# yxgeee/OpenIBL

Hardware: NVIDIA H100
Metric: images_per_sec_extraction (higher is better)
Workload: dtype f32 (bf16x3 split on wgmma, fp32 accumulate)

## Files before the change

### include/iblb200.h

```cpp
#ifndef IBLB200_H_
#define IBLB200_H_

#include <stddef.h>
#include <stdint.h>

#ifdef __cplusplus
extern "C" {
#endif

#define IBLB200_ABI_VERSION 1

typedef enum ibl_status {
  IBL_OK = 0,
  IBL_ERR_BAD_ARG = 1,
  IBL_ERR_NOT_READY = 2,
  IBL_ERR_CUDA = 3,
  IBL_ERR_NO_DEVICE = 4,
  IBL_ERR_OOM = 5,
  IBL_ERR_UNSUPPORTED = 6
} ibl_status;

typedef struct ibl_engine ibl_engine;

#define IBL_OUT_VLAD 0x1u
#define IBL_OUT_PCA  0x2u
#define IBL_OUT_POOL 0x4u

#define IBL_CONV_SIMT_FP32 0
#define IBL_CONV_TC_BF16X3 1

int ibl_abi_version(void);
const char* ibl_status_string(int status);
const char* ibl_last_error(void);

int ibl_engine_create(int device, ibl_engine** out);
int ibl_engine_destroy(ibl_engine* e);
int ibl_engine_set_conv_mode(ibl_engine* e, int mode);
int ibl_engine_get_conv_mode(ibl_engine* e, int* mode);
int ibl_engine_set_gemm_mode(ibl_engine* e, int mode);
int ibl_engine_launch_count(ibl_engine* e, uint64_t* count);

int ibl_engine_set_vgg16(ibl_engine* e, const float* const* weights13,
                         const float* const* biases13, void* stream);
int ibl_engine_set_netvlad(ibl_engine* e, const float* conv_w, const float* centroids,
                           int K, int C, void* stream);
int ibl_engine_set_pca(ibl_engine* e, const float* W, const float* b, int P, int D, void* stream);

int ibl_vgg16_forward(ibl_engine* e, const float* x_nchw, int N, int H, int W,
                      float* feat_nhwc, float* feat_nchw, float* pool, void* stream);

int ibl_vgg16_prefix_forward(ibl_engine* e, const float* x_nchw, int N, int H, int W, int n_layers,
                             float* out_nhwc, void* stream);
int ibl_vgg16_layer_forward(ibl_engine* e, int layer, const float* x, int N, int H, int W, float* y_nhwc,
                            void* stream);
int ibl_maxpool2x2_forward(ibl_engine* e, const float* x_nhwc, int N, int H, int W, int C, float* y_nhwc,
                           void* stream);
int ibl_maxpool2x2_backward(ibl_engine* e, const float* x_nhwc, const float* gy_nhwc, int N, int H, int W, int C,
                            float* gx_nhwc, void* stream);
int ibl_vgg16_layer_backward(ibl_engine* e, int layer, const float* x, const float* y, const float* gy, int N,
                             int H, int W, float* gx, float* gw, float* gb, void* stream);

int ibl_netvlad_forward(ibl_engine* e, const float* feat, int nhwc, int N, int C, int S,
                        const float* conv_w, const float* centroids, int K,
                        int normalize_input, float* vlad_raw, float* vlad_norm, void* stream);
int ibl_netvlad_backward(ibl_engine* e, const float* feat, int nhwc, int N, int C, int S,
                         const float* conv_w, const float* centroids, int K, int normalize_input,
                         const float* grad_vlad, float* grad_feat, float* grad_conv_w,
                         float* grad_centroids, void* stream);
int ibl_vlad_normalize(ibl_engine* e, const float* vlad_raw, int N, int K, int C,
                       float* out, void* stream);

int ibl_pca_l2(ibl_engine* e, const float* v, int N, int D, const float* W, const float* b,
               int P, float* out, void* stream);
int ibl_l2_normalize_rows(ibl_engine* e, const float* x, int N, int D, float* out, void* stream);

int ibl_extract(ibl_engine* e, const float* x_nchw, int N, int H, int W, unsigned flags,
                float* out, float* pool, void* stream);
int ibl_extract_host(ibl_engine* e, const float* x_nchw_host, int N, int H, int W,
                     unsigned flags, float* out_host, float* pool_host, void* stream);

int ibl_extract_host_submit(ibl_engine* e, int slot, const float* x_nchw_host, int N, int H, int W, unsigned flags,
                            float* out_host, float* pool_host, void* stream);
int ibl_extract_host_wait(ibl_engine* e, int slot);

int ibl_preprocess_u8(ibl_engine* e, const uint8_t* x_nhwc, int N, int H, int W, const float* mean3,
                      const float* std3, float* out_nchw, void* stream);
int ibl_resize_bilinear_u8(ibl_engine* e, const uint8_t* x_nhwc, int N, int Hin, int Win, int Hout, int Wout,
                           const int* bounds_h, const int* kk_h, int ksize_h, const int* bounds_v, const int* kk_v,
                           int ksize_v, uint8_t* out_nhwc, void* stream);
int ibl_extract_host_u8(ibl_engine* e, const uint8_t* x_nhwc_host, int N, int H, int W, const float* mean3,
                        const float* std3, unsigned flags, float* out_host, float* pool_host, void* stream);

typedef struct ibl_jpeg_info {
  int width, height;
  int components;
  int h_samp, v_samp;
  int restart_interval;
  int intervals;
  int mcus;
  uint64_t entropy_bytes;
  char reason[120];
} ibl_jpeg_info;
int ibl_jpeg_parse(const uint8_t* data, size_t len, ibl_jpeg_info* out);
int ibl_jpeg_decode_u8(ibl_engine* e, const uint8_t* const* files, const size_t* lens, int N, uint8_t* out_u8,
                       const uint64_t* out_offsets, int* status, int* err_dev, void* stream);
typedef struct ibl_jpeg_scan {
  int components;
  int comp[3];
  int ss, se, ah, al;
  int restart_interval;
  int intervals;
} ibl_jpeg_scan;
int ibl_jpeg_parse_progressive(const uint8_t* data, size_t len, ibl_jpeg_info* out, int* n_scans,
                               ibl_jpeg_scan* scans, int max_scans);
int ibl_jpeg_decode_progressive_u8(ibl_engine* e, const uint8_t* const* files, const size_t* lens, int N,
                                   uint8_t* out_u8, const uint64_t* out_offsets, int* status, int* err_dev,
                                   void* stream);

typedef struct ibl_png_info {
  int width, height;
  int color_type;
  int bit_depth;
  int palette_size;
  uint64_t zlib_bytes;
  char reason[120];
} ibl_png_info;
int ibl_png_parse(const uint8_t* data, size_t len, ibl_png_info* out);
int ibl_png_decode_u8(ibl_engine* e, const uint8_t* const* files, const size_t* lens, int N, uint8_t* out_u8,
                      const uint64_t* out_offsets, int* status, int* err_dev, void* stream);

typedef struct ibl_color_jitter_params {
  int order[4];
  float brightness, contrast, saturation, hue;
} ibl_color_jitter_params;
int ibl_color_jitter_u8(ibl_engine* e, uint8_t* buf, const uint64_t* out_offsets, const int* H, const int* W,
                        const ibl_color_jitter_params* params, int N, void* stream);

int ibl_l2dist_self(ibl_engine* e, const float* x, int n, int d, float* out, void* stream);
int ibl_l2dist_dense(ibl_engine* e, const float* q, int m, const float* db, int n, int d,
                     float* out, void* stream);
int ibl_l2dist_topk(ibl_engine* e, const float* q, int m, const float* db, int n, int n_valid,
                    int d, int k, int64_t idx_base, float* out_dist, int64_t* out_idx,
                    void* stream);
int ibl_topk_rows(ibl_engine* e, const float* dist, int m, int n, int k, float* out_dist,
                  int64_t* out_idx, void* stream);
int ibl_argsort_rows(ibl_engine* e, const float* dist, int m, int n, int64_t* out_idx, void* stream);
int ibl_topk_merge(ibl_engine* e, const float* cand_dist, const int64_t* cand_idx, int parts,
                   int m, int k_in, int k_out, float* out_dist, int64_t* out_idx, void* stream);
int ibl_l2dist_topk_host(ibl_engine* e, const float* q_host, int m, const float* db_host, int n,
                         int d, int k, float* out_dist_host, int64_t* out_idx_host, void* stream);

int ibl_knn_rowmax(ibl_engine* e, const float* X, int N, int d, int row0, int n_rows, int w, int64_t* out_idx,
                   float* out_dist, float* out_rowmax, void* stream);
int ibl_rerank_topk(ibl_engine* e, const float* X, int N, int m, int d, const int64_t* nbr_idx, const float* nbr_dist,
                    int w, const float* rowmax, int k1, int k2, float lambda_value, const int64_t* orig_idx, int k_orig,
                    int k, float* out_dist, int64_t* out_idx, void* stream);
int ibl_rerank_dense(ibl_engine* e, const float* qg, const float* qq, const float* gg, int m, int n, int k1, int k2,
                     double lambda_value, float* out_final, void* stream);

int ibl_gemm_nt(ibl_engine* e, const float* A, int m, const float* B, int n, int k, float alpha, float* C, int mode,
                void* stream);

int ibl_debug_dist_flagged(ibl_engine* e, int* count, void* stream);
int ibl_debug_dist_path(ibl_engine* e, int* path);
int ibl_debug_knn_flagged(ibl_engine* e, int* count, void* stream);
int ibl_debug_rerank_workspace_bytes(ibl_engine* e, uint64_t* bytes);
int ibl_selftest_tc(ibl_engine* e, float* max_rel_err);

int ibl_debug_conv3x3(ibl_engine* e, const float* x_nhwc, int N, int H, int W, int cin,
                      const float* w_oihw, const float* bias, int cout, int relu, int pool, int mode,
                      int bn_override, float* y_nhwc, void* stream);

int ibl_debug_gemm_tn(ibl_engine* e, const float* A, const float* B, float* C, void* stream);
int ibl_debug_umma_strided(ibl_engine* e, const void* A, int rows, const void* B, int s0, int group_rows,
                           int base_mode, float* D, void* stream);
int ibl_debug_umma_halo_view(ibl_engine* e, const void* A, int rows, const void* B, int s0, int group_rows,
                             int half_rows, float* D, void* stream);
int ibl_debug_conv1_fused(ibl_engine* e, const float* x, int N, int H, int W, void* y_hi, void* y_lo, void* stream);
int ibl_debug_time_layer(ibl_engine* e, int layer, const float* x, int N, int H, int W, int bn_override,
                         int reps, float* ms_out);

#ifdef __cplusplus
}
#endif
#endif
```

### openibl_b200/_cabi.py

```python
from __future__ import annotations

import ctypes
import os
from ctypes import POINTER, Structure, c_char, c_char_p, c_double, c_float, c_int, c_int64, c_size_t, c_uint, c_uint64, c_void_p

_HERE = os.path.dirname(os.path.abspath(__file__))
LIB_PATH = os.path.join(_HERE, "lib", "libiblb200.so")

IBL_OK = 0
STATUS_NAMES = {0: "IBL_OK", 1: "IBL_ERR_BAD_ARG", 2: "IBL_ERR_NOT_READY", 3: "IBL_ERR_CUDA",
                4: "IBL_ERR_NO_DEVICE", 5: "IBL_ERR_OOM", 6: "IBL_ERR_UNSUPPORTED"}
OUT_VLAD, OUT_PCA, OUT_POOL = 0x1, 0x2, 0x4
CONV_SIMT_FP32, CONV_TC_BF16X3 = 0, 1
PNG_SIGNATURE = b"\x89PNG\r\n\x1a\n"

_P = c_void_p


class JpegInfo(Structure):
    _fields_ = [("width", c_int), ("height", c_int), ("components", c_int), ("h_samp", c_int), ("v_samp", c_int),
                ("restart_interval", c_int), ("intervals", c_int), ("mcus", c_int), ("entropy_bytes", c_uint64),
                ("reason", c_char * 120)]


class JpegScan(Structure):
    _fields_ = [("components", c_int), ("comp", c_int * 3), ("ss", c_int), ("se", c_int), ("ah", c_int), ("al", c_int),
                ("restart_interval", c_int), ("intervals", c_int)]


class PngInfo(Structure):
    _fields_ = [("width", c_int), ("height", c_int), ("color_type", c_int), ("bit_depth", c_int),
                ("palette_size", c_int), ("zlib_bytes", c_uint64), ("reason", c_char * 120)]


class ColorJitterParams(Structure):
    _fields_ = [("order", c_int * 4), ("brightness", c_float), ("contrast", c_float), ("saturation", c_float),
                ("hue", c_float)]


SIGNATURES = {
    "ibl_abi_version": (c_int, []),
    "ibl_status_string": (c_char_p, [c_int]),
    "ibl_last_error": (c_char_p, []),
    "ibl_engine_create": (c_int, [c_int, POINTER(c_void_p)]),
    "ibl_engine_destroy": (c_int, [_P]),
    "ibl_engine_set_conv_mode": (c_int, [_P, c_int]),
    "ibl_engine_set_gemm_mode": (c_int, [_P, c_int]),
    "ibl_engine_get_conv_mode": (c_int, [_P, POINTER(c_int)]),
    "ibl_engine_launch_count": (c_int, [_P, POINTER(c_uint64)]),
    "ibl_engine_set_vgg16": (c_int, [_P, POINTER(c_void_p), POINTER(c_void_p), _P]),
    "ibl_engine_set_netvlad": (c_int, [_P, _P, _P, c_int, c_int, _P]),
    "ibl_engine_set_pca": (c_int, [_P, _P, _P, c_int, c_int, _P]),
    "ibl_vgg16_forward": (c_int, [_P, _P, c_int, c_int, c_int, _P, _P, _P, _P]),
    "ibl_vgg16_prefix_forward": (c_int, [_P, _P, c_int, c_int, c_int, c_int, _P, _P]),
    "ibl_vgg16_layer_forward": (c_int, [_P, c_int, _P, c_int, c_int, c_int, _P, _P]),
    "ibl_maxpool2x2_forward": (c_int, [_P, _P, c_int, c_int, c_int, c_int, _P, _P]),
    "ibl_maxpool2x2_backward": (c_int, [_P, _P, _P, c_int, c_int, c_int, c_int, _P, _P]),
    "ibl_vgg16_layer_backward": (c_int, [_P, c_int, _P, _P, _P, c_int, c_int, c_int, _P, _P, _P, _P]),
    "ibl_netvlad_forward": (c_int, [_P, _P, c_int, c_int, c_int, c_int, _P, _P, c_int, c_int, _P, _P, _P]),
    "ibl_netvlad_backward": (c_int, [_P, _P, c_int, c_int, c_int, c_int, _P, _P, c_int, c_int, _P, _P, _P, _P, _P]),
    "ibl_vlad_normalize": (c_int, [_P, _P, c_int, c_int, c_int, _P, _P]),
    "ibl_pca_l2": (c_int, [_P, _P, c_int, c_int, _P, _P, c_int, _P, _P]),
    "ibl_l2_normalize_rows": (c_int, [_P, _P, c_int, c_int, _P, _P]),
    "ibl_extract": (c_int, [_P, _P, c_int, c_int, c_int, c_uint, _P, _P, _P]),
    "ibl_extract_host": (c_int, [_P, _P, c_int, c_int, c_int, c_uint, _P, _P, _P]),
    "ibl_extract_host_submit": (c_int, [_P, c_int, _P, c_int, c_int, c_int, c_uint, _P, _P, _P]),
    "ibl_extract_host_wait": (c_int, [_P, c_int]),
    "ibl_preprocess_u8": (c_int, [_P, _P, c_int, c_int, c_int, _P, _P, _P, _P]),
    "ibl_resize_bilinear_u8": (c_int, [_P, _P, c_int, c_int, c_int, c_int, c_int, _P, _P, c_int, _P, _P, c_int, _P, _P]),
    "ibl_extract_host_u8": (c_int, [_P, _P, c_int, c_int, c_int, _P, _P, c_uint, _P, _P, _P]),
    "ibl_jpeg_parse": (c_int, [c_char_p, c_size_t, POINTER(JpegInfo)]),
    "ibl_jpeg_decode_u8": (c_int, [_P, _P, _P, c_int, _P, _P, _P, _P, _P]),
    "ibl_jpeg_parse_progressive": (c_int, [c_char_p, c_size_t, POINTER(JpegInfo), POINTER(c_int), POINTER(JpegScan),
                                           c_int]),
    "ibl_jpeg_decode_progressive_u8": (c_int, [_P, _P, _P, c_int, _P, _P, _P, _P, _P]),
    "ibl_png_parse": (c_int, [c_char_p, c_size_t, POINTER(PngInfo)]),
    "ibl_png_decode_u8": (c_int, [_P, _P, _P, c_int, _P, _P, _P, _P, _P]),
    "ibl_color_jitter_u8": (c_int, [_P, _P, _P, _P, _P, POINTER(ColorJitterParams), c_int, _P]),
    "ibl_l2dist_dense": (c_int, [_P, _P, c_int, _P, c_int, c_int, _P, _P]),
    "ibl_l2dist_self": (c_int, [_P, _P, c_int, c_int, _P, _P]),
    "ibl_l2dist_topk": (c_int, [_P, _P, c_int, _P, c_int, c_int, c_int, c_int, c_int64, _P, _P, _P]),
    "ibl_topk_rows": (c_int, [_P, _P, c_int, c_int, c_int, _P, _P, _P]),
    "ibl_argsort_rows": (c_int, [_P, _P, c_int, c_int, _P, _P]),
    "ibl_topk_merge": (c_int, [_P, _P, _P, c_int, c_int, c_int, c_int, _P, _P, _P]),
    "ibl_l2dist_topk_host": (c_int, [_P, _P, c_int, _P, c_int, c_int, c_int, _P, _P, _P]),
    "ibl_knn_rowmax": (c_int, [_P, _P, c_int, c_int, c_int, c_int, c_int, _P, _P, _P, _P]),
    "ibl_rerank_topk": (c_int, [_P, _P, c_int, c_int, c_int, _P, _P, c_int, _P, c_int, c_int, c_float, _P, c_int,
                                c_int, _P, _P, _P]),
    "ibl_rerank_dense": (c_int, [_P, _P, _P, _P, c_int, c_int, c_int, c_int, c_double, _P, _P]),
    "ibl_debug_rerank_workspace_bytes": (c_int, [_P, POINTER(c_uint64)]),
    "ibl_debug_knn_flagged": (c_int, [_P, POINTER(c_int), _P]),
    "ibl_gemm_nt": (c_int, [_P, _P, c_int, _P, c_int, c_int, c_float, _P, c_int, _P]),
    "ibl_debug_dist_flagged": (c_int, [_P, POINTER(c_int), _P]),
    "ibl_debug_dist_path": (c_int, [_P, POINTER(c_int)]),
    "ibl_selftest_tc": (c_int, [_P, POINTER(c_float)]),
    "ibl_debug_gemm_tn": (c_int, [_P, _P, _P, _P, _P]),
    "ibl_debug_umma_strided": (c_int, [_P, _P, c_int, _P, c_int, c_int, c_int, _P, _P]),
    "ibl_debug_umma_halo_view": (c_int, [_P, _P, c_int, _P, c_int, c_int, c_int, _P, _P]),
    "ibl_debug_conv1_fused": (c_int, [_P, _P, c_int, c_int, c_int, _P, _P, _P]),
    "ibl_debug_time_layer": (c_int, [_P, c_int, _P, c_int, c_int, c_int, c_int, c_int, POINTER(c_float)]),
    "ibl_debug_conv3x3": (c_int, [_P, _P, c_int, c_int, c_int, c_int, _P, _P, c_int, c_int, c_int, c_int,
                                  c_int, _P, _P]),
}

_lib = None


class IblError(RuntimeError):
    def __init__(self, status: int, where: str, detail: str):
        self.status = status
        super().__init__(f"{where}: {STATUS_NAMES.get(status, status)}: {detail}")


def load(build_if_missing: bool = True) -> ctypes.CDLL:
    global _lib
    if _lib is not None:
        return _lib
    if not os.path.exists(LIB_PATH):
        if not build_if_missing:
            raise ImportError(f"{LIB_PATH} is missing; run `python -m openibl_b200.build`")
        from . import build as _build
        _build.build()
    lib = ctypes.CDLL(LIB_PATH)
    for name, (res, args) in SIGNATURES.items():
        fn = getattr(lib, name)
        fn.restype = res
        fn.argtypes = args
    _lib = lib
    return lib


def jpeg_parse(data: bytes) -> dict:
    lib = load()
    info = JpegInfo()
    data = bytes(data)
    st = lib.ibl_jpeg_parse(data, len(data), ctypes.byref(info))
    return {"ok": st == IBL_OK, "status": st, "width": info.width, "height": info.height,
            "components": info.components, "h_samp": info.h_samp, "v_samp": info.v_samp,
            "restart_interval": info.restart_interval, "intervals": info.intervals, "mcus": info.mcus,
            "entropy_bytes": info.entropy_bytes, "reason": info.reason.decode()}


def jpeg_parse_progressive(data: bytes) -> dict:
    lib = load()
    info = JpegInfo()
    data = bytes(data)
    n = c_int(0)
    st = lib.ibl_jpeg_parse_progressive(data, len(data), ctypes.byref(info), ctypes.byref(n), None, 0)
    scans = (JpegScan * max(n.value, 1))()
    if n.value:
        lib.ibl_jpeg_parse_progressive(data, len(data), ctypes.byref(info), ctypes.byref(n), scans, n.value)
    return {"ok": st == IBL_OK, "status": st, "width": info.width, "height": info.height,
            "components": info.components, "h_samp": info.h_samp, "v_samp": info.v_samp,
            "restart_interval": info.restart_interval, "intervals": info.intervals, "mcus": info.mcus,
            "entropy_bytes": info.entropy_bytes, "reason": info.reason.decode(),
            "scans": [{"components": tuple(s.comp[:s.components]), "ss": s.ss, "se": s.se, "ah": s.ah, "al": s.al,
                       "restart_interval": s.restart_interval, "intervals": s.intervals}
                      for s in scans[:n.value]]}


def png_parse(data: bytes) -> dict:
    lib = load()
    info = PngInfo()
    data = bytes(data)
    st = lib.ibl_png_parse(data, len(data), ctypes.byref(info))
    return {"ok": st == IBL_OK, "status": st, "width": info.width, "height": info.height,
            "color_type": info.color_type, "bit_depth": info.bit_depth, "palette_size": info.palette_size,
            "zlib_bytes": info.zlib_bytes, "reason": info.reason.decode()}


def check(status: int, where: str) -> None:
    if status != IBL_OK:
        lib = load()
        detail = lib.ibl_last_error().decode() or lib.ibl_status_string(status).decode()
        raise IblError(status, where, detail)
```

### openibl_b200/csrc/common.cuh

```cuda
#pragma once
#include <cuda_runtime.h>
#include <cuda_bf16.h>
#include <stdint.h>
#include <stdio.h>
#include <atomic>
#include <string>

#include "../../include/iblb200.h"

namespace ibl {

void set_last_error(const std::string& s);

#define IBL_CUDA_OK(expr)                                                          \
  do {                                                                             \
    cudaError_t _e = (expr);                                                       \
    if (_e != cudaSuccess) {                                                       \
      ::ibl::set_last_error(std::string(#expr) + ": " + cudaGetErrorString(_e) +   \
                            " (" __FILE__ ":" + std::to_string(__LINE__) + ")");   \
      return IBL_ERR_CUDA;                                                         \
    }                                                                              \
  } while (0)

#define IBL_RET(expr)                 \
  do {                                \
    int _s = (expr);                  \
    if (_s != IBL_OK) return _s;      \
  } while (0)

#define IBL_REQUIRE(cond, msg)                                  \
  do {                                                          \
    if (!(cond)) {                                              \
      ::ibl::set_last_error(std::string("bad argument: ") + msg); \
      return IBL_ERR_BAD_ARG;                                   \
    }                                                           \
  } while (0)

static inline int cdiv(long long a, long long b) { return (int)((a + b - 1) / b); }

constexpr int NETVLAD_MAX_K = 64;
static inline int check_netvlad_clusters(int K) {
  if (K < 1) {
    set_last_error("bad argument: NetVLAD num_clusters must be in 1..64, got " + std::to_string(K));
    return IBL_ERR_BAD_ARG;
  }
  if (K > NETVLAD_MAX_K) {
    set_last_error("unsupported: NetVLAD num_clusters must be in 1..64, got " + std::to_string(K));
    return IBL_ERR_UNSUPPORTED;
  }
  return IBL_OK;
}

struct DeviceOnce {
  std::atomic<unsigned long long> mask[4];
  DeviceOnce() { for (auto& m : mask) m.store(0); }
  static int cur() { int d = 0; cudaGetDevice(&d); return d & 255; }
  bool done() const { const int d = cur(); return (mask[d >> 6].load(std::memory_order_acquire) >> (d & 63)) & 1ull; }
  void mark() { const int d = cur(); mask[d >> 6].fetch_or(1ull << (d & 63), std::memory_order_release); }
};

static inline int device_sm_count() {
  int dev = 0, sms = 0;
  cudaGetDevice(&dev);
  if (cudaDeviceGetAttribute(&sms, cudaDevAttrMultiProcessorCount, dev) != cudaSuccess || sms <= 0) sms = 132;
  return sms;
}

struct ConvLayer {
  int cin, cout;
  bool relu;
  bool pool;
};

struct ConvParams {
  float* w_tck = nullptr;
  float* bias = nullptr;
  __nv_bfloat16* w_hi = nullptr;
  __nv_bfloat16* w_lo = nullptr;
  int cin_pad = 0;
};

int launch_repack_weights(const float* w_oihw, int cout, int cin, ConvParams& p, cudaStream_t s);
int launch_conv3x3_simt(const float* x_nhwc, const ConvParams& p, int N, int H, int W, int cin,
                        int cout, bool relu, float* y_nhwc, cudaStream_t s);
int launch_conv1_1(const float* x_nchw, const ConvParams& p, int N, int H, int W, float* y_nhwc, cudaStream_t s);
int launch_maxpool2x2(const float* x, int N, int H, int W, int C, float* y, cudaStream_t s);
int launch_nhwc_to_nchw(const float* x, int N, int S, int C, float* y, cudaStream_t s);
int launch_u8_hwc_to_nchw_norm(const uint8_t* x, int N, int H, int W, const float* mean, const float* stdv, float* y,
                               cudaStream_t s);
int launch_global_maxpool_nhwc(const float* x, int N, int S, int C, float* y, cudaStream_t s);
int launch_planes_to_f32(const __nv_bfloat16* hi, const __nv_bfloat16* lo, size_t n, float* y,
                         cudaStream_t s);
int launch_f32_to_planes(const float* x, size_t n, __nv_bfloat16* hi, __nv_bfloat16* lo,
                         cudaStream_t s);

struct TcConvPlan;
int tc_driver_init();
int launch_conv3x3_tc(const __nv_bfloat16* x_hi, const __nv_bfloat16* x_lo, const ConvParams& p,
                      int N, int H, int W, int cin, int cout, bool relu, bool pool,
                      __nv_bfloat16* y_hi, __nv_bfloat16* y_lo, float* y_f32, cudaStream_t s,
                      float* ssq = nullptr, int* ssq_parts = nullptr);
int launch_conv1_fused_tc(const float* x_nchw, const float* w1_oihw, const float* bias1, const ConvParams& p2, int N, int H,
                          int W, __nv_bfloat16* y_hi, __nv_bfloat16* y_lo, cudaStream_t s);
int launch_maxpool2x2_planes(const __nv_bfloat16* hi, const __nv_bfloat16* lo, int N, int H, int W,
                             int C, __nv_bfloat16* yhi, __nv_bfloat16* ylo, cudaStream_t s);
int tc_selftest(float* max_rel_err, cudaStream_t s);
int launch_argsort_rows(const float* dist, long long ld, int m, int n, long long* idx, unsigned long long* scratch,
                        cudaStream_t s, uint64_t* launches);
int launch_resize_bilinear_u8(const uint8_t* x, int N, int Hin, int Win, int Hout, int Wout, const int* bounds_h,
                              const int* kk_h, int ksize_h, const int* bounds_v, const int* kk_v, int ksize_v,
                              uint8_t* tmp, uint8_t* out, cudaStream_t s, uint64_t* launches);
struct JpegWs {
  uint8_t* host = nullptr;
  size_t host_cap = 0;
  void* blob = nullptr;
  size_t blob_cap = 0;
  void* arena = nullptr;
  size_t arena_cap = 0;
  cudaEvent_t copied = nullptr;
  bool pending = false;
};
void jpeg_ws_destroy(JpegWs* ws);
int ws_open(JpegWs** pws);
int grow_device(void** p, size_t* cap, size_t need);
int stage_host(JpegWs* ws, size_t bytes);
int jpeg_decode_u8(JpegWs** ws, const uint8_t* const* files, const size_t* lens, int N, uint8_t* out_u8,
                   const uint64_t* out_offsets, int* status, int* err_dev, cudaStream_t s, uint64_t* launches);
int jpeg_decode_progressive_u8(JpegWs** ws, const uint8_t* const* files, const size_t* lens, int N, uint8_t* out_u8,
                               const uint64_t* out_offsets, int* status, int* err_dev, cudaStream_t s,
                               uint64_t* launches);
int png_decode_u8(JpegWs** ws, const uint8_t* const* files, const size_t* lens, int N, uint8_t* out_u8,
                  const uint64_t* out_offsets, int* status, int* err_dev, cudaStream_t s, uint64_t* launches);
struct JitterWs;
void jitter_ws_destroy(JitterWs* ws);
int color_jitter_u8(JitterWs** ws, uint8_t* buf, const uint64_t* out_offsets, const int* H, const int* W,
                    const ibl_color_jitter_params* params, int N, cudaStream_t s, uint64_t* launches);
int launch_repack_weights_dgrad(const float* w_tck, int cout, int cin, __nv_bfloat16* w_hi, __nv_bfloat16* w_lo,
                                cudaStream_t s);
int launch_relu_mask_planes(const float* g, const float* y, size_t n, bool relu, __nv_bfloat16* hi, __nv_bfloat16* lo,
                            cudaStream_t s);
int launch_maxpool2x2_bwd(const float* x, const float* gy, int N, int H, int W, int C, float* gx, cudaStream_t s);
int wgrad_tc_splits(int N, int H, int W, int cin, int cout);
int launch_conv_wgrad_tc(const __nv_bfloat16* g_hi, const __nv_bfloat16* g_lo, const __nv_bfloat16* x_hi,
                         const __nv_bfloat16* x_lo, int N, int H, int W, int cin, int cout, float* part, int splits,
                         float* bpart, float* dw_oihw, float* db, cudaStream_t s);
int launch_conv1_1_wgrad(const float* x_nchw, const __nv_bfloat16* g_hi, const __nv_bfloat16* g_lo, int N, int H, int W,
                         float* part, float* dw_oihw, float* db, cudaStream_t s);
int launch_conv1_1_tc(const float* x_nchw, const float* w_oihw, const float* bias, int N, int H, int W,
                      __nv_bfloat16* y_hi, __nv_bfloat16* y_lo, cudaStream_t s);
int debug_gmma_strided(const void* A, int rows, const void* B, int s0, int group_rows, int half_rows, int base_mode,
                       float* D, cudaStream_t s);
int debug_gemm_tn(const float* A, const float* B, float* C, cudaStream_t s);
int netvlad_tc_units(int B, int S);
int launch_netvlad_tc(const __nv_bfloat16* x_hi, const __nv_bfloat16* x_lo, int B, int S, int K,
                      const __nv_bfloat16* w_hi, const __nv_bfloat16* w_lo, const float* ssq, int ssq_parts,
                      const float* cent, bool normalize_input, float* part, float* asum_part, int* ticket,
                      float* vlad_raw, float* vlad_norm, cudaStream_t s);
int launch_global_maxpool_planes(const __nv_bfloat16* hi, const __nv_bfloat16* lo, int N, int S, int C, float* y,
                                 cudaStream_t s);

int dist_top16_max_runs(int n_valid);
int launch_dist_top16_tc(const __nv_bfloat16* q_hi, const __nv_bfloat16* q_lo, const float* qn, int m,
                         const __nv_bfloat16* d_hi, const __nv_bfloat16* d_lo, const float* dn, int n,
                         int n_valid, int K, float* cand_d, long long* cand_i, int max_runs, int* runs_out,
                         cudaStream_t s);
int launch_dist_dense_tc(const __nv_bfloat16* q_hi, const __nv_bfloat16* q_lo, const float* qn, int m,
                         const __nv_bfloat16* d_hi, const __nv_bfloat16* d_lo, const float* dn, int n, int K,
                         float* out, long long ld_out, cudaStream_t s);
size_t dist1_workspace_bytes(int m, int n, int d, size_t* off );
int launch_dist_topk_1pass(const float* q, int m, const float* db, int n, int n_valid, int d, int k, long long idx_base,
                           void* ws, float* out_dist, long long* out_idx, uint64_t* launches, cudaStream_t s);
const int* dist1_flag_counter(const void* ws, int m, int n, int d);
size_t dist_guard_workspace_bytes(int m);
int launch_dist_guard_bf16x3(const float* q, const float* q_sq, const float2* q_err, int m, const float* db,
                             const float* db_sq, const float2* db_err, int n_valid, int d, const float* screened, int kc,
                             int k, long long idx_base, void* ws, float* out_dist, long long* out_idx,
                             uint64_t* launches, cudaStream_t s);
int launch_bf16x3_colmax(const float2* err, const float* sq, int n, float* out3, cudaStream_t s);
int pca_tc_splits(int P, int D);
int launch_pca_partial_tc(const __nv_bfloat16* w_hi, const __nv_bfloat16* w_lo, int P,
                          const __nv_bfloat16* v_hi, const __nv_bfloat16* v_lo, int N, int D,
                          float* partial, int* splits_out, cudaStream_t s);
int launch_rescore_sort(const float* q, const float* qn, int m, const float* db, const float* dbn, int d,
                        const long long* cand_i, int kc, int k_out, long long idx_base, float* out_dist,
                        long long* out_idx, cudaStream_t s);
int launch_pca_finalize(const float* partial, int splits, int N, int P, const float* bias, float* out,
                        cudaStream_t s);

struct NetvladWorkspace {
  float* assign = nullptr;
  float* invnorm = nullptr;
  float* asum = nullptr;
  float* raw = nullptr;
  size_t cap_N = 0;
  int cap_S = 0, cap_K = 0, cap_C = 0;
};
int launch_netvlad(const float* feat, bool nhwc, int N, int C, int S, const float* conv_w,
                   const float* centroids, int K, bool normalize_input, float* assign,
                   float* invnorm, float* asum, float* vlad_raw, float* vlad_norm,
                   cudaStream_t s, uint64_t* launches);
int launch_vlad_normalize(const float* raw, int N, int K, int C, float* out, cudaStream_t s);
int launch_netvlad_assign(const float* feat, bool nhwc, int N, int C, int S, const float* conv_w, int K,
                          bool normalize_input, float* assign, float* invnorm, cudaStream_t s);
int launch_netvlad_backward(const float* x, bool nhwc, int N, int C, int S, const float* conv_w,
                            const float* centroids, int K, const float* g, bool normalize_input, float* assign,
                            float* invnorm, float* dz, float* part, int splits, float* dx, float* dW,
                            float* dcent, cudaStream_t s, uint64_t* launches);

int launch_pca_l2(const float* v, int N, int D, const float* W, const float* b, int P,
                  float* partial, int splits, float* out, cudaStream_t s, uint64_t* launches);
int launch_l2_normalize_rows(const float* x, int N, int D, float* out, cudaStream_t s);
int launch_row_sqnorm(const float* x, int N, int D, float* out, cudaStream_t s);
int launch_scale(const float* x, float s, int n, float* y, cudaStream_t st);
int launch_planes_sqnorm(const float* x, int N, int D, __nv_bfloat16* hi, __nv_bfloat16* lo, float* sq,
                         float2* err, cudaStream_t st);
int launch_l2dist_dense(const float* q, const float* qn, int m, const float* db, const float* dbn,
                        int n, int d, float* out, long long ld_out, cudaStream_t s);

size_t knn_rowmax_workspace_bytes(int N, int d, int n_rows, int w);
const int* knn_rowmax_flag_counter(const void* ws, int N, int d, int n_rows, int w);
int launch_knn_rowmax(const float* X, int N, int d, int row0, int n_rows, int w, void* ws, long long* out_idx,
                      float* out_dist, float* out_max, uint64_t* launches, cudaStream_t s);
struct RerankWs;
RerankWs* rerank_ws_create();
void rerank_ws_destroy(RerankWs* w);
size_t rerank_ws_bytes(const RerankWs* w);
int launch_rerank_topk(RerankWs* W, const float* X, int N, int m, int d, const long long* nbr, const float* nbr_dist,
                       int w, const float* rowmax, int k1, int k2, float lam, const long long* orig, int k_orig, int k,
                       float* out_dist, long long* out_idx, uint64_t* launches, cudaStream_t s);
int launch_rerank_dense(RerankWs* W, const float* qg, const float* qq, const float* gg, int m, int n, int k1, int k2,
                        double lam, float* out, uint64_t* launches, cudaStream_t s);

int launch_topk_rows(const float* dist, long long ld, int m, int n_valid, int k, int64_t idx_base,
                     float* out_dist, int64_t* out_idx, bool accumulate, cudaStream_t s);
int launch_topk_merge(const float* cand_dist, const int64_t* cand_idx, int parts, int m, int k_in,
                      int k_out, float* out_dist, int64_t* out_idx, cudaStream_t s);

}
```

### openibl_b200/csrc/engine.cu

```cuda
#include <stdlib.h>

#include <mutex>
#include <new>
#include <vector>

#include "common.cuh"

namespace ibl {

static thread_local std::string g_last_error;
void set_last_error(const std::string& s) { g_last_error = s; }
void tc_set_bn_override(int bn);

static const ConvLayer kVgg16[13] = {
    {3, 64, true, false},    {64, 64, true, true},
    {64, 128, true, false},  {128, 128, true, true},
    {128, 256, true, false}, {256, 256, true, false}, {256, 256, true, true},
    {256, 512, true, false}, {512, 512, true, false}, {512, 512, true, true},
    {512, 512, true, false}, {512, 512, true, false}, {512, 512, false, false}
};

struct DevBuf {
  void* p = nullptr;
  size_t cap = 0;
  int ensure(size_t bytes) {
    if (bytes <= cap) return IBL_OK;
    if (p) cudaFree(p);
    p = nullptr;
    cap = 0;
    cudaError_t e = cudaMalloc(&p, bytes);
    if (e != cudaSuccess) {
      cudaGetLastError();
      set_last_error("workspace cudaMalloc(" + std::to_string(bytes) + " B) failed: " + cudaGetErrorString(e));
      return IBL_ERR_OOM;
    }
    cap = bytes;
    return IBL_OK;
  }
  void release() {
    if (p) cudaFree(p);
    p = nullptr;
    cap = 0;
  }
  template <class T> T* as() const { return reinterpret_cast<T*>(p); }
};

}

using namespace ibl;

struct ibl_engine {
  int device = 0;
  int conv_mode = IBL_CONV_TC_BF16X3;
  int gemm_mode = IBL_CONV_TC_BF16X3;
  uint64_t launches = 0;
  bool vgg_ready = false;
  ConvParams conv[13];
  float* w0_oihw = nullptr;
  const float* nv_w = nullptr;
  const float* nv_c = nullptr;
  int nv_K = 0, nv_C = 0;
  const float* pca_W = nullptr;
  const float* pca_b = nullptr;
  int pca_P = 0, pca_D = 0;
  DevBuf act[2];
  DevBuf feat;
  DevBuf nv_assign, nv_inv, nv_raw, vlad;
  DevBuf pca_partial;
  DevBuf qn, dbn, dist_chunk, cand_d, cand_i;
  DevBuf stage_in, stage_out, stage_out2, stage_u8;
  DevBuf q_pl, db_pl, v_pl, pca_pl;
  const float* pca_pl_src = nullptr;
  DevBuf mrg_d, mrg_i;
  DevBuf bw_g, bw_x, bw_part, bw_w;
  DevBuf d1_ws;
  DevBuf q_err, db_err, guard_ws;
  DevBuf knn_ws;
  const int* knn_flag_counter = nullptr;
  JpegWs* jpeg_ws = nullptr;
  JpegWs* jpeg_prog_ws = nullptr;
  JpegWs* png_ws = nullptr;
  JitterWs* jitter_ws = nullptr;
  RerankWs* rr_ws = nullptr;
  const int* flag_counter = nullptr;
  int dist_path = -1;
  DevBuf ssq, nv_part, nv_asum, nvw_pl;
  DevBuf nv_ticket;
  const float* nvw_pl_src = nullptr;
  cudaStream_t copy_stream = nullptr;
  cudaEvent_t copy_ev[2] = {nullptr, nullptr};
  DevBuf pipe_in[2], pipe_out[2], pipe_pool[2];
  cudaEvent_t pipe_h2d[2] = {nullptr, nullptr}, pipe_done[2] = {nullptr, nullptr};
  bool pipe_busy[2] = {false, false};
};

struct FeatPlanes {
  __nv_bfloat16* hi = nullptr;
  __nv_bfloat16* lo = nullptr;
  int ssq_parts = 0;
};

namespace {

inline cudaStream_t S(void* s) { return reinterpret_cast<cudaStream_t>(s); }

struct DeviceGuard {
  int prev = -1;
  explicit DeviceGuard(int dev) {
    cudaGetDevice(&prev);
    if (prev != dev) cudaSetDevice(dev);
    else prev = -1;
  }
  ~DeviceGuard() {
    if (prev >= 0) cudaSetDevice(prev);
  }
};

int ensure_tickets(ibl_engine* e, int n_images, cudaStream_t s) {
  const size_t need = (size_t)(n_images > 1024 ? n_images : 1024) * sizeof(int);
  if (e->nv_ticket.cap >= need) return IBL_OK;
  IBL_RET(e->nv_ticket.ensure(need));
  IBL_CUDA_OK(cudaMemsetAsync(e->nv_ticket.p, 0, e->nv_ticket.cap, s));
  return IBL_OK;
}

int vgg_forward_impl(ibl_engine* e, const float* x, int N, int H, int W, float* feat_nhwc,
                     cudaStream_t s, FeatPlanes* planes_out = nullptr, int last_layer = 12) {
  const size_t act_bytes = (size_t)N * H * W * 64 * 4;
  IBL_RET(e->act[0].ensure(act_bytes));
  IBL_RET(e->act[1].ensure(act_bytes));
  int h = H, w = W;
  int cur = 0;
  if (e->conv_mode == IBL_CONV_SIMT_FP32) {
    IBL_RET(launch_conv1_1(x, e->conv[0], N, h, w, e->act[0].as<float>(), s));
    e->launches++;
    for (int l = 1; l <= last_layer; ++l) {
      const ConvLayer& L = kVgg16[l];
      const bool last = (l == last_layer);
      float* dst = (last && !L.pool) ? feat_nhwc : e->act[cur ^ 1].as<float>();
      IBL_RET(launch_conv3x3_simt(e->act[cur].as<float>(), e->conv[l], N, h, w, L.cin, L.cout, L.relu, dst, s));
      e->launches++;
      cur ^= 1;
      if (L.pool) {
        IBL_RET(launch_maxpool2x2(e->act[cur].as<float>(), N, h, w, L.cout, last ? feat_nhwc : e->act[cur ^ 1].as<float>(), s));
        e->launches++;
        cur ^= 1;
        h /= 2;
        w /= 2;
      }
    }
    return IBL_OK;
  }
  auto hi_of = [&](int b, size_t elems) { (void)elems; return e->act[b].as<__nv_bfloat16>(); };
  auto lo_of = [&](int b, size_t elems) { return e->act[b].as<__nv_bfloat16>() + elems; };
  size_t elems = (size_t)N * h * w * 64;
  int first_l = 1;
  const bool fused1 = last_layer >= 2 && h >= 2 && w >= 2;
  if (fused1) {
    const size_t out_elems = (size_t)N * (h / 2) * (w / 2) * 64;
    IBL_RET(launch_conv1_fused_tc(x, e->w0_oihw, e->conv[0].bias, e->conv[1], N, h, w, hi_of(1, out_elems),
                                  lo_of(1, out_elems), s));
    e->launches++;
    cur = 1;
    h /= 2;
    w /= 2;
    first_l = 2;
  } else {
    IBL_RET(launch_conv1_1_tc(x, e->w0_oihw, e->conv[0].bias, N, h, w, hi_of(0, elems), lo_of(0, elems), s));
    e->launches++;
  }
  for (int l = first_l; l <= last_layer; ++l) {
    const ConvLayer& L = kVgg16[l];
    const bool last = (l == last_layer);
    const size_t in_elems = (size_t)N * h * w * L.cin;
    const int oh = L.pool ? h / 2 : h, ow = L.pool ? w / 2 : w;
    const size_t out_elems = (size_t)N * oh * ow * L.cout;
    if (last && planes_out) {
      IBL_RET(e->ssq.ensure((size_t)8 * N * oh * ow * sizeof(float)));
      IBL_RET(launch_conv3x3_tc(hi_of(cur, in_elems), lo_of(cur, in_elems), e->conv[l], N, h, w, L.cin,
                                L.cout, L.relu, L.pool, hi_of(cur ^ 1, out_elems), lo_of(cur ^ 1, out_elems),
                                nullptr, s, e->ssq.as<float>(), &planes_out->ssq_parts));
      planes_out->hi = hi_of(cur ^ 1, out_elems);
      planes_out->lo = lo_of(cur ^ 1, out_elems);
      e->launches++;
      return IBL_OK;
    }
    IBL_RET(launch_conv3x3_tc(hi_of(cur, in_elems), lo_of(cur, in_elems), e->conv[l], N, h, w, L.cin,
                              L.cout, L.relu, L.pool, last ? nullptr : hi_of(cur ^ 1, out_elems),
                              last ? nullptr : lo_of(cur ^ 1, out_elems), last ? feat_nhwc : nullptr, s));
    e->launches++;
    cur ^= 1;
    h = oh;
    w = ow;
  }
  return IBL_OK;
}

}

extern "C" {

int ibl_abi_version(void) { return IBLB200_ABI_VERSION; }

const char* ibl_status_string(int status) {
  switch (status) {
    case IBL_OK: return "ok";
    case IBL_ERR_BAD_ARG: return "bad argument";
    case IBL_ERR_NOT_READY: return "parameters for this stage were not set";
    case IBL_ERR_CUDA: return "CUDA error";
    case IBL_ERR_NO_DEVICE: return "no usable sm_90 CUDA device (this library has no CPU fallback)";
    case IBL_ERR_OOM: return "out of device memory";
    case IBL_ERR_UNSUPPORTED: return "unsupported request";
    default: return "unknown status";
  }
}

const char* ibl_last_error(void) { return g_last_error.c_str(); }

int ibl_engine_create(int device, ibl_engine** out) {
  if (!out) return IBL_ERR_BAD_ARG;
  *out = nullptr;
  int count = 0;
  if (cudaGetDeviceCount(&count) != cudaSuccess || count <= 0) {
    cudaGetLastError();
    set_last_error("no CUDA device visible; libiblb200 has no CPU fallback");
    return IBL_ERR_NO_DEVICE;
  }
  IBL_REQUIRE(device >= 0 && device < count, "device index out of range");
  cudaDeviceProp prop;
  IBL_CUDA_OK(cudaGetDeviceProperties(&prop, device));
  if (prop.major != 9 || prop.minor != 0) {
    set_last_error(std::string("device '") + prop.name + "' is sm_" + std::to_string(prop.major) +
                   std::to_string(prop.minor) + "; this library is built for sm_90a only");
    return IBL_ERR_NO_DEVICE;
  }
  ibl_engine* e = new (std::nothrow) ibl_engine();
  if (!e) return IBL_ERR_OOM;
  e->device = device;
  *out = e;
  return IBL_OK;
}

int ibl_engine_destroy(ibl_engine* e) {
  if (!e) return IBL_OK;
  DeviceGuard g(e->device);
  for (auto& c : e->conv) {
    if (c.w_tck) cudaFree(c.w_tck);
    if (c.bias) cudaFree(c.bias);
    if (c.w_hi) cudaFree(c.w_hi);
    if (c.w_lo) cudaFree(c.w_lo);
  }
  if (e->w0_oihw) cudaFree(e->w0_oihw);
  if (e->copy_stream) { cudaStreamDestroy(e->copy_stream); cudaEventDestroy(e->copy_ev[0]); cudaEventDestroy(e->copy_ev[1]); }
  for (int i = 0; i < 2; ++i) {
    if (e->pipe_h2d[i]) cudaEventDestroy(e->pipe_h2d[i]);
    if (e->pipe_done[i]) cudaEventDestroy(e->pipe_done[i]);
    e->pipe_in[i].release(); e->pipe_out[i].release(); e->pipe_pool[i].release();
  }
  DevBuf* bufs[] = {&e->act[0], &e->act[1], &e->feat, &e->nv_assign, &e->nv_inv, &e->nv_raw, &e->vlad,
                    &e->pca_partial, &e->qn, &e->dbn, &e->dist_chunk, &e->cand_d, &e->cand_i,
                    &e->stage_in, &e->stage_out, &e->stage_out2, &e->stage_u8, &e->q_pl, &e->db_pl, &e->v_pl, &e->pca_pl,
                    &e->mrg_d, &e->mrg_i, &e->d1_ws, &e->bw_g, &e->bw_x, &e->bw_part, &e->bw_w, &e->ssq, &e->nv_part, &e->nv_asum, &e->nvw_pl, &e->nv_ticket};
  for (DevBuf* b : bufs) b->release();
  e->knn_ws.release();
  rerank_ws_destroy(e->rr_ws);
  jpeg_ws_destroy(e->jpeg_ws);
  jpeg_ws_destroy(e->jpeg_prog_ws);
  jpeg_ws_destroy(e->png_ws);
  jitter_ws_destroy(e->jitter_ws);
  delete e;
  return IBL_OK;
}

int ibl_engine_set_conv_mode(ibl_engine* e, int mode) {
  IBL_REQUIRE(e, "null engine");
  IBL_REQUIRE(mode == IBL_CONV_SIMT_FP32 || mode == IBL_CONV_TC_BF16X3, "unknown conv mode");
  e->conv_mode = mode;
  return IBL_OK;
}
int ibl_engine_get_conv_mode(ibl_engine* e, int* mode) {
  IBL_REQUIRE(e && mode, "null argument");
  *mode = e->conv_mode;
  return IBL_OK;
}
int ibl_engine_set_gemm_mode(ibl_engine* e, int mode) {
  IBL_REQUIRE(e, "null engine");
  IBL_REQUIRE(mode == IBL_CONV_SIMT_FP32 || mode == IBL_CONV_TC_BF16X3, "unknown gemm mode");
  e->gemm_mode = mode;
  return IBL_OK;
}
int ibl_engine_launch_count(ibl_engine* e, uint64_t* count) {
  IBL_REQUIRE(e && count, "null argument");
  *count = e->launches;
  return IBL_OK;
}

int ibl_engine_set_vgg16(ibl_engine* e, const float* const* w13, const float* const* b13, void* stream) {
  IBL_REQUIRE(e && w13 && b13, "null argument");
  DeviceGuard g(e->device);
  for (int l = 0; l < 13; ++l) {
    IBL_REQUIRE(w13[l] && b13[l], "null weight/bias pointer");
    const ConvLayer& L = kVgg16[l];
    ConvParams& p = e->conv[l];
    const size_t nw = (size_t)L.cout * L.cin * 9;
    if (!p.w_tck) IBL_CUDA_OK(cudaMalloc(&p.w_tck, nw * sizeof(float)));
    if (!p.bias) IBL_CUDA_OK(cudaMalloc(&p.bias, L.cout * sizeof(float)));
    if (L.cin % 64 == 0) {
      if (!p.w_hi) IBL_CUDA_OK(cudaMalloc(&p.w_hi, nw * sizeof(__nv_bfloat16)));
      if (!p.w_lo) IBL_CUDA_OK(cudaMalloc(&p.w_lo, nw * sizeof(__nv_bfloat16)));
      p.cin_pad = L.cin;
    }
    IBL_RET(launch_repack_weights(w13[l], L.cout, L.cin, p, S(stream)));
    IBL_CUDA_OK(cudaMemcpyAsync(p.bias, b13[l], L.cout * sizeof(float), cudaMemcpyDeviceToDevice, S(stream)));
    if (l == 0) {
      if (!e->w0_oihw) IBL_CUDA_OK(cudaMalloc(&e->w0_oihw, nw * sizeof(float)));
      IBL_CUDA_OK(cudaMemcpyAsync(e->w0_oihw, w13[0], nw * sizeof(float), cudaMemcpyDeviceToDevice, S(stream)));
    }
    e->launches++;
  }
  e->vgg_ready = true;
  return IBL_OK;
}

static int netvlad_weight_planes(const float* conv_w, int K, __nv_bfloat16* pl, cudaStream_t s) {
  const size_t n64 = (size_t)NETVLAD_MAX_K * 512;
  if (K < NETVLAD_MAX_K) IBL_CUDA_OK(cudaMemsetAsync(pl, 0, n64 * 4, s));
  return launch_f32_to_planes(conv_w, (size_t)K * 512, pl, pl + n64, s);
}

int ibl_engine_set_netvlad(ibl_engine* e, const float* conv_w, const float* centroids, int K, int C,
                           void* stream) {
  IBL_RET(check_netvlad_clusters(K));
  IBL_REQUIRE(e && conv_w && centroids, "null argument");
  IBL_REQUIRE(C >= 4 && C % 4 == 0, "NetVLAD dim must be a positive multiple of 4");
  e->nv_w = conv_w;
  e->nv_c = centroids;
  e->nv_K = K;
  e->nv_C = C;
  e->nvw_pl_src = nullptr;
  if (C == 512) {
    DeviceGuard g(e->device);
    IBL_RET(e->nvw_pl.ensure((size_t)NETVLAD_MAX_K * 512 * 4));
    IBL_RET(netvlad_weight_planes(conv_w, K, e->nvw_pl.as<__nv_bfloat16>(), S(stream)));
    e->launches++;
    e->nvw_pl_src = conv_w;
  }
  return IBL_OK;
}

int ibl_engine_set_pca(ibl_engine* e, const float* W, const float* b, int P, int D, void* stream) {
  (void)stream;
  IBL_REQUIRE(e && W && b, "null argument");
  IBL_REQUIRE(P >= 1 && D >= 4 && D % 4 == 0, "bad PCA shape");
  e->pca_W = W;
  e->pca_b = b;
  e->pca_P = P;
  e->pca_D = D;
  e->pca_pl_src = nullptr;
  if (D % 64 == 0) {
    DeviceGuard g(e->device);
    const size_t n = (size_t)P * D;
    IBL_RET(e->pca_pl.ensure(n * 4));
    IBL_RET(launch_f32_to_planes(W, n, e->pca_pl.as<__nv_bfloat16>(), e->pca_pl.as<__nv_bfloat16>() + n, S(stream)));
    e->launches++;
    e->pca_pl_src = W;
  }
  return IBL_OK;
}

int ibl_vgg16_forward(ibl_engine* e, const float* x, int N, int H, int W, float* feat_nhwc,
                      float* feat_nchw, float* pool, void* stream) {
  IBL_REQUIRE(e && x, "null argument");
  IBL_REQUIRE(N >= 1 && H >= 16 && W >= 16, "VGG16 trunk needs N>=1 and H,W>=16");
  if (!e->vgg_ready) { set_last_error("ibl_engine_set_vgg16 was not called"); return IBL_ERR_NOT_READY; }
  DeviceGuard g(e->device);
  const int fh = H / 16, fw = W / 16;
  const size_t fbytes = (size_t)N * fh * fw * 512 * sizeof(float);
  float* f = feat_nhwc;
  if (!f) {
    IBL_RET(e->feat.ensure(fbytes));
    f = e->feat.as<float>();
  }
  IBL_RET(vgg_forward_impl(e, x, N, H, W, f, S(stream)));
  if (feat_nchw) { IBL_RET(launch_nhwc_to_nchw(f, N, fh * fw, 512, feat_nchw, S(stream))); e->launches++; }
  if (pool) { IBL_RET(launch_global_maxpool_nhwc(f, N, fh * fw, 512, pool, S(stream))); e->launches++; }
  return IBL_OK;
}


int ibl_vgg16_prefix_forward(ibl_engine* e, const float* x, int N, int H, int W, int n_layers, float* out_nhwc,
                             void* stream) {
  IBL_REQUIRE(e && x && out_nhwc, "null argument");
  IBL_REQUIRE(n_layers >= 1 && n_layers <= 13, "prefix length must be 1..13");
  IBL_REQUIRE(N >= 1 && H >= 16 && W >= 16, "VGG16 trunk needs N>=1 and H,W>=16");
  if (!e->vgg_ready) { set_last_error("ibl_engine_set_vgg16 was not called"); return IBL_ERR_NOT_READY; }
  DeviceGuard g(e->device);
  if (n_layers == 1) {
    e->launches++;
    return launch_conv1_1(x, e->conv[0], N, H, W, out_nhwc, S(stream));
  }
  return vgg_forward_impl(e, x, N, H, W, out_nhwc, S(stream), nullptr, n_layers - 1);
}

int ibl_vgg16_layer_forward(ibl_engine* e, int layer, const float* x, int N, int H, int W, float* y_nhwc, void* stream) {
  IBL_REQUIRE(e && x && y_nhwc, "null argument");
  IBL_REQUIRE(layer >= 0 && layer < 13 && N >= 1 && H >= 1 && W >= 1, "bad layer / shape");
  if (!e->vgg_ready) { set_last_error("ibl_engine_set_vgg16 was not called"); return IBL_ERR_NOT_READY; }
  DeviceGuard g(e->device);
  cudaStream_t s = S(stream);
  const ConvLayer& L = kVgg16[layer];
  if (layer == 0) {
    e->launches++;
    return launch_conv1_1(x, e->conv[0], N, H, W, y_nhwc, s);
  }
  if (e->conv_mode == IBL_CONV_SIMT_FP32) {
    e->launches++;
    return launch_conv3x3_simt(x, e->conv[layer], N, H, W, L.cin, L.cout, L.relu, y_nhwc, s);
  }
  const size_t in_e = (size_t)N * H * W * L.cin;
  IBL_RET(e->act[0].ensure(in_e * 4));
  __nv_bfloat16* xh = e->act[0].as<__nv_bfloat16>();
  IBL_RET(launch_f32_to_planes(x, in_e, xh, xh + in_e, s));
  IBL_RET(launch_conv3x3_tc(xh, xh + in_e, e->conv[layer], N, H, W, L.cin, L.cout, L.relu, false, nullptr, nullptr,
                            y_nhwc, s));
  e->launches += 2;
  return IBL_OK;
}

int ibl_maxpool2x2_forward(ibl_engine* e, const float* x_nhwc, int N, int H, int W, int C, float* y_nhwc, void* stream) {
  IBL_REQUIRE(e && x_nhwc && y_nhwc && N >= 1 && H >= 2 && W >= 2 && C >= 4 && C % 4 == 0, "bad argument");
  DeviceGuard g(e->device);
  e->launches++;
  return launch_maxpool2x2(x_nhwc, N, H, W, C, y_nhwc, S(stream));
}

int ibl_maxpool2x2_backward(ibl_engine* e, const float* x_nhwc, const float* gy_nhwc, int N, int H, int W, int C,
                            float* gx_nhwc, void* stream) {
  IBL_REQUIRE(e && x_nhwc && gy_nhwc && gx_nhwc && N >= 1 && H >= 2 && W >= 2 && C >= 1, "bad argument");
  DeviceGuard g(e->device);
  e->launches++;
  return launch_maxpool2x2_bwd(x_nhwc, gy_nhwc, N, H, W, C, gx_nhwc, S(stream));
}

int ibl_vgg16_layer_backward(ibl_engine* e, int layer, const float* x, const float* y, const float* gy, int N, int H,
                             int W, float* gx, float* gw, float* gb, void* stream) {
  IBL_REQUIRE(e && x && gy && gw && gb, "null argument");
  IBL_REQUIRE(layer >= 0 && layer < 13 && N >= 1 && H >= 1 && W >= 1, "bad layer / shape");
  if (!e->vgg_ready) { set_last_error("ibl_engine_set_vgg16 was not called"); return IBL_ERR_NOT_READY; }
  const ConvLayer& L = kVgg16[layer];
  IBL_REQUIRE(!L.relu || y, "the layer has a ReLU: its output is needed for the mask");
  DeviceGuard g(e->device);
  cudaStream_t s = S(stream);
  const size_t out_e = (size_t)N * H * W * L.cout, in_e = (size_t)N * H * W * L.cin;
  IBL_RET(e->bw_g.ensure(out_e * 4));
  __nv_bfloat16* gh = e->bw_g.as<__nv_bfloat16>();
  IBL_RET(launch_relu_mask_planes(gy, y, out_e, L.relu, gh, gh + out_e, s));
  e->launches++;
  if (layer == 0) {
    IBL_REQUIRE(!gx, "conv1_1 has no input gradient (its input is the image)");
    IBL_RET(e->bw_part.ensure((size_t)1024 * 64 * 28 * sizeof(float)));
    IBL_RET(launch_conv1_1_wgrad(x, gh, gh + out_e, N, H, W, e->bw_part.as<float>(), gw, gb, s));
    e->launches += 2;
    return IBL_OK;
  }
  IBL_RET(e->bw_x.ensure(in_e * 4));
  __nv_bfloat16* xh = e->bw_x.as<__nv_bfloat16>();
  IBL_RET(launch_f32_to_planes(x, in_e, xh, xh + in_e, s));
  const int splits = wgrad_tc_splits(N, H, W, L.cin, L.cout);
  IBL_RET(e->bw_part.ensure(((size_t)splits * 9 * L.cout * L.cin + (size_t)256 * L.cout) * sizeof(float)));
  float* part = e->bw_part.as<float>();
  IBL_RET(launch_conv_wgrad_tc(gh, gh + out_e, xh, xh + in_e, N, H, W, L.cin, L.cout, part, splits,
                               part + (size_t)splits * 9 * L.cout * L.cin, gw, gb, s));
  e->launches += 5;
  if (gx) {
    const size_t nw = (size_t)L.cout * L.cin * 9;
    IBL_RET(e->bw_w.ensure(nw * 4 + (size_t)L.cin * sizeof(float)));
    ConvParams p;
    p.w_hi = e->bw_w.as<__nv_bfloat16>();
    p.w_lo = p.w_hi + nw;
    p.bias = reinterpret_cast<float*>(p.w_lo + nw);
    p.cin_pad = L.cout;
// ... 483 lines not shown
      const int max_runs = dist_top16_max_runs(n_valid);
      IBL_RET(e->cand_d.ensure((size_t)max_runs * m * kc * sizeof(float)));
      IBL_RET(e->cand_i.ensure((size_t)max_runs * m * kc * sizeof(int64_t)));
      IBL_RET(launch_dist_top16_tc(qh, qh + qe, e->qn.as<float>(), m, dh, dh + de, e->dbn.as<float>(), n,
                                   n_valid, d, e->cand_d.as<float>(), e->cand_i.as<long long>(), max_runs,
                                   &parts, s));
      e->launches++;
    } else {
      const int CHT = 32768;
      parts = cdiv(n_valid, CHT);
      kc = k + 8 > 128 ? 128 : k + 8;
      IBL_REQUIRE((long long)parts * kc <= 8192, "database shard too large for one call; shard it");
      const int chw = n_valid < CHT ? cdiv(n_valid, 4) * 4 : CHT;
      IBL_RET(e->dist_chunk.ensure((size_t)m * chw * sizeof(float)));
      IBL_RET(e->cand_d.ensure((size_t)parts * m * kc * sizeof(float)));
      IBL_RET(e->cand_i.ensure((size_t)parts * m * kc * sizeof(int64_t)));
      for (int c = 0; c < parts; ++c) {
        const int j0 = c * CHT;
        const int nc = (n_valid - j0 < CHT) ? (n_valid - j0) : CHT;
        IBL_RET(launch_dist_dense_tc(qh, qh + qe, e->qn.as<float>(), m, dh + (size_t)j0 * d, dh + de + (size_t)j0 * d,
                                     e->dbn.as<float>() + j0, nc, d, e->dist_chunk.as<float>(), chw, s));
        IBL_RET(launch_topk_rows(e->dist_chunk.as<float>(), chw, m, nc, kc, j0,
                                 e->cand_d.as<float>() + (size_t)c * m * kc, e->cand_i.as<int64_t>() + (size_t)c * m * kc,
                                 false, s));
        e->launches += 2;
      }
    }
    const long long* ci = e->cand_i.as<long long>();
    const float* cd = e->cand_d.as<float>();
    if (parts > 1) {
      IBL_RET(e->mrg_d.ensure((size_t)m * kc * sizeof(float)));
      IBL_RET(e->mrg_i.ensure((size_t)m * kc * sizeof(int64_t)));
      IBL_RET(launch_topk_merge(e->cand_d.as<float>(), e->cand_i.as<int64_t>(), parts, m, kc, kc,
                                e->mrg_d.as<float>(), e->mrg_i.as<int64_t>(), s));
      e->launches++;
      ci = e->mrg_i.as<long long>();
      cd = e->mrg_d.as<float>();
    }
    IBL_RET(launch_rescore_sort(q, e->qn.as<float>(), m, db, e->dbn.as<float>(), d, ci, kc, k, idx_base, out_dist,
                                reinterpret_cast<long long*>(out_idx), s));
    e->launches++;
    return launch_dist_guard_bf16x3(q, e->qn.as<float>(), qerr, m, db, e->dbn.as<float>(), dberr, n_valid, d, cd, kc, k,
                                    idx_base, e->guard_ws.p, out_dist, reinterpret_cast<long long*>(out_idx),
                                    &e->launches, s);
  }
  const int CH = 32768;
  e->dist_path = 0;
  e->flag_counter = nullptr;
  const int nch = n_valid > 0 ? cdiv(n_valid, CH) : 1;
  IBL_REQUIRE((long long)nch * k <= 8192, "database shard too large for one call; shard it");
  IBL_RET(e->qn.ensure((size_t)m * sizeof(float)));
  IBL_RET(e->dbn.ensure((size_t)n * sizeof(float)));
  const int chw = n_valid < CH ? (n_valid > 0 ? n_valid : 1) : CH;
  IBL_RET(e->dist_chunk.ensure((size_t)m * chw * sizeof(float)));
  IBL_RET(launch_row_sqnorm(q, m, d, e->qn.as<float>(), S(stream)));
  IBL_RET(launch_row_sqnorm(db, n, d, e->dbn.as<float>(), S(stream)));
  e->launches += 2;
  float* cd = out_dist;
  int64_t* ci = out_idx;
  if (nch > 1) {
    IBL_RET(e->cand_d.ensure((size_t)nch * m * k * sizeof(float)));
    IBL_RET(e->cand_i.ensure((size_t)nch * m * k * sizeof(int64_t)));
    cd = e->cand_d.as<float>();
    ci = e->cand_i.as<int64_t>();
  }
  for (int c = 0; c < nch; ++c) {
    const int j0 = c * CH;
    const int nc = (n_valid - j0 < CH) ? (n_valid - j0) : CH;
    if (nc > 0)
      IBL_RET(launch_l2dist_dense(q, e->qn.as<float>(), m, db + (size_t)j0 * d, e->dbn.as<float>() + j0, nc,
                                  d, e->dist_chunk.as<float>(), chw, S(stream)));
    IBL_RET(launch_topk_rows(e->dist_chunk.as<float>(), chw, m, nc > 0 ? nc : 0, k, idx_base + j0,
                             cd + (size_t)c * m * k, ci + (size_t)c * m * k, false, S(stream)));
    e->launches += 2;
  }
  if (nch > 1) {
    IBL_RET(launch_topk_merge(cd, ci, nch, m, k, k, out_dist, out_idx, S(stream)));
    e->launches++;
  }
  return IBL_OK;
}

int ibl_topk_rows(ibl_engine* e, const float* dist, int m, int n, int k, float* out_dist, int64_t* out_idx,
                  void* stream) {
  IBL_REQUIRE(e && dist && out_dist && out_idx, "null argument");
  IBL_REQUIRE(m >= 0 && n >= 1 && k >= 1 && k <= 1024, "bad shape (ibl_topk_rows: 1 <= k <= 1024)");
  DeviceGuard g(e->device);
  e->launches++;
  return launch_topk_rows(dist, n, m, n, k, 0, out_dist, out_idx, false, S(stream));
}

int ibl_argsort_rows(ibl_engine* e, const float* dist, int m, int n, int64_t* out_idx, void* stream) {
  IBL_REQUIRE(e && dist && out_idx, "null argument");
  IBL_REQUIRE(m >= 0 && n >= 1, "bad shape");
  DeviceGuard g(e->device);
  unsigned long long* scratch = nullptr;
  if (n > 16384) {
    IBL_RET(e->dist_chunk.ensure((size_t)2 * m * n * sizeof(unsigned long long)));
    scratch = e->dist_chunk.as<unsigned long long>();
  }
  return launch_argsort_rows(dist, n, m, n, reinterpret_cast<long long*>(out_idx), scratch, S(stream), &e->launches);
}

int ibl_topk_merge(ibl_engine* e, const float* cand_dist, const int64_t* cand_idx, int parts, int m,
                   int k_in, int k_out, float* out_dist, int64_t* out_idx, void* stream) {
  IBL_REQUIRE(e && cand_dist && cand_idx && out_dist && out_idx, "null argument");
  IBL_REQUIRE(parts >= 1 && m >= 0 && k_in >= 1, "bad shape");
  DeviceGuard g(e->device);
  e->launches++;
  return launch_topk_merge(cand_dist, cand_idx, parts, m, k_in, k_out, out_dist, out_idx, S(stream));
}

int ibl_knn_rowmax(ibl_engine* e, const float* X, int N, int d, int row0, int n_rows, int w, int64_t* out_idx,
                   float* out_dist, float* out_rowmax, void* stream) {
  IBL_REQUIRE(e && X, "null argument");
  IBL_REQUIRE(N >= 1 && d >= 1, "bad shape");
  IBL_REQUIRE(w >= 1 && w <= 128, "knn_rowmax: 1 <= w <= 128");
  IBL_REQUIRE(w <= N, "knn_rowmax: w <= N");
  IBL_REQUIRE(row0 >= 0 && n_rows >= 0 && (long long)row0 + n_rows <= N, "knn_rowmax: rows out of range");
  if (n_rows == 0) return IBL_OK;
  IBL_REQUIRE(out_idx && out_dist && out_rowmax, "null argument");
  DeviceGuard g(e->device);
  IBL_RET(e->knn_ws.ensure(knn_rowmax_workspace_bytes(N, d, n_rows, w)));
  e->knn_flag_counter = knn_rowmax_flag_counter(e->knn_ws.p, N, d, n_rows, w);
  return launch_knn_rowmax(X, N, d, row0, n_rows, w, e->knn_ws.p, reinterpret_cast<long long*>(out_idx), out_dist,
                           out_rowmax, &e->launches, S(stream));
}

int ibl_rerank_topk(ibl_engine* e, const float* X, int N, int m, int d, const int64_t* nbr_idx, const float* nbr_dist,
                    int w, const float* rowmax, int k1, int k2, float lambda_value, const int64_t* orig_idx, int k_orig,
                    int k, float* out_dist, int64_t* out_idx, void* stream) {
  IBL_REQUIRE(e && X && nbr_idx && nbr_dist && rowmax && out_dist && out_idx, "null argument");
  IBL_REQUIRE(N >= 1 && d >= 1 && m >= 1 && m < N, "bad shape (1 <= m < N)");
  IBL_REQUIRE(k1 >= 0 && k1 + 1 <= w && w <= 128, "re-ranking: k1 + 1 <= w <= 128");
  IBL_REQUIRE(N >= k1 + 1, "re-ranking needs at least k1 + 1 images");
  IBL_REQUIRE(k2 >= 1 && k2 <= w, "re-ranking: 1 <= k2 <= w");
  IBL_REQUIRE(k >= 1 && k <= 128, "re-ranking: 1 <= k <= 128");
  IBL_REQUIRE(lambda_value >= 0.f && lambda_value <= 1.f, "re-ranking: 0 <= lambda <= 1");
  IBL_REQUIRE(lambda_value == 0.f || (orig_idx && k_orig >= (k < N - m ? k : N - m) && k_orig <= 256),
              "re-ranking with lambda > 0 needs the original ranking, min(k, N - m) <= k_orig <= 256");
  DeviceGuard g(e->device);
  if (!e->rr_ws) e->rr_ws = rerank_ws_create();
  return launch_rerank_topk(e->rr_ws, X, N, m, d, reinterpret_cast<const long long*>(nbr_idx), nbr_dist, w, rowmax,
                            k1, k2, lambda_value, reinterpret_cast<const long long*>(orig_idx),
                            lambda_value == 0.f ? 0 : k_orig, k, out_dist, reinterpret_cast<long long*>(out_idx),
                            &e->launches, S(stream));
}

int ibl_rerank_dense(ibl_engine* e, const float* qg, const float* qq, const float* gg, int m, int n, int k1, int k2,
                     double lambda_value, float* out_final, void* stream) {
  IBL_REQUIRE(e && qg && qq && gg && out_final, "null argument");
  IBL_REQUIRE(m >= 1 && n >= 1, "bad shape (m >= 1, n >= 1)");
  IBL_REQUIRE(k1 >= 0 && k2 >= 1, "re-ranking: k1 >= 0, k2 >= 1");
  IBL_REQUIRE((long long)m + n >= k1 + 1, "re-ranking needs at least k1 + 1 images");
  IBL_REQUIRE((k1 + 1 > k2 ? k1 + 1 : k2) <= 128, "dense re-ranking: max(k1 + 1, k2) <= 128");
  IBL_REQUIRE(k2 <= m + n, "dense re-ranking: k2 <= m + n");
  IBL_REQUIRE(lambda_value >= 0.0 && lambda_value <= 1.0, "re-ranking: 0 <= lambda <= 1");
  DeviceGuard g(e->device);
  if (!e->rr_ws) e->rr_ws = rerank_ws_create();
  return launch_rerank_dense(e->rr_ws, qg, qq, gg, m, n, k1, k2, lambda_value, out_final, &e->launches, S(stream));
}

int ibl_debug_knn_flagged(ibl_engine* e, int* count, void* stream) {
  IBL_REQUIRE(e && count, "null argument");
  *count = -1;
  if (!e->knn_flag_counter) return IBL_OK;
  DeviceGuard g(e->device);
  IBL_CUDA_OK(cudaMemcpyAsync(count, e->knn_flag_counter, sizeof(int), cudaMemcpyDeviceToHost, S(stream)));
  IBL_CUDA_OK(cudaStreamSynchronize(S(stream)));
  return IBL_OK;
}

int ibl_debug_rerank_workspace_bytes(ibl_engine* e, uint64_t* bytes) {
  IBL_REQUIRE(e && bytes, "null argument");
  *bytes = e->knn_ws.cap + (e->rr_ws ? rerank_ws_bytes(e->rr_ws) : 0);
  return IBL_OK;
}

int ibl_l2dist_topk_host(ibl_engine* e, const float* q_host, int m, const float* db_host, int n, int d,
                         int k, float* out_dist_host, int64_t* out_idx_host, void* stream) {
  IBL_REQUIRE(e && q_host && db_host && out_dist_host && out_idx_host, "null argument");
  IBL_REQUIRE(m >= 1 && n >= 1 && d >= 4 && k >= 1 && k <= 128, "bad shape");
  DeviceGuard g(e->device);
  const size_t qb = (size_t)m * d * sizeof(float), dbb = (size_t)n * d * sizeof(float);
  IBL_RET(e->stage_in.ensure(qb + dbb));
  IBL_RET(e->stage_out.ensure((size_t)m * k * sizeof(float)));
  IBL_RET(e->stage_out2.ensure((size_t)m * k * sizeof(int64_t)));
  float* dq = e->stage_in.as<float>();
  float* ddb = dq + (size_t)m * d;
  IBL_CUDA_OK(cudaMemcpyAsync(dq, q_host, qb, cudaMemcpyHostToDevice, S(stream)));
  IBL_CUDA_OK(cudaMemcpyAsync(ddb, db_host, dbb, cudaMemcpyHostToDevice, S(stream)));
  IBL_RET(ibl_l2dist_topk(e, dq, m, ddb, n, n, d, k, 0, e->stage_out.as<float>(), e->stage_out2.as<int64_t>(), stream));
  IBL_CUDA_OK(cudaMemcpyAsync(out_dist_host, e->stage_out.p, (size_t)m * k * sizeof(float), cudaMemcpyDeviceToHost, S(stream)));
  IBL_CUDA_OK(cudaMemcpyAsync(out_idx_host, e->stage_out2.p, (size_t)m * k * sizeof(int64_t), cudaMemcpyDeviceToHost, S(stream)));
  IBL_CUDA_OK(cudaStreamSynchronize(S(stream)));
  return IBL_OK;
}

int ibl_debug_dist_flagged(ibl_engine* e, int* count, void* stream) {
  IBL_REQUIRE(e && count, "null argument");
  *count = -1;
  if (!e->flag_counter) return IBL_OK;
  DeviceGuard g(e->device);
  IBL_CUDA_OK(cudaMemcpyAsync(count, e->flag_counter, sizeof(int), cudaMemcpyDeviceToHost, S(stream)));
  IBL_CUDA_OK(cudaStreamSynchronize(S(stream)));
  return IBL_OK;
}

int ibl_debug_dist_path(ibl_engine* e, int* path) {
  IBL_REQUIRE(e && path, "null argument");
  *path = e->dist_path;
  return IBL_OK;
}

int ibl_selftest_tc(ibl_engine* e, float* max_rel_err) {
  IBL_REQUIRE(e, "null engine");
  DeviceGuard g(e->device);
  return tc_selftest(max_rel_err, nullptr);
}

int ibl_debug_conv3x3(ibl_engine* e, const float* x_nhwc, int N, int H, int W, int cin, const float* w_oihw,
                      const float* bias, int cout, int relu, int pool, int mode, int bn_override,
                      float* y_nhwc, void* stream) {
  IBL_REQUIRE(e && x_nhwc && w_oihw && bias && y_nhwc, "null argument");
  IBL_REQUIRE(cin % 64 == 0 && cout % 64 == 0, "debug conv needs Cin%64==0, Cout%64==0");
  DeviceGuard g(e->device);
  cudaStream_t s = S(stream);
  ConvParams p;
  const size_t nw = (size_t)cout * cin * 9;
  IBL_CUDA_OK(cudaMalloc(&p.w_tck, nw * 4));
  IBL_CUDA_OK(cudaMalloc(&p.bias, cout * 4));
  IBL_CUDA_OK(cudaMalloc(&p.w_hi, nw * 2));
  IBL_CUDA_OK(cudaMalloc(&p.w_lo, nw * 2));
  int rc = launch_repack_weights(w_oihw, cout, cin, p, s);
  cudaMemcpyAsync(p.bias, bias, cout * 4, cudaMemcpyDeviceToDevice, s);
  const size_t in_e = (size_t)N * H * W * cin;
  const int oh = pool ? H / 2 : H, ow = pool ? W / 2 : W;
  const size_t out_e = (size_t)N * oh * ow * cout;
  if (rc == IBL_OK && mode == IBL_CONV_SIMT_FP32) {
    if (!pool) {
      rc = launch_conv3x3_simt(x_nhwc, p, N, H, W, cin, cout, relu != 0, y_nhwc, s);
    } else {
      float* tmp = nullptr;
      if (cudaMalloc(&tmp, (size_t)N * H * W * cout * 4) != cudaSuccess) rc = IBL_ERR_OOM;
      if (rc == IBL_OK) rc = launch_conv3x3_simt(x_nhwc, p, N, H, W, cin, cout, relu != 0, tmp, s);
      if (rc == IBL_OK) rc = launch_maxpool2x2(tmp, N, H, W, cout, y_nhwc, s);
      cudaStreamSynchronize(s);
      if (tmp) cudaFree(tmp);
    }
  } else if (rc == IBL_OK) {
    __nv_bfloat16 *xh = nullptr, *xl = nullptr;
    if (cudaMalloc(&xh, in_e * 2) != cudaSuccess || cudaMalloc(&xl, in_e * 2) != cudaSuccess) rc = IBL_ERR_OOM;
    if (rc == IBL_OK) rc = launch_f32_to_planes(x_nhwc, in_e, xh, xl, s);
    tc_set_bn_override(bn_override);
    if (mode == 2) {
      __nv_bfloat16 *yh = nullptr, *yl = nullptr;
      if (cudaMalloc(&yh, out_e * 2) != cudaSuccess || cudaMalloc(&yl, out_e * 2) != cudaSuccess) rc = IBL_ERR_OOM;
      if (rc == IBL_OK) rc = launch_conv3x3_tc(xh, xl, p, N, H, W, cin, cout, relu != 0, pool != 0, yh, yl, nullptr, s);
      if (rc == IBL_OK) rc = launch_planes_to_f32(yh, yl, out_e, y_nhwc, s);
      cudaStreamSynchronize(s);
      if (yh) cudaFree(yh);
      if (yl) cudaFree(yl);
    } else if (rc == IBL_OK) {
      rc = launch_conv3x3_tc(xh, xl, p, N, H, W, cin, cout, relu != 0, pool != 0, nullptr, nullptr, y_nhwc, s);
    }
    tc_set_bn_override(0);
    cudaStreamSynchronize(s);
    if (xh) cudaFree(xh);
    if (xl) cudaFree(xl);
  }
  cudaError_t ce = cudaStreamSynchronize(s);
  cudaFree(p.w_tck); cudaFree(p.bias); cudaFree(p.w_hi); cudaFree(p.w_lo);
  if (rc == IBL_OK && ce != cudaSuccess) {
    set_last_error(std::string("debug conv: ") + cudaGetErrorString(ce));
    return IBL_ERR_CUDA;
  }
  e->launches += 3;
  return rc;
}

int ibl_debug_gemm_tn(ibl_engine* e, const float* A, const float* B, float* C, void* stream) {
  IBL_REQUIRE(e && A && B && C, "null argument");
  DeviceGuard g(e->device);
  e->launches += 3;
  return debug_gemm_tn(A, B, C, S(stream));
}

int ibl_debug_umma_strided(ibl_engine* e, const void* A, int rows, const void* B, int s0, int group_rows,
                            int base_mode, float* D, void* stream) {
  IBL_REQUIRE(e && A && B && D, "null argument");
  DeviceGuard g(e->device);
  e->launches += 1;
  return debug_gmma_strided(A, rows, B, s0, group_rows, 8 * group_rows, base_mode, D, S(stream));
}

int ibl_debug_umma_halo_view(ibl_engine* e, const void* A, int rows, const void* B, int s0, int group_rows,
                             int half_rows, float* D, void* stream) {
  IBL_REQUIRE(e && A && B && D, "null argument");
  DeviceGuard g(e->device);
  e->launches += 1;
  return debug_gmma_strided(A, rows, B, s0, group_rows, half_rows, 0, D, S(stream));
}

int ibl_debug_conv1_fused(ibl_engine* e, const float* x, int N, int H, int W, void* y_hi, void* y_lo, void* stream) {
  IBL_REQUIRE(e && x && y_hi && y_lo && N >= 1 && H >= 2 && W >= 2, "bad argument");
  if (!e->vgg_ready) { set_last_error("ibl_engine_set_vgg16 was not called"); return IBL_ERR_NOT_READY; }
  DeviceGuard g(e->device);
  e->launches += 1;
  return launch_conv1_fused_tc(x, e->w0_oihw, e->conv[0].bias, e->conv[1], N, H, W, static_cast<__nv_bfloat16*>(y_hi),
                               static_cast<__nv_bfloat16*>(y_lo), S(stream));
}

int ibl_debug_time_layer(ibl_engine* e, int layer, const float* x, int N, int H, int W, int bn_override,
                         int reps, float* ms_out) {
  IBL_REQUIRE(e && x && ms_out && layer >= -1 && layer <= 12 && reps >= 1, "bad argument");
  if (!e->vgg_ready) { set_last_error("ibl_engine_set_vgg16 was not called"); return IBL_ERR_NOT_READY; }
  DeviceGuard g(e->device);
  const bool fused1 = layer < 0;
  const ConvLayer& L = kVgg16[fused1 ? 1 : layer];
  const size_t in_e = (size_t)N * H * W * L.cin;
  const int oh = L.pool ? H / 2 : H, ow = L.pool ? W / 2 : W;
  const size_t out_e = (size_t)N * oh * ow * L.cout;
  IBL_RET(e->act[0].ensure((in_e > out_e ? in_e : out_e) * 4));
  IBL_RET(e->act[1].ensure((in_e > out_e ? in_e : out_e) * 4));
  cudaEvent_t e0, e1;
  IBL_CUDA_OK(cudaEventCreate(&e0));
  IBL_CUDA_OK(cudaEventCreate(&e1));
  __nv_bfloat16* ih = e->act[0].as<__nv_bfloat16>();
  __nv_bfloat16* oh_ = e->act[1].as<__nv_bfloat16>();
  int rc = IBL_OK;
  if (layer > 0) rc = launch_f32_to_planes(x, in_e, ih, ih + in_e, nullptr);
  tc_set_bn_override(bn_override);
  for (int r = -1; r < reps && rc == IBL_OK; ++r) {
    if (r == 0) cudaEventRecord(e0, nullptr);
    if (fused1)
      rc = launch_conv1_fused_tc(x, e->w0_oihw, e->conv[0].bias, e->conv[1], N, H, W, oh_, oh_ + out_e, nullptr);
    else if (layer == 0)
      rc = launch_conv1_1_tc(x, e->w0_oihw, e->conv[0].bias, N, H, W, oh_, oh_ + out_e, nullptr);
    else
      rc = launch_conv3x3_tc(ih, ih + in_e, e->conv[layer], N, H, W, L.cin, L.cout, L.relu, L.pool,
                             layer == 12 ? nullptr : oh_, layer == 12 ? nullptr : oh_ + out_e,
                             layer == 12 ? e->act[1].as<float>() : nullptr, nullptr);
  }
  tc_set_bn_override(0);
  cudaEventRecord(e1, nullptr);
  cudaError_t ce = cudaEventSynchronize(e1);
  float ms = 0.f;
  cudaEventElapsedTime(&ms, e0, e1);
  cudaEventDestroy(e0);
  cudaEventDestroy(e1);
  if (rc == IBL_OK && ce != cudaSuccess) { set_last_error(cudaGetErrorString(ce)); return IBL_ERR_CUDA; }
  *ms_out = ms / reps;
  e->launches += reps + 1;
  return rc;
}

}
```

### openibl_b200/csrc/tc_common.cuh

```cuda
#pragma once
#include <cuda.h>
#include <cuda_runtime.h>
#include <stdint.h>

#include "wgmma.cuh"

namespace ibl {
namespace tc {

__device__ __forceinline__ uint32_t smem_u32(const void* p) {
  return static_cast<uint32_t>(__cvta_generic_to_shared(p));
}

__device__ __forceinline__ uint32_t warp_uniform(uint32_t v) { return __reduce_or_sync(0xffffffffu, v); }

__device__ __forceinline__ bool elect_one() {
  uint32_t pred;
  asm volatile(
      "{\n\t"
      ".reg .pred p;\n\t"
      "elect.sync _|p, 0xffffffff;\n\t"
      "selp.u32 %0, 1, 0, p;\n\t"
      "}"
      : "=r"(pred));
  return pred != 0;
}

__device__ __forceinline__ void mbar_init(uint64_t* bar, uint32_t count) {
  asm volatile("mbarrier.init.shared::cta.b64 [%0], %1;" ::"r"(smem_u32(bar)), "r"(count) : "memory");
}
__device__ __forceinline__ void mbar_arrive(uint64_t* bar) {
  asm volatile("mbarrier.arrive.shared::cta.b64 _, [%0];" ::"r"(smem_u32(bar)) : "memory");
}
__device__ __forceinline__ void mbar_arrive_expect_tx(uint64_t* bar, uint32_t bytes) {
  asm volatile("mbarrier.arrive.expect_tx.shared::cta.b64 _, [%0], %1;" ::"r"(smem_u32(bar)),
               "r"(bytes)
               : "memory");
}
__device__ __forceinline__ bool mbar_try_wait(uint64_t* bar, uint32_t parity) {
  uint32_t ok;
  asm volatile(
      "{\n\t"
      ".reg .pred p;\n\t"
      "mbarrier.try_wait.parity.shared::cta.b64 p, [%1], %2;\n\t"
      "selp.u32 %0, 1, 0, p;\n\t"
      "}"
      : "=r"(ok)
      : "r"(smem_u32(bar)), "r"(parity)
      : "memory");
  return ok != 0;
}
__device__ __forceinline__ void mbar_wait(uint64_t* bar, uint32_t parity) {
  while (!mbar_try_wait(bar, parity)) {
  }
}
__device__ __forceinline__ void mbar_wait_warp(uint64_t* bar, uint32_t parity) {
  if ((threadIdx.x & 31) == 0) mbar_wait(bar, parity);
  __syncwarp();
}
__device__ __forceinline__ void mbar_wait_warp_a(uint32_t bar_addr, uint32_t parity) {
  if ((threadIdx.x & 31) == 0) {
    uint32_t ok;
    do {
      asm volatile(
          "{\n\t"
          ".reg .pred p;\n\t"
          "mbarrier.try_wait.parity.shared::cta.b64 p, [%1], %2;\n\t"
          "selp.u32 %0, 1, 0, p;\n\t"
          "}"
          : "=r"(ok)
          : "r"(bar_addr), "r"(parity)
          : "memory");
    } while (!ok);
  }
  __syncwarp();
}
__device__ __forceinline__ void fence_barrier_init() {
  asm volatile("fence.mbarrier_init.release.cluster;" ::: "memory");
}
__device__ __forceinline__ void fence_proxy_async() {
  asm volatile("fence.proxy.async.shared::cta;" ::: "memory");
}

__device__ __forceinline__ void tma_prefetch_desc(const CUtensorMap* m) {
  asm volatile("prefetch.tensormap [%0];" ::"l"(reinterpret_cast<uint64_t>(m)) : "memory");
}
__device__ __forceinline__ void tma_load_2d(void* dst, const CUtensorMap* m, uint64_t* bar, int c0,
                                            int c1) {
  asm volatile(
      "cp.async.bulk.tensor.2d.shared::cluster.global.mbarrier::complete_tx::bytes"
      " [%0], [%1, {%3, %4}], [%2];" ::"r"(smem_u32(dst)),
      "l"(reinterpret_cast<uint64_t>(m)), "r"(smem_u32(bar)), "r"(c0), "r"(c1)
      : "memory");
}
__device__ __forceinline__ void tma_load_3d(void* dst, const CUtensorMap* m, uint64_t* bar, int c0,
                                            int c1, int c2) {
  asm volatile(
      "cp.async.bulk.tensor.3d.shared::cluster.global.mbarrier::complete_tx::bytes"
      " [%0], [%1, {%3, %4, %5}], [%2];" ::"r"(smem_u32(dst)),
      "l"(reinterpret_cast<uint64_t>(m)), "r"(smem_u32(bar)), "r"(c0), "r"(c1), "r"(c2)
      : "memory");
}
__device__ __forceinline__ void tma_load_4d(void* dst, const CUtensorMap* m, uint64_t* bar, int c0,
                                            int c1, int c2, int c3) {
  asm volatile(
      "cp.async.bulk.tensor.4d.shared::cluster.global.mbarrier::complete_tx::bytes"
      " [%0], [%1, {%3, %4, %5, %6}], [%2];" ::"r"(smem_u32(dst)),
      "l"(reinterpret_cast<uint64_t>(m)), "r"(smem_u32(bar)), "r"(c0), "r"(c1), "r"(c2), "r"(c3)
      : "memory");
}

__device__ __forceinline__ void mbar_arrive_expect_tx_a(uint32_t bar_addr, uint32_t bytes) {
  asm volatile("mbarrier.arrive.expect_tx.shared::cta.b64 _, [%0], %1;" ::"r"(bar_addr), "r"(bytes) : "memory");
}
__device__ __forceinline__ void tma_load_2d_a(uint32_t dst, const CUtensorMap* m, uint32_t bar_addr, int c0, int c1) {
  asm volatile(
      "cp.async.bulk.tensor.2d.shared::cluster.global.mbarrier::complete_tx::bytes"
      " [%0], [%1, {%3, %4}], [%2];" ::"r"(dst),
      "l"(reinterpret_cast<uint64_t>(m)), "r"(bar_addr), "r"(c0), "r"(c1)
      : "memory");
}
__device__ __forceinline__ void tma_load_3d_a(uint32_t dst, const CUtensorMap* m, uint32_t bar_addr, int c0, int c1,
                                              int c2) {
  asm volatile(
      "cp.async.bulk.tensor.3d.shared::cluster.global.mbarrier::complete_tx::bytes"
      " [%0], [%1, {%3, %4, %5}], [%2];" ::"r"(dst),
      "l"(reinterpret_cast<uint64_t>(m)), "r"(bar_addr), "r"(c0), "r"(c1), "r"(c2)
      : "memory");
}
__device__ __forceinline__ void tma_load_4d_a(uint32_t dst, const CUtensorMap* m, uint32_t bar_addr, int c0, int c1,
                                              int c2, int c3) {
  asm volatile(
      "cp.async.bulk.tensor.4d.shared::cluster.global.mbarrier::complete_tx::bytes"
      " [%0], [%1, {%3, %4, %5, %6}], [%2];" ::"r"(dst),
      "l"(reinterpret_cast<uint64_t>(m)), "r"(bar_addr), "r"(c0), "r"(c1), "r"(c2), "r"(c3)
      : "memory");
}
__device__ __forceinline__ void tma_load_2d_mc_a(uint32_t dst, const CUtensorMap* m, uint32_t bar_addr, int c0, int c1,
                                                 uint16_t mask) {
  asm volatile(
      "cp.async.bulk.tensor.2d.shared::cluster.global.mbarrier::complete_tx::bytes.multicast::cluster"
      " [%0], [%1, {%4, %5}], [%2], %3;" ::"r"(dst),
      "l"(reinterpret_cast<uint64_t>(m)), "r"(bar_addr), "h"(mask), "r"(c0), "r"(c1)
      : "memory");
}
__device__ __forceinline__ void tma_load_3d_mc_a(uint32_t dst, const CUtensorMap* m, uint32_t bar_addr, int c0, int c1,
                                                 int c2, uint16_t mask) {
  asm volatile(
      "cp.async.bulk.tensor.3d.shared::cluster.global.mbarrier::complete_tx::bytes.multicast::cluster"
      " [%0], [%1, {%4, %5, %6}], [%2], %3;" ::"r"(dst),
      "l"(reinterpret_cast<uint64_t>(m)), "r"(bar_addr), "h"(mask), "r"(c0), "r"(c1), "r"(c2)
      : "memory");
}
__device__ __forceinline__ void cluster_sync_all() {
  asm volatile("barrier.cluster.arrive.release.aligned;" ::: "memory");
  asm volatile("barrier.cluster.wait.acquire.aligned;" ::: "memory");
}
__device__ __forceinline__ uint32_t cluster_ctarank() {
  uint32_t r;
  asm volatile("mov.u32 %0, %%cluster_ctarank;" : "=r"(r));
  return r;
}
__device__ __forceinline__ uint32_t mapa_u32(uint32_t addr, uint32_t rank) {
  uint32_t r;
  asm volatile("mapa.shared::cluster.u32 %0, %1, %2;" : "=r"(r) : "r"(addr), "r"(rank));
  return r;
}
__device__ __forceinline__ void mbar_arrive_remote(uint32_t cluster_addr) {
  asm volatile("mbarrier.arrive.release.cluster.shared::cluster.b64 _, [%0];" ::"r"(cluster_addr) : "memory");
}

__device__ __forceinline__ void tma_prefetch_3d(const CUtensorMap* m, int c0, int c1, int c2) {
  asm volatile("cp.async.bulk.prefetch.tensor.3d.L2.global [%0, {%1, %2, %3}];" ::"l"(
                   reinterpret_cast<uint64_t>(m)),
               "r"(c0), "r"(c1), "r"(c2)
               : "memory");
}

__device__ __forceinline__ uint64_t gmma_desc_kmajor_sw128(uint32_t smem_addr) {
  uint64_t d = 0;
  d |= (uint64_t)((smem_addr >> 4) & 0x3fffu);
  d |= (uint64_t)1 << 16;
  d |= (uint64_t)(1024u >> 4) << 32;
  d |= (uint64_t)1 << 62;
  return d;
}
__device__ __forceinline__ uint64_t gmma_desc_kmajor_sw64(uint32_t smem_addr) {
  uint64_t d = 0;
  d |= (uint64_t)((smem_addr >> 4) & 0x3fffu);
  d |= (uint64_t)1 << 16;
  d |= (uint64_t)(512u >> 4) << 32;
  d |= (uint64_t)2 << 62;
  return d;
}
__device__ __forceinline__ uint64_t gmma_desc_mnmajor_sw128(uint32_t smem_addr, uint32_t lbo_bytes) {
  uint64_t d = 0;
  d |= (uint64_t)((smem_addr >> 4) & 0x3fffu);
  d |= (uint64_t)((lbo_bytes >> 4) & 0x3fffu) << 16;
  d |= (uint64_t)(1024u >> 4) << 32;
  d |= (uint64_t)1 << 62;
  return d;
}

__device__ __forceinline__ void wgmma_fence() { asm volatile("wgmma.fence.sync.aligned;" ::: "memory"); }
__device__ __forceinline__ void wgmma_commit() { asm volatile("wgmma.commit_group.sync.aligned;" ::: "memory"); }
template <int N>
__device__ __forceinline__ void wgmma_wait() { asm volatile("wgmma.wait_group.sync.aligned %0;" ::"n"(N) : "memory"); }

__device__ __forceinline__ void wg_sync(int id = 1) { asm volatile("bar.sync %0, 128;" ::"r"(id) : "memory"); }

template <int N>
__device__ __forceinline__ void setmaxnreg_dec() { asm volatile("setmaxnreg.dec.sync.aligned.u32 %0;" ::"n"(N)); }
template <int N>
__device__ __forceinline__ void setmaxnreg_inc() { asm volatile("setmaxnreg.inc.sync.aligned.u32 %0;" ::"n"(N)); }

template <int N>
struct Acc128 {
  float h[2][N / 2];
  template <bool F16 = false, int TA = 0, int TB = 0>
  __device__ __forceinline__ void mma(uint64_t a0, uint64_t a1, uint64_t b, uint32_t accumulate) {
    Wgmma<N, F16, TA, TB>::mma(h[0], a0, b, accumulate);
    Wgmma<N, F16, TA, TB>::mma(h[1], a1, b, accumulate);
  }
  __device__ __forceinline__ void fence_operands() {
#pragma unroll
    for (int j = 0; j < 2; ++j)
#pragma unroll
      for (int i = 0; i < N / 2; ++i) asm volatile("" : "+f"(h[j][i])::"memory");
  }
  __device__ __forceinline__ void rows32(int ch, float* stg, uint32_t (&raw)[32], int bar = 1) const;
};
constexpr int ACC_STG_PITCH = 36;
constexpr int ACC_STG_BYTES = 128 * ACC_STG_PITCH * 4;

template <int N>
__device__ __forceinline__ void Acc128<N>::rows32(int ch, float* stg, uint32_t (&raw)[32], int bar) const {
  const int t = threadIdx.x & 127, w = t >> 5, l = t & 31;
  wg_sync(bar);
#pragma unroll
  for (int j = 0; j < 2; ++j)
#pragma unroll
    for (int i = 0; i < 4; ++i) {
      const int r = 64 * j + 16 * w + (l >> 2), c = 8 * i + 2 * (l & 3);
      const float* f = &h[j][4 * (4 * ch + i)];
      *reinterpret_cast<float2*>(stg + r * ACC_STG_PITCH + c) = make_float2(f[0], f[1]);
      *reinterpret_cast<float2*>(stg + (r + 8) * ACC_STG_PITCH + c) = make_float2(f[2], f[3]);
    }
  wg_sync(bar);
#pragma unroll
  for (int i = 0; i < 8; ++i) {
    const float4 v = *reinterpret_cast<const float4*>(stg + t * ACC_STG_PITCH + 4 * i);
    raw[4 * i] = __float_as_uint(v.x); raw[4 * i + 1] = __float_as_uint(v.y);
    raw[4 * i + 2] = __float_as_uint(v.z); raw[4 * i + 3] = __float_as_uint(v.w);
  }
}

typedef CUresult (*EncodeTiledFn)(CUtensorMap*, CUtensorMapDataType, cuuint32_t, void*,
                                  const cuuint64_t*, const cuuint64_t*, const cuuint32_t*,
                                  const cuuint32_t*, CUtensorMapInterleave, CUtensorMapSwizzle,
                                  CUtensorMapL2promotion, CUtensorMapFloatOOBfill);
EncodeTiledFn get_encode_tiled();

int make_tmap(CUtensorMap* out, CUtensorMapDataType dt, int rank, const void* base,
              const uint64_t* dims, const uint64_t* strides_bytes, const uint32_t* box, int swizzle_bytes = 128);

}
}
```

### openibl_b200/csrc/tc_conv.cu

```cuda
#include "common.cuh"
#include "tc_common.cuh"

namespace ibl {

using namespace tc;

namespace tc {
EncodeTiledFn get_encode_tiled() {
  static const EncodeTiledFn fn = []() -> EncodeTiledFn {
    void* p = nullptr;
    cudaDriverEntryPointQueryResult qres;
    if (cudaGetDriverEntryPoint("cuTensorMapEncodeTiled", &p, cudaEnableDefault, &qres) ==
            cudaSuccess &&
        qres == cudaDriverEntryPointSuccess)
      return reinterpret_cast<EncodeTiledFn>(p);
    return nullptr;
  }();
  return fn;
}

int make_tmap(CUtensorMap* out, CUtensorMapDataType dt, int rank, const void* base,
              const uint64_t* dims, const uint64_t* strides_bytes, const uint32_t* box, int swizzle_bytes) {
  EncodeTiledFn enc = get_encode_tiled();
  if (!enc) {
    set_last_error("cuTensorMapEncodeTiled is not available (no CUDA driver?)");
    return IBL_ERR_NO_DEVICE;
  }
  cuuint64_t gdim[5];
  cuuint64_t gstr[5];
  cuuint32_t bx[5], es[5];
  for (int i = 0; i < rank; ++i) {
    gdim[i] = dims[i];
    bx[i] = box[i];
    es[i] = 1;
  }
  for (int i = 0; i + 1 < rank; ++i) gstr[i] = strides_bytes[i];
  CUresult r = enc(out, dt, (cuuint32_t)rank, const_cast<void*>(base), gdim, gstr, bx, es,
                   CU_TENSOR_MAP_INTERLEAVE_NONE,
                   swizzle_bytes == 64 ? CU_TENSOR_MAP_SWIZZLE_64B : CU_TENSOR_MAP_SWIZZLE_128B,
                   CU_TENSOR_MAP_L2_PROMOTION_L2_256B, CU_TENSOR_MAP_FLOAT_OOB_FILL_NONE);
  if (r != CUDA_SUCCESS) {
    set_last_error("cuTensorMapEncodeTiled failed with CUresult " + std::to_string((int)r));
    return IBL_ERR_CUDA;
  }
  return IBL_OK;
}
}

int tc_driver_init() { return get_encode_tiled() ? IBL_OK : IBL_ERR_NO_DEVICE; }

struct ConvTcArgs {
  int N, H, W, cin, cout;
  int tw_log2;
  int tiles_w, tiles_h;
  int n_tiles;
  int total_tiles;
  int relu, pool;
  const float* bias;
  __nv_bfloat16* y_hi;
  __nv_bfloat16* y_lo;
  float* y_f32;
  float* ssq;
  long long ssq_stride;
};

__device__ __forceinline__ uint32_t pack_bf16x2(float a, float b) {
  __nv_bfloat162 t = __floats2bfloat162_rn(a, b);
  return *reinterpret_cast<uint32_t*>(&t);
}

template <int BN>
__device__ __forceinline__ void conv_epilogue_tile(const ConvTcArgs& a, const Acc128<BN>& acc, float* stg, int img, int h0,
                                                   int w0, int n0, int nt, int r, int c, int dr_lanes, int bar = 1) {
  const int h = h0 + r, w = w0 + c;
  bool valid;
  long long pix;
  if (a.pool) {
    const int OH = a.H >> 1, OW = a.W >> 1;
    const int oh = h >> 1, ow = w >> 1;
    valid = oh < OH && ow < OW && img < a.N;
    pix = ((long long)img * OH + oh) * OW + ow;
  } else {
    valid = h < a.H && w < a.W && img < a.N;
    pix = ((long long)img * a.H + h) * a.W + w;
  }
  float ssq_acc = 0.f;
#pragma unroll
  for (int ch = 0; ch < BN / 32; ++ch) {
    uint32_t raw[32];
    acc.rows32(ch, stg, raw, bar);
    if (a.pool) {
      const bool s1 = (c & 1) != 0, s2 = (r & 1) != 0;
      float u[16];
#pragma unroll
      for (int j = 0; j < 16; ++j) {
        const float lo_h = __uint_as_float(raw[j]), hi_h = __uint_as_float(raw[j + 16]);
        const float got = __shfl_xor_sync(0xffffffffu, s1 ? lo_h : hi_h, 1);
        u[j] = fmaxf(s1 ? hi_h : lo_h, got);
      }
      float w8[8];
#pragma unroll
      for (int j = 0; j < 8; ++j) {
        const float got = __shfl_xor_sync(0xffffffffu, s2 ? u[j] : u[j + 8], dr_lanes);
        w8[j] = fmaxf(s2 ? u[j + 8] : u[j], got);
      }
      if (valid) {
        const int cbase = n0 + ch * 32 + (s1 ? 16 : 0) + (s2 ? 8 : 0);
        const float4 b0 = __ldg(reinterpret_cast<const float4*>(a.bias + cbase));
        const float4 b1 = __ldg(reinterpret_cast<const float4*>(a.bias + cbase) + 1);
        const float bb[8] = {b0.x, b0.y, b0.z, b0.w, b1.x, b1.y, b1.z, b1.w};
#pragma unroll
        for (int j = 0; j < 8; ++j) {
          w8[j] = w8[j] + bb[j];
          if (a.relu) w8[j] = fmaxf(w8[j], 0.f);
        }
        const long long off = pix * a.cout + cbase;
        if (a.y_f32) {
          float4* o = reinterpret_cast<float4*>(a.y_f32 + off);
          o[0] = make_float4(w8[0], w8[1], w8[2], w8[3]);
          o[1] = make_float4(w8[4], w8[5], w8[6], w8[7]);
        } else {
          uint32_t hi[4], lo[4];
#pragma unroll
          for (int j = 0; j < 4; ++j) {
            const float x0 = w8[2 * j], x1 = w8[2 * j + 1];
            const __nv_bfloat16 h0b = __float2bfloat16_rn(x0), h1b = __float2bfloat16_rn(x1);
            __nv_bfloat162 hh(h0b, h1b);
            hi[j] = *reinterpret_cast<uint32_t*>(&hh);
            lo[j] = pack_bf16x2(x0 - __bfloat162float(h0b), x1 - __bfloat162float(h1b));
          }
          *reinterpret_cast<uint4*>(a.y_hi + off) = make_uint4(hi[0], hi[1], hi[2], hi[3]);
          *reinterpret_cast<uint4*>(a.y_lo + off) = make_uint4(lo[0], lo[1], lo[2], lo[3]);
        }
      }
      continue;
    }
    float v[32];
    const float4* bp = reinterpret_cast<const float4*>(a.bias + n0 + ch * 32);
#pragma unroll
    for (int j = 0; j < 8; ++j) {
      const float4 b = __ldg(bp + j);
      v[4 * j + 0] = __uint_as_float(raw[4 * j + 0]) + b.x;
      v[4 * j + 1] = __uint_as_float(raw[4 * j + 1]) + b.y;
      v[4 * j + 2] = __uint_as_float(raw[4 * j + 2]) + b.z;
      v[4 * j + 3] = __uint_as_float(raw[4 * j + 3]) + b.w;
    }
    if (a.relu) {
#pragma unroll
      for (int j = 0; j < 32; ++j) v[j] = fmaxf(v[j], 0.f);
    }
    if (a.ssq) {
#pragma unroll
      for (int j = 0; j < 32; ++j) ssq_acc = fmaf(v[j], v[j], ssq_acc);
    }
    if (valid) {
      const long long off = pix * a.cout + n0 + ch * 32;
      if (a.y_f32) {
        float4* o = reinterpret_cast<float4*>(a.y_f32 + off);
#pragma unroll
        for (int j = 0; j < 8; ++j) o[j] = make_float4(v[4 * j], v[4 * j + 1], v[4 * j + 2], v[4 * j + 3]);
      } else {
        uint32_t hi[16], lo[16];
#pragma unroll
        for (int j = 0; j < 16; ++j) {
          const float x0 = v[2 * j], x1 = v[2 * j + 1];
          const __nv_bfloat16 h0b = __float2bfloat16_rn(x0), h1b = __float2bfloat16_rn(x1);
          __nv_bfloat162 hh(h0b, h1b);
          hi[j] = *reinterpret_cast<uint32_t*>(&hh);
          lo[j] = pack_bf16x2(x0 - __bfloat162float(h0b), x1 - __bfloat162float(h1b));
        }
        uint4* oh4 = reinterpret_cast<uint4*>(a.y_hi + off);
        uint4* ol4 = reinterpret_cast<uint4*>(a.y_lo + off);
#pragma unroll
        for (int j = 0; j < 4; ++j) {
          oh4[j] = make_uint4(hi[4 * j], hi[4 * j + 1], hi[4 * j + 2], hi[4 * j + 3]);
          ol4[j] = make_uint4(lo[4 * j], lo[4 * j + 1], lo[4 * j + 2], lo[4 * j + 3]);
        }
      }
    }
  }
  if (a.ssq && valid && !a.pool) a.ssq[(long long)nt * a.ssq_stride + pix] = ssq_acc;
}

constexpr int TC_BM = 128;
constexpr int TC_BK = 64;
constexpr int TC_A_BYTES = TC_BM * TC_BK * 2;

constexpr int TC_HALO_W = 10, TC_HALO_H = 18;
constexpr int TC_HALO_ROWS = TC_HALO_W * TC_HALO_H;
constexpr int TC_HALO_PLANE = 23 * 1024;
constexpr int TC_HALO_STAGE = 2 * TC_HALO_PLANE;

template <int BN, int STAGES, bool HALO = false, int NA = 0>
struct ConvTcSmem {
  static constexpr int THREADS = HALO ? 384 : 160;
  static constexpr int CONSUMERS = HALO ? 2 : 1;
  static constexpr int B_BYTES = BN * TC_BK * 2;
  static constexpr int STAGE_BYTES = HALO ? 2 * B_BYTES : 2 * TC_A_BYTES + 2 * B_BYTES;
  static constexpr int A_RING = HALO ? NA * TC_HALO_STAGE : 0;
  static constexpr int STG = CONSUMERS * ACC_STG_BYTES;
  static constexpr int BYTES = A_RING + STAGES * STAGE_BYTES + STG + 1024  + 256 ;
};

template <int BN, int STAGES, bool HALO, int NA>
__global__ void __launch_bounds__(ConvTcSmem<BN, STAGES, HALO, NA>::THREADS, 1)
conv3x3_tc_kernel(const __grid_constant__ CUtensorMap tm_xhi, const __grid_constant__ CUtensorMap tm_xlo,
                  const __grid_constant__ CUtensorMap tm_whi, const __grid_constant__ CUtensorMap tm_wlo,
                  const ConvTcArgs a) {
  extern __shared__ __align__(1024) uint8_t smem_raw[];
  uint8_t* smem = reinterpret_cast<uint8_t*>((reinterpret_cast<uintptr_t>(smem_raw) + 1023) & ~uintptr_t(1023));
  using L = ConvTcSmem<BN, STAGES, HALO, NA>;
  constexpr int B_BYTES = L::B_BYTES;
  constexpr int STAGE_BYTES = L::STAGE_BYTES;
  constexpr int A_RING = L::A_RING;
  uint8_t* ring = smem + A_RING;
  float* stg = reinterpret_cast<float*>(ring + STAGES * STAGE_BYTES);
  uint64_t* bars = reinterpret_cast<uint64_t*>(ring + STAGES * STAGE_BYTES + L::STG);
  uint64_t* full_bar = bars;
  uint64_t* empty_bar = bars + STAGES;
  uint64_t* afull_bar = bars + 2 * STAGES;
  uint64_t* aempty_bar = afull_bar + NA;
  uint64_t* order_bar = aempty_bar + NA;

  const int warp = threadIdx.x >> 5, lane = threadIdx.x & 31;
  const int worker = (int)blockIdx.x;
  const int n_workers = (int)gridDim.x;
  const int producer_warp = HALO ? 0 : 4;
  if (warp == producer_warp && lane == 0) {
    tma_prefetch_desc(&tm_xhi);
    tma_prefetch_desc(&tm_xlo);
    tma_prefetch_desc(&tm_whi);
    tma_prefetch_desc(&tm_wlo);
    for (int i = 0; i < STAGES; ++i) {
      mbar_init(&full_bar[i], 1);
      mbar_init(&empty_bar[i], 4);
    }
    for (int i = 0; i < NA; ++i) {
      mbar_init(&afull_bar[i], 1);
      mbar_init(&aempty_bar[i], 4);
    }
    if (HALO) {
      mbar_init(&order_bar[0], 4);
      mbar_init(&order_bar[1], 4);
    }
    fence_barrier_init();
    fence_proxy_async();
  }
  __syncthreads();

  const int TW = 1 << a.tw_log2;
  const int kchunks = a.cin / TC_BK;
  const int kiters = 9 * kchunks;
  const int tiles_per_img = a.tiles_h * a.tiles_w;
  auto coords = [&](int tile, int& img, int& h0, int& w0, int& nt) {
    nt = tile % a.n_tiles;
    const int pt = tile / a.n_tiles;
    img = pt / tiles_per_img;
    const int rem = pt - img * tiles_per_img;
    h0 = (rem / a.tiles_w) * (TC_BM >> a.tw_log2);
    w0 = (rem % a.tiles_w) * TW;
  };

  if (HALO && warp < 4) setmaxnreg_dec<40>();
  if (warp == producer_warp) {
    const uint32_t smem_a = warp_uniform(smem_u32(smem));
    const uint32_t ring_a = smem_a + A_RING;
    const uint32_t bars_a = ring_a + STAGES * STAGE_BYTES + L::STG;
    const uint32_t full_a = bars_a, empty_a = bars_a + 8 * STAGES;
    const uint32_t afull_a = bars_a + 16 * STAGES, aempty_a = afull_a + 8 * NA;
    auto load_w = [&](uint32_t st, uint32_t fb, int c0, int n0, int tap) {
      tma_load_3d_a(st, &tm_whi, fb, c0, n0, tap);
      tma_load_3d_a(st + B_BYTES, &tm_wlo, fb, c0, n0, tap);
    };
    int stage = 0;
    uint32_t phase = 0;
    if constexpr (HALO) {
      auto try_wait_warp = [&](uint32_t bar, uint32_t parity) -> bool {
        uint32_t ok = 0;
        if (lane == 0) {
          asm volatile(
              "{\n\t"
              ".reg .pred p;\n\t"
              "mbarrier.try_wait.parity.shared::cta.b64 p, [%1], %2;\n\t"
              "selp.u32 %0, 1, 0, p;\n\t"
              "}"
              : "=r"(ok)
              : "r"(bar), "r"(parity)
              : "memory");
        }
        return warp_uniform(ok) != 0;
      };
      int astage = 0;
      uint32_t aphase = 0;
      int tA = worker, kcA = 0, tB = worker, kcB = 0, tapB = 0;
      while (tB < a.total_tiles) {
        const uint32_t as_u = warp_uniform((uint32_t)astage);
        if (tA < a.total_tiles && try_wait_warp(aempty_a + 8 * as_u, aphase ^ 1)) {
          int img, h0, w0, nt;
          coords(tA, img, h0, w0, nt);
          img = (int)warp_uniform((uint32_t)img); h0 = (int)warp_uniform((uint32_t)h0);
          w0 = (int)warp_uniform((uint32_t)w0);
          const int c0 = (int)warp_uniform((uint32_t)(kcA * TC_BK));
          const uint32_t sa = smem_a + as_u * TC_HALO_STAGE;
          constexpr uint32_t kHaloBytes = 2u * TC_HALO_ROWS * 128u;
          if (elect_one()) {
            mbar_arrive_expect_tx_a(afull_a + 8 * as_u, kHaloBytes);
            tma_load_4d_a(sa, &tm_xhi, afull_a + 8 * as_u, c0, w0 - 1, h0 - 1, img);
            tma_load_4d_a(sa + TC_HALO_PLANE, &tm_xlo, afull_a + 8 * as_u, c0, w0 - 1, h0 - 1, img);
          }
          __syncwarp();
          if (++astage == NA) { astage = 0; aphase ^= 1; }
          if (++kcA == kchunks) { kcA = 0; tA += n_workers; }
          continue;
        }
        const uint32_t st_u = warp_uniform((uint32_t)stage);
        if (try_wait_warp(empty_a + 8 * st_u, phase ^ 1)) {
          int img, h0, w0, nt;
          coords(tB, img, h0, w0, nt);
          const int n0 = (int)warp_uniform((uint32_t)(nt * BN));
          const int c0 = (int)warp_uniform((uint32_t)(kcB * TC_BK));
          const int tap = (int)warp_uniform((uint32_t)tapB);
          const uint32_t st = ring_a + st_u * STAGE_BYTES;
          if (elect_one()) {
            mbar_arrive_expect_tx_a(full_a + 8 * st_u, STAGE_BYTES);
            load_w(st, full_a + 8 * st_u, c0, n0, tap);
          }
          __syncwarp();
          if (++stage == STAGES) { stage = 0; phase ^= 1; }
          if (++tapB == 9) { tapB = 0; if (++kcB == kchunks) { kcB = 0; tB += n_workers; } }
        }
      }
    } else
    for (int tile = worker; tile < a.total_tiles; tile += n_workers) {
      int img, h0, w0, nt;
      coords(tile, img, h0, w0, nt);
      img = (int)warp_uniform((uint32_t)img); h0 = (int)warp_uniform((uint32_t)h0);
      w0 = (int)warp_uniform((uint32_t)w0);
      const int n0 = (int)warp_uniform((uint32_t)(nt * BN));
      for (int kit = 0; kit < kiters; ++kit) {
        const int tap = (int)warp_uniform((uint32_t)(kit / kchunks));
        const int c0 = (int)warp_uniform((uint32_t)((kit - tap * kchunks) * TC_BK));
        const int kh = tap / 3 - 1, kw = tap % 3 - 1;
        const uint32_t st_u = warp_uniform((uint32_t)stage);
        mbar_wait_warp_a(empty_a + 8 * st_u, phase ^ 1);
        const uint32_t st = smem_a + st_u * STAGE_BYTES;
        if (elect_one()) {
          const uint32_t fb = full_a + 8 * st_u;
          mbar_arrive_expect_tx_a(fb, STAGE_BYTES);
          tma_load_4d_a(st, &tm_xhi, fb, c0, w0 + kw, h0 + kh, img);
          tma_load_4d_a(st + TC_A_BYTES, &tm_xlo, fb, c0, w0 + kw, h0 + kh, img);
          load_w(st + 2 * TC_A_BYTES, fb, c0, n0, tap);
        }
        __syncwarp();
        if (++stage == STAGES) { stage = 0; phase ^= 1; }
      }
    }
  } else if (!HALO || warp >= 4) {
    const uint32_t smem_a = smem_u32(smem);
    const uint32_t ring_a = smem_a + A_RING;
    auto release_w = [&](int st) {
      if (lane == 0) mbar_arrive(&empty_bar[st]);
    };
    if constexpr (HALO) {
    setmaxnreg_inc<232>();
    const int cw = warp / 4 - 1;
    const int bar = 1 + cw;
    float* my_stg = stg + cw * (ACC_STG_BYTES / 4);
    const int m = threadIdx.x & 127;
    const int r = TW == 16 ? (m >> 3) & 7 : m >> 3;
    const int c = TW == 16 ? ((m >> 6) << 3) | (m & 7) : m & 7;
    const uint32_t halo_w = (uint32_t)TW + 2;
    const uint64_t halo_desc = ((uint64_t)1 << 16) | ((uint64_t)((halo_w * 128) >> 4) << 32) | ((uint64_t)1 << 62);
    const uint64_t a_half = (TW == 16 ? 8u : 8u * halo_w) * 128u / 16u;
    for (int i = cw; worker + i * n_workers < a.total_tiles; i += 2) {
      int img, h0, w0, nt;
      coords(worker + i * n_workers, img, h0, w0, nt);
      int astage = (i * kchunks) % NA, stage = (i * kiters) % STAGES;
      uint32_t aphase = (uint32_t)((i * kchunks) / NA) & 1u, phase = (uint32_t)((i * kiters) / STAGES) & 1u;
      if (i > 0) mbar_wait(&order_bar[cw], (uint32_t)((i - 1) >> 1) & 1u);
      Acc128<BN> acc;
      int prev = -1, prev_a = -1;
      for (int kc = 0; kc < kchunks; ++kc) {
        mbar_wait(&afull_bar[astage], aphase);
        const uint32_t ha = smem_a + astage * TC_HALO_STAGE;
        for (int tap = 0; tap < 9; ++tap) {
          mbar_wait(&full_bar[stage], phase);
          const uint32_t toff = ((uint32_t)(tap / 3) * halo_w + (uint32_t)(tap % 3)) * 128u;
          const uint64_t a_hi = halo_desc | (uint64_t)(((ha + toff) >> 4) & 0x3fffu);
          const uint64_t a_lo = halo_desc | (uint64_t)(((ha + TC_HALO_PLANE + toff) >> 4) & 0x3fffu);
          const uint32_t sb = ring_a + stage * STAGE_BYTES;
          const uint64_t b_hi = gmma_desc_kmajor_sw128(sb), b_lo = gmma_desc_kmajor_sw128(sb + B_BYTES);
          wgmma_fence();
#pragma unroll
          for (int k = 0; k < TC_BK / 16; ++k) {
            const uint64_t ko = (uint64_t)(k * 2);
            acc.mma(a_lo + ko, a_lo + a_half + ko, b_hi + ko, (kc > 0 || tap > 0 || k > 0) ? 1u : 0u);
            acc.mma(a_hi + ko, a_hi + a_half + ko, b_lo + ko, 1u);
            acc.mma(a_hi + ko, a_hi + a_half + ko, b_hi + ko, 1u);
          }
          wgmma_commit();
          if (kc == kchunks - 1 && tap == 8 && lane == 0) mbar_arrive(&order_bar[cw ^ 1]);
          wgmma_wait<1>();
          if (prev >= 0) release_w(prev);
          if (prev_a >= 0) {
            if (lane == 0) mbar_arrive(&aempty_bar[prev_a]);
            prev_a = -1;
          }
          prev = stage;
          if (++stage == STAGES) { stage = 0; phase ^= 1; }
        }
        prev_a = astage;
        if (++astage == NA) { astage = 0; aphase ^= 1; }
      }
      wgmma_wait<0>();
      acc.fence_operands();
      release_w(prev);
      if (lane == 0) mbar_arrive(&aempty_bar[prev_a]);
      conv_epilogue_tile<BN>(a, acc, my_stg, img, h0, w0, nt * BN, nt, r, c, 8, bar);
    }
    } else {
    const int m = threadIdx.x;
    const int r = m >> a.tw_log2, c = m & (TW - 1);
    int stage = 0;
    uint32_t phase = 0;
    for (int tile = worker; tile < a.total_tiles; tile += n_workers) {
      int img, h0, w0, nt;
      coords(tile, img, h0, w0, nt);
      Acc128<BN> acc;
      int prev = -1;
      for (int kit = 0; kit < kiters; ++kit) {
        mbar_wait(&full_bar[stage], phase);
        const uint32_t sa = ring_a + stage * STAGE_BYTES;
        const uint64_t a_hi = gmma_desc_kmajor_sw128(sa), a_lo = gmma_desc_kmajor_sw128(sa + TC_A_BYTES);
        const uint64_t b_hi = gmma_desc_kmajor_sw128(sa + 2 * TC_A_BYTES);
        const uint64_t b_lo = gmma_desc_kmajor_sw128(sa + 2 * TC_A_BYTES + B_BYTES);
        constexpr uint64_t kHalf = (TC_BM / 2) * 128 / 16;
        wgmma_fence();
#pragma unroll
        for (int k = 0; k < TC_BK / 16; ++k) {
          const uint64_t ko = (uint64_t)(k * 2);
          acc.mma(a_lo + ko, a_lo + kHalf + ko, b_hi + ko, (kit > 0 || k > 0) ? 1u : 0u);
          acc.mma(a_hi + ko, a_hi + kHalf + ko, b_lo + ko, 1u);
          acc.mma(a_hi + ko, a_hi + kHalf + ko, b_hi + ko, 1u);
        }
        wgmma_commit();
        wgmma_wait<1>();
        if (prev >= 0) release_w(prev);
        prev = stage;
        if (++stage == STAGES) { stage = 0; phase ^= 1; }
      }
      wgmma_wait<0>();
      acc.fence_operands();
      if (prev >= 0) release_w(prev);
      conv_epilogue_tile<BN>(a, acc, stg, img, h0, w0, nt * BN, nt, r, c, TW);
    }
    }
  }
  __syncthreads();
}

template <int BN, int STAGES, bool HALO = false, int NA = 0>
static int launch_tc_variant(const CUtensorMap& xhi, const CUtensorMap& xlo, const CUtensorMap& whi,
                             const CUtensorMap& wlo, const ConvTcArgs& a, cudaStream_t s) {
  constexpr int smem = ConvTcSmem<BN, STAGES, HALO, NA>::BYTES;
  static_assert(smem <= 232448, "shared-memory budget");
  static DeviceOnce attr_done;
  if (!attr_done.done()) {
    IBL_CUDA_OK(cudaFuncSetAttribute(conv3x3_tc_kernel<BN, STAGES, HALO, NA>, cudaFuncAttributeMaxDynamicSharedMemorySize, smem));
    attr_done.mark();
  }
  const int sms = device_sm_count();
  const int grid = a.total_tiles < sms ? a.total_tiles : sms;
  conv3x3_tc_kernel<BN, STAGES, HALO, NA><<<grid, ConvTcSmem<BN, STAGES, HALO, NA>::THREADS, smem, s>>>(xhi, xlo, whi, wlo, a);
  IBL_CUDA_OK(cudaGetLastError());
  return IBL_OK;
}

static int g_tc_bn_override = 0;
void tc_set_bn_override(int bn) { g_tc_bn_override = bn; }

int launch_conv3x3_tc(const __nv_bfloat16* x_hi, const __nv_bfloat16* x_lo, const ConvParams& p,
                      int N, int H, int W, int cin, int cout, bool relu, bool pool,
                      __nv_bfloat16* y_hi, __nv_bfloat16* y_lo, float* y_f32, cudaStream_t s, float* ssq,
                      int* ssq_parts) {
  IBL_REQUIRE(cin % 64 == 0 && cout % 64 == 0, "tensor-core conv needs Cin%64==0 and Cout%64==0");
  IBL_REQUIRE(p.w_hi && p.w_lo, "tensor-core conv: weights were not re-laid-out");
  IBL_REQUIRE(H >= 1 && W >= 1 && N >= 1, "empty conv input");
  ConvTcArgs a{};
  a.N = N; a.H = H; a.W = W; a.cin = cin; a.cout = cout;
  auto waste = [&](int tw) {
    int th = 128 / tw;
    return (long long)cdiv(W, tw) * tw * cdiv(H, th) * th;
  };
  a.tw_log2 = (waste(16) <= waste(8)) ? 4 : 3;
  const int TW = 1 << a.tw_log2, TH = 128 / TW;
  a.tiles_w = cdiv(W, TW);
  a.tiles_h = cdiv(H, TH);
  int bn = cout % 128 == 0 ? 128 : 64;
  if (g_tc_bn_override && cout % g_tc_bn_override == 0 && (g_tc_bn_override == 64 || g_tc_bn_override == 128))
    bn = g_tc_bn_override;
  const bool halo = bn == 128;
  a.n_tiles = cout / bn;
  a.total_tiles = (int)((long long)N * a.tiles_h * a.tiles_w * a.n_tiles);
  a.relu = relu; a.pool = pool;
  a.bias = p.bias; a.y_hi = y_hi; a.y_lo = y_lo; a.y_f32 = y_f32;
  a.ssq = pool ? nullptr : ssq;
  a.ssq_stride = (long long)N * H * W;
  if (ssq_parts) *ssq_parts = a.n_tiles;

  CUtensorMap m_xhi, m_xlo, m_whi, m_wlo;
  {
    uint64_t dims[4] = {(uint64_t)cin, (uint64_t)W, (uint64_t)H, (uint64_t)N};
    uint64_t str[3] = {(uint64_t)cin * 2, (uint64_t)W * cin * 2, (uint64_t)H * W * cin * 2};
    uint32_t box[4] = {64, (uint32_t)(halo ? TW + 2 : TW), (uint32_t)(halo ? TH + 2 : TH), 1};
    IBL_RET(make_tmap(&m_xhi, CU_TENSOR_MAP_DATA_TYPE_BFLOAT16, 4, x_hi, dims, str, box));
    IBL_RET(make_tmap(&m_xlo, CU_TENSOR_MAP_DATA_TYPE_BFLOAT16, 4, x_lo, dims, str, box));
  }
  {
    uint64_t dims[3] = {(uint64_t)cin, (uint64_t)cout, 9};
    uint64_t str[2] = {(uint64_t)cin * 2, (uint64_t)cout * cin * 2};
    uint32_t box[3] = {64, (uint32_t)bn, 1};
    IBL_RET(make_tmap(&m_whi, CU_TENSOR_MAP_DATA_TYPE_BFLOAT16, 3, p.w_hi, dims, str, box));
    IBL_RET(make_tmap(&m_wlo, CU_TENSOR_MAP_DATA_TYPE_BFLOAT16, 3, p.w_lo, dims, str, box));
  }
  if (halo) return launch_tc_variant<128, 3, true, 2>(m_xhi, m_xlo, m_whi, m_wlo, a, s);
  return launch_tc_variant<64, 4>(m_xhi, m_xlo, m_whi, m_wlo, a, s);
}

struct Conv1FusedArgs {
  const float* x;
  const float* w1;
  const float* bias1;
  ConvTcArgs c2;
};

constexpr int F1_A1_ROWS = 192;
constexpr int F1_A1_PLANE = F1_A1_ROWS * 64;
constexpr int F1_W1_PLANE = 64 * 64;
constexpr int F1_W2_STAGE = 2 * 64 * TC_BK * 2;
constexpr int F1_W2_STAGES = 4;
constexpr int F1_OFF_W1 = 2 * TC_HALO_STAGE;
constexpr int F1_OFF_W2 = F1_OFF_W1 + 2 * F1_W1_PLANE;
constexpr int F1_OFF_STG = F1_OFF_W2 + F1_W2_STAGES * F1_W2_STAGE;
constexpr int F1_OFF_BAR = F1_OFF_STG + 2 * ACC_STG_BYTES;
constexpr int F1_SMEM = F1_OFF_BAR + 512 + 1024;
static_assert(2 * F1_A1_PLANE <= TC_HALO_STAGE, "A1 (hi | lo) is built inside the consumer's halo buffer");
static_assert(TC_HALO_STAGE % 1024 == 0 && F1_OFF_W1 % 512 == 0 && F1_OFF_W2 % 1024 == 0, "swizzle atom alignment");
static_assert(F1_SMEM <= 232448, "shared-memory budget of the fused conv1 kernel");

__device__ __forceinline__ void wgmma_n64_into_n128(float (&d)[64], uint64_t a, uint64_t b) {
  asm volatile(
      "{\n\t.reg .pred p;\n\tsetp.ne.b32 p, 1, 0;\n\t"
      "wgmma.mma_async.sync.aligned.m64n64k16.f32.bf16.bf16 {%0, %1, %2, %3, %4, %5, %6, %7, %8, %9, %10, %11, %12, %13, %14, %15, %16, %17, %18, %19, %20, %21, %22, %23, %24, %25, %26, %27, %28, %29, %30, %31}, %32, %33, p, 1, 1, 0, 0;\n\t}"
      : "+f"(d[0]), "+f"(d[1]), "+f"(d[2]), "+f"(d[3]), "+f"(d[4]), "+f"(d[5]), "+f"(d[6]), "+f"(d[7]), "+f"(d[8]), "+f"(d[9]), "+f"(d[10]), "+f"(d[11]), "+f"(d[12]), "+f"(d[13]), "+f"(d[14]), "+f"(d[15]), "+f"(d[16]), "+f"(d[17]), "+f"(d[18]), "+f"(d[19]), "+f"(d[20]), "+f"(d[21]), "+f"(d[22]), "+f"(d[23]), "+f"(d[24]), "+f"(d[25]), "+f"(d[26]), "+f"(d[27]), "+f"(d[28]), "+f"(d[29]), "+f"(d[30]), "+f"(d[31])
      : "l"(a), "l"(b));
}

__global__ void __launch_bounds__(384, 1)
conv1_fused_tc_kernel(const __grid_constant__ CUtensorMap tm_whi, const __grid_constant__ CUtensorMap tm_wlo,
                      const Conv1FusedArgs fa) {
  extern __shared__ __align__(1024) uint8_t smem_raw[];
  uint8_t* smem = reinterpret_cast<uint8_t*>((reinterpret_cast<uintptr_t>(smem_raw) + 1023) & ~uintptr_t(1023));
  const ConvTcArgs& a = fa.c2;
  uint8_t* w1 = smem + F1_OFF_W1;
  uint8_t* w2 = smem + F1_OFF_W2;
  float* stg = reinterpret_cast<float*>(smem + F1_OFF_STG);
  uint64_t* bars = reinterpret_cast<uint64_t*>(smem + F1_OFF_BAR);
  uint64_t* w_full = bars;
  uint64_t* w_empty = bars + F1_W2_STAGES;
  uint64_t* order_bar = bars + 2 * F1_W2_STAGES;
  float* bias1_s = reinterpret_cast<float*>(bars + 16);

  const int warp = threadIdx.x >> 5, lane = threadIdx.x & 31;
  for (int i = threadIdx.x; i < 64 * 4; i += blockDim.x) {
    const int n = i >> 2, j = i & 3;
    uint32_t hi[4], lo[4];
#pragma unroll
    for (int e = 0; e < 4; ++e) {
      float v[2];
#pragma unroll
      for (int u = 0; u < 2; ++u) {
        const int k = j * 8 + e * 2 + u;
        v[u] = 0.f;
        if (k < 27) v[u] = fa.w1[(n * 3 + (k % 3)) * 9 + (k / 3)];
      }
      const __nv_bfloat16 h0 = __float2bfloat16_rn(v[0]), h1 = __float2bfloat16_rn(v[1]);
      __nv_bfloat162 hh(h0, h1);
      hi[e] = *reinterpret_cast<uint32_t*>(&hh);
      lo[e] = pack_bf16x2(v[0] - __bfloat162float(h0), v[1] - __bfloat162float(h1));
    }
    const int pos = n * 64 + ((j ^ ((n >> 1) & 3)) * 16);
    *reinterpret_cast<uint4*>(w1 + pos) = make_uint4(hi[0], hi[1], hi[2], hi[3]);
    *reinterpret_cast<uint4*>(w1 + F1_W1_PLANE + pos) = make_uint4(lo[0], lo[1], lo[2], lo[3]);
  }
  if (threadIdx.x < 64) bias1_s[threadIdx.x] = fa.bias1[threadIdx.x];
  if (threadIdx.x == 0) {
    tma_prefetch_desc(&tm_whi);
    tma_prefetch_desc(&tm_wlo);
    for (int i = 0; i < F1_W2_STAGES; ++i) { mbar_init(&w_full[i], 1); mbar_init(&w_empty[i], 4); }
    mbar_init(&order_bar[0], 4);
    mbar_init(&order_bar[1], 4);
    fence_barrier_init();
  }
  fence_proxy_async();
  __syncthreads();
  const int tiles_per_img = a.tiles_h * a.tiles_w;
  auto coords = [&](int tile, int& img, int& h0, int& w0) {
    img = tile / tiles_per_img;
    const int rem = tile - img * tiles_per_img;
    h0 = (rem / a.tiles_w) * 16;
    w0 = (rem % a.tiles_w) * 8;
  };

  if (warp < 4) setmaxnreg_dec<40>();
  if (warp == 0) {
    int stage = 0; uint32_t phase = 0;
    for (int tile = blockIdx.x; tile < a.total_tiles; tile += gridDim.x) {
      for (int tap = 0; tap < 9; ++tap) {
        mbar_wait_warp(&w_empty[stage], phase ^ 1);
        uint8_t* st = w2 + stage * F1_W2_STAGE;
        if (elect_one()) {
          mbar_arrive_expect_tx(&w_full[stage], F1_W2_STAGE);
          tma_load_3d(st, &tm_whi, &w_full[stage], 0, 0, tap);
          tma_load_3d(st + F1_W2_STAGE / 2, &tm_wlo, &w_full[stage], 0, 0, tap);
        }
        __syncwarp();
        if (++stage == F1_W2_STAGES) { stage = 0; phase ^= 1; }
      }
    }
  } else if (warp >= 4) {
    setmaxnreg_inc<232>();
    const int cw = warp / 4 - 1;
    const int bar = 1 + cw;
    float* my_stg = stg + cw * (ACC_STG_BYTES / 4);
    uint8_t* halo = smem + cw * TC_HALO_STAGE;
    const int t = threadIdx.x & 127;
    const int r = t >> 3, c = t & 7;
    const uint32_t ha = smem_u32(halo);
    const uint64_t b1h = gmma_desc_kmajor_sw64(smem_u32(w1)), b1l = gmma_desc_kmajor_sw64(smem_u32(w1) + F1_W1_PLANE);
    const uint64_t a1h = gmma_desc_kmajor_sw64(ha), a1l = gmma_desc_kmajor_sw64(ha + F1_A1_PLANE);
    constexpr uint64_t kA1Tile = 64 * 64 / 16;
    constexpr uint64_t kHaloDesc = ((uint64_t)1 << 16) | ((uint64_t)((TC_HALO_W * 128) >> 4) << 32) | ((uint64_t)1 << 62);
    constexpr uint64_t kHaloHalf = 8 * TC_HALO_W * 128 / 16;
    const long long HW = (long long)a.H * a.W;
    for (int i = cw; blockIdx.x + i * gridDim.x < a.total_tiles; i += 2) {
      int img, h0, w0;
      coords(blockIdx.x + i * gridDim.x, img, h0, w0);
      int tl = t;
      asm volatile("" : "+r"(tl));
#pragma unroll
      for (int q = 0; q < 2; ++q) {
        const int p = q * 128 + tl;
        if (p < F1_A1_ROWS) {
          float v[32];
#pragma unroll
          for (int k = 0; k < 32; ++k) v[k] = 0.f;
          const int hl = p / TC_HALO_W, wl = p - hl * TC_HALO_W;
          const int ph = h0 - 1 + hl, pw = w0 - 1 + wl;
          if (p < TC_HALO_ROWS && ph >= 0 && ph < a.H && pw >= 0 && pw < a.W && img < a.N) {
            const float* xb = fa.x + (long long)img * 3 * HW;
#pragma unroll
            for (int tap = 0; tap < 9; ++tap) {
              const int ih = ph + tap / 3 - 1, iw = pw + tap % 3 - 1;
              if (ih >= 0 && ih < a.H && iw >= 0 && iw < a.W) {
                const long long o = (long long)ih * a.W + iw;
#pragma unroll
                for (int ci = 0; ci < 3; ++ci) v[tap * 3 + ci] = __ldg(xb + ci * HW + o);
              }
            }
          }
          uint8_t* rh = halo + p * 64;
#pragma unroll
          for (int j = 0; j < 4; ++j) {
            uint32_t hi[4], lo[4];
#pragma unroll
            for (int e = 0; e < 4; ++e) {
              const float x0 = v[8 * j + 2 * e], x1 = v[8 * j + 2 * e + 1];
              const __nv_bfloat16 h0b = __float2bfloat16_rn(x0), h1b = __float2bfloat16_rn(x1);
              __nv_bfloat162 hv(h0b, h1b);
              hi[e] = *reinterpret_cast<uint32_t*>(&hv);
              lo[e] = pack_bf16x2(x0 - __bfloat162float(h0b), x1 - __bfloat162float(h1b));
            }
            const int pos = (j ^ ((p >> 1) & 3)) * 16;
            *reinterpret_cast<uint4*>(rh + pos) = make_uint4(hi[0], hi[1], hi[2], hi[3]);
            *reinterpret_cast<uint4*>(rh + F1_A1_PLANE + pos) = make_uint4(lo[0], lo[1], lo[2], lo[3]);
          }
        }
      }
      fence_proxy_async();
      wg_sync(bar);
      float c1[3][32];
      wgmma_fence();
#pragma unroll
      for (int k = 0; k < 2; ++k) {
        const uint64_t ko = (uint64_t)(k * 2);
#pragma unroll
        for (int f = 0; f < 3; ++f) {
          const uint64_t fo = f * kA1Tile + ko;
          Wgmma<64, false, 0, 0>::mma(c1[f], a1l + fo, b1h + ko, k > 0 ? 1u : 0u);
          Wgmma<64, false, 0, 0>::mma(c1[f], a1h + fo, b1l + ko, 1u);
          Wgmma<64, false, 0, 0>::mma(c1[f], a1h + fo, b1h + ko, 1u);
        }
      }
      wgmma_commit();
      wgmma_wait<0>();
#pragma unroll
      for (int f = 0; f < 3; ++f)
#pragma unroll
        for (int j = 0; j < 32; ++j) asm volatile("" : "+f"(c1[f][j])::"memory");
      wg_sync(bar);
#pragma unroll
      for (int f = 0; f < 3; ++f) {
#pragma unroll
        for (int hf = 0; hf < 2; ++hf) {
          const int p = 64 * f + (tl & ~31) / 2 + ((tl & 31) >> 2) + 8 * hf;
          if (p < TC_HALO_ROWS) {
            const int hl = p / TC_HALO_W, wl = p - hl * TC_HALO_W;
            const int ph = h0 - 1 + hl, pw = w0 - 1 + wl;
            const bool inside = ph >= 0 && ph < a.H && pw >= 0 && pw < a.W && img < a.N;
            uint8_t* rh = halo + p * 128 + (tl & 3) * 4;
#pragma unroll
            for (int j = 0; j < 8; ++j) {
              const int ch = 8 * j + 2 * (tl & 3);
              float x0 = fmaxf(c1[f][4 * j + 2 * hf] + bias1_s[ch], 0.f);
              float x1 = fmaxf(c1[f][4 * j + 2 * hf + 1] + bias1_s[ch + 1], 0.f);
              if (!inside) { x0 = 0.f; x1 = 0.f; }
              const __nv_bfloat16 h0b = __float2bfloat16_rn(x0), h1b = __float2bfloat16_rn(x1);
              __nv_bfloat162 hv(h0b, h1b);
              const int pos = (j ^ (p & 7)) * 16;
              *reinterpret_cast<uint32_t*>(rh + pos) = *reinterpret_cast<uint32_t*>(&hv);
              *reinterpret_cast<uint32_t*>(rh + TC_HALO_PLANE + pos) =
                  pack_bf16x2(x0 - __bfloat162float(h0b), x1 - __bfloat162float(h1b));
            }
          }
        }
      }
      fence_proxy_async();
      wg_sync(bar);
      int stage = (i * 9) % F1_W2_STAGES;
      uint32_t phase = (uint32_t)((i * 9) / F1_W2_STAGES) & 1u;
      if (i > 0) mbar_wait(&order_bar[cw], (uint32_t)((i - 1) >> 1) & 1u);
      float d[2][64];
#pragma unroll
      for (int hm = 0; hm < 2; ++hm)
#pragma unroll
        for (int j = 0; j < 64; ++j) d[hm][j] = 0.f;
      int prev = -1;
      for (int tap = 0; tap < 9; ++tap) {
        mbar_wait(&w_full[stage], phase);
        const uint32_t toff = (uint32_t)((tap / 3) * TC_HALO_W + tap % 3) * 128u;
        const uint64_t a_hi = kHaloDesc | (uint64_t)(((ha + toff) >> 4) & 0x3fffu);
        const uint64_t a_lo = kHaloDesc | (uint64_t)(((ha + TC_HALO_PLANE + toff) >> 4) & 0x3fffu);
        const uint64_t b_w = gmma_desc_kmajor_sw128(smem_u32(w2 + stage * F1_W2_STAGE));
        wgmma_fence();
#pragma unroll
        for (int k = 0; k < TC_BK / 16; ++k) {
          const uint64_t ko = (uint64_t)(k * 2);
#pragma unroll
          for (int hm = 0; hm < 2; ++hm) {
            const uint64_t ho = hm ? kHaloHalf : 0;
            Wgmma<128, false, 0, 0>::mma(d[hm], a_hi + ho + ko, b_w + ko, (tap > 0 || k > 0) ? 1u : 0u);
            wgmma_n64_into_n128(d[hm], a_lo + ho + ko, b_w + ko);
          }
        }
        wgmma_commit();
        if (tap == 8 && lane == 0) mbar_arrive(&order_bar[cw ^ 1]);
        wgmma_wait<1>();
        if (prev >= 0 && lane == 0) mbar_arrive(&w_empty[prev]);
        prev = stage;
        if (++stage == F1_W2_STAGES) { stage = 0; phase ^= 1; }
      }
      wgmma_wait<0>();
#pragma unroll
      for (int hm = 0; hm < 2; ++hm)
#pragma unroll
        for (int j = 0; j < 64; ++j) asm volatile("" : "+f"(d[hm][j])::"memory");
      if (lane == 0) mbar_arrive(&w_empty[prev]);
      Acc128<64> acc;
#pragma unroll
      for (int hm = 0; hm < 2; ++hm)
#pragma unroll
        for (int j = 0; j < 32; ++j) acc.h[hm][j] = d[hm][j] + d[hm][32 + j];
      conv_epilogue_tile<64>(a, acc, my_stg, img, h0, w0, 0, 0, r, c, 8, bar);
    }
  }
  __syncthreads();
}

int launch_conv1_fused_tc(const float* x_nchw, const float* w1_oihw, const float* bias1, const ConvParams& p2, int N, int H,
                          int W, __nv_bfloat16* y_hi, __nv_bfloat16* y_lo, cudaStream_t s) {
  IBL_REQUIRE(p2.w_hi && p2.w_lo && p2.bias, "fused conv1: conv1_2 weights were not re-laid-out");
  Conv1FusedArgs fa{};
  fa.x = x_nchw; fa.w1 = w1_oihw; fa.bias1 = bias1;
  ConvTcArgs& a = fa.c2;
  a.N = N; a.H = H; a.W = W; a.cin = 64; a.cout = 64;
  a.tw_log2 = 3;
  a.tiles_w = cdiv(W, 8);
  a.tiles_h = cdiv(H, 16);
  a.n_tiles = 1;
  a.total_tiles = (int)((long long)N * a.tiles_h * a.tiles_w);
  a.relu = 1; a.pool = 1;
  a.bias = p2.bias; a.y_hi = y_hi; a.y_lo = y_lo; a.y_f32 = nullptr; a.ssq = nullptr; a.ssq_stride = 0;
  CUtensorMap m_whi, m_wlo;
  {
    uint64_t dims[3] = {64, 64, 9};
    uint64_t str[2] = {64 * 2, 64 * 64 * 2};
    uint32_t box[3] = {64, 64, 1};
    IBL_RET(make_tmap(&m_whi, CU_TENSOR_MAP_DATA_TYPE_BFLOAT16, 3, p2.w_hi, dims, str, box));
    IBL_RET(make_tmap(&m_wlo, CU_TENSOR_MAP_DATA_TYPE_BFLOAT16, 3, p2.w_lo, dims, str, box));
  }
  static DeviceOnce attr_done;
  if (!attr_done.done()) {
    IBL_CUDA_OK(cudaFuncSetAttribute(conv1_fused_tc_kernel, cudaFuncAttributeMaxDynamicSharedMemorySize, F1_SMEM));
    attr_done.mark();
  }
  const int sms = device_sm_count();
  const int grid = a.total_tiles < sms ? a.total_tiles : sms;
  conv1_fused_tc_kernel<<<grid, 384, F1_SMEM, s>>>(m_whi, m_wlo, fa);
  IBL_CUDA_OK(cudaGetLastError());
  return IBL_OK;
}

__global__ void maxpool2x2_planes_kernel(const __nv_bfloat16* __restrict__ hi,
                                         const __nv_bfloat16* __restrict__ lo, int N, int H, int W,
                                         int C, __nv_bfloat16* __restrict__ yhi,
                                         __nv_bfloat16* __restrict__ ylo) {
  const int OH = H / 2, OW = W / 2;
// ... 44 lines not shown
```

### openibl_b200/csrc/tc_probe.cu

```cuda
#include "common.cuh"
#include "tc_common.cuh"

namespace ibl {

using namespace tc;

__device__ __forceinline__ uint64_t probe_desc(uint32_t a_addr, uint32_t sbo, int base_mode) {
  uint64_t d = 0;
  d |= (uint64_t)((a_addr >> 4) & 0x3fffu);
  d |= (uint64_t)1 << 16;
  d |= (uint64_t)((sbo >> 4) & 0x3fffu) << 32;
  if (base_mode == 1) d |= (uint64_t)((a_addr >> 7) & 7u) << 49;
  d |= (uint64_t)1 << 62;
  return d;
}

__global__ void __launch_bounds__(128, 1)
gmma_strided_probe_kernel(const __grid_constant__ CUtensorMap tm_a, const __grid_constant__ CUtensorMap tm_b,
                          int rows, int s0, int group_rows, int half_rows, int base_mode, float* __restrict__ D) {
  extern __shared__ __align__(1024) uint8_t smem_raw[];
  uint8_t* smem = reinterpret_cast<uint8_t*>((reinterpret_cast<uintptr_t>(smem_raw) + 1023) & ~uintptr_t(1023));
  uint8_t* a_sm = smem;
  uint8_t* b_sm = smem + 32768;
  float* stg = reinterpret_cast<float*>(smem + 32768 + 8192);
  uint64_t* bars = reinterpret_cast<uint64_t*>(smem + 32768 + 8192 + ACC_STG_BYTES);
  if (threadIdx.x == 0) {
    mbar_init(&bars[0], 1);
    fence_barrier_init();
    fence_proxy_async();
  }
  __syncthreads();
  if (threadIdx.x == 0) {
    mbar_arrive_expect_tx(&bars[0], rows * 128 + 8192);
    tma_load_2d(a_sm, &tm_a, &bars[0], 0, 0);
    tma_load_2d(b_sm, &tm_b, &bars[0], 0, 0);
  }
  mbar_wait(&bars[0], 0);
  const uint32_t sbo = (uint32_t)group_rows * 128u;
  const uint32_t a0 = smem_u32(a_sm) + (uint32_t)s0 * 128u;
  const uint32_t a1 = a0 + (uint32_t)half_rows * 128u;
  const uint64_t da0 = probe_desc(a0, sbo, base_mode), da1 = probe_desc(a1, sbo, base_mode);
  const uint64_t db = gmma_desc_kmajor_sw128(smem_u32(b_sm));
  Acc128<64> acc;
  wgmma_fence();
#pragma unroll
  for (int k = 0; k < 4; ++k)
    acc.mma(da0 + (uint64_t)(k * 2), da1 + (uint64_t)(k * 2), db + (uint64_t)(k * 2), k > 0 ? 1u : 0u);
  wgmma_commit();
  wgmma_wait<0>();
  acc.fence_operands();
  float* o = D + (size_t)threadIdx.x * 64;
#pragma unroll
  for (int ch = 0; ch < 2; ++ch) {
    uint32_t r[32];
    acc.rows32(ch, stg, r);
#pragma unroll
    for (int j = 0; j < 32; ++j) o[ch * 32 + j] = __uint_as_float(r[j]);
  }
}

int debug_gmma_strided(const void* A, int rows, const void* B, int s0, int group_rows, int half_rows, int base_mode,
                       float* D, cudaStream_t s) {
  IBL_REQUIRE(rows >= 8 && rows <= 256 && s0 >= 0 && group_rows >= 8 && half_rows >= 0 &&
                  s0 + half_rows + 7 * group_rows + 8 <= rows,
              "probe view does not fit the halo tile");
  CUtensorMap ma, mb;
  {
    uint64_t dims[2] = {64, (uint64_t)rows};
    uint64_t str[1] = {128};
    uint32_t box[2] = {64, (uint32_t)rows};
    IBL_RET(make_tmap(&ma, CU_TENSOR_MAP_DATA_TYPE_BFLOAT16, 2, A, dims, str, box));
  }
  {
    uint64_t dims[2] = {64, 64};
    uint64_t str[1] = {128};
    uint32_t box[2] = {64, 64};
    IBL_RET(make_tmap(&mb, CU_TENSOR_MAP_DATA_TYPE_BFLOAT16, 2, B, dims, str, box));
  }
  const int smem = 32768 + 8192 + ACC_STG_BYTES + 1024 + 64;
  static DeviceOnce attr_done;
  if (!attr_done.done()) {
    IBL_CUDA_OK(cudaFuncSetAttribute(gmma_strided_probe_kernel, cudaFuncAttributeMaxDynamicSharedMemorySize, smem));
    attr_done.mark();
  }
  gmma_strided_probe_kernel<<<1, 128, smem, s>>>(ma, mb, rows, s0, group_rows, half_rows, base_mode, D);
  IBL_CUDA_OK(cudaGetLastError());
  return IBL_OK;
}

}
```

### openibl_b200/csrc/wgmma.cuh

```cuda
#pragma once
#include <stdint.h>

namespace ibl {
namespace tc {

template <int N, bool F16, int TA, int TB> struct Wgmma;

template <> struct Wgmma<32, false, 0, 0> {
  static __device__ __forceinline__ void mma(float (&d)[16], uint64_t a, uint64_t b, uint32_t accumulate) {
    asm volatile(
        "{\n\t.reg .pred p;\n\tsetp.ne.b32 p, %18, 0;\n\t"
        "wgmma.mma_async.sync.aligned.m64n32k16.f32.bf16.bf16 {%0, %1, %2, %3, %4, %5, %6, %7, %8, %9, %10, %11, %12, %13, %14, %15}, %16, %17, p, 1, 1, 0, 0;\n\t}"
        : "+f"(d[0]), "+f"(d[1]), "+f"(d[2]), "+f"(d[3]), "+f"(d[4]), "+f"(d[5]), "+f"(d[6]), "+f"(d[7]), "+f"(d[8]), "+f"(d[9]), "+f"(d[10]), "+f"(d[11]), "+f"(d[12]), "+f"(d[13]), "+f"(d[14]), "+f"(d[15])
        : "l"(a), "l"(b), "r"(accumulate));
  }
};

template <> struct Wgmma<64, false, 0, 0> {
  static __device__ __forceinline__ void mma(float (&d)[32], uint64_t a, uint64_t b, uint32_t accumulate) {
    asm volatile(
        "{\n\t.reg .pred p;\n\tsetp.ne.b32 p, %34, 0;\n\t"
        "wgmma.mma_async.sync.aligned.m64n64k16.f32.bf16.bf16 {%0, %1, %2, %3, %4, %5, %6, %7, %8, %9, %10, %11, %12, %13, %14, %15, %16, %17, %18, %19, %20, %21, %22, %23, %24, %25, %26, %27, %28, %29, %30, %31}, %32, %33, p, 1, 1, 0, 0;\n\t}"
        : "+f"(d[0]), "+f"(d[1]), "+f"(d[2]), "+f"(d[3]), "+f"(d[4]), "+f"(d[5]), "+f"(d[6]), "+f"(d[7]), "+f"(d[8]), "+f"(d[9]), "+f"(d[10]), "+f"(d[11]), "+f"(d[12]), "+f"(d[13]), "+f"(d[14]), "+f"(d[15]), "+f"(d[16]), "+f"(d[17]), "+f"(d[18]), "+f"(d[19]), "+f"(d[20]), "+f"(d[21]), "+f"(d[22]), "+f"(d[23]), "+f"(d[24]), "+f"(d[25]), "+f"(d[26]), "+f"(d[27]), "+f"(d[28]), "+f"(d[29]), "+f"(d[30]), "+f"(d[31])
        : "l"(a), "l"(b), "r"(accumulate));
  }
};

template <> struct Wgmma<128, false, 0, 0> {
  static __device__ __forceinline__ void mma(float (&d)[64], uint64_t a, uint64_t b, uint32_t accumulate) {
    asm volatile(
        "{\n\t.reg .pred p;\n\tsetp.ne.b32 p, %66, 0;\n\t"
        "wgmma.mma_async.sync.aligned.m64n128k16.f32.bf16.bf16 {%0, %1, %2, %3, %4, %5, %6, %7, %8, %9, %10, %11, %12, %13, %14, %15, %16, %17, %18, %19, %20, %21, %22, %23, %24, %25, %26, %27, %28, %29, %30, %31, %32, %33, %34, %35, %36, %37, %38, %39, %40, %41, %42, %43, %44, %45, %46, %47, %48, %49, %50, %51, %52, %53, %54, %55, %56, %57, %58, %59, %60, %61, %62, %63}, %64, %65, p, 1, 1, 0, 0;\n\t}"
        : "+f"(d[0]), "+f"(d[1]), "+f"(d[2]), "+f"(d[3]), "+f"(d[4]), "+f"(d[5]), "+f"(d[6]), "+f"(d[7]), "+f"(d[8]), "+f"(d[9]), "+f"(d[10]), "+f"(d[11]), "+f"(d[12]), "+f"(d[13]), "+f"(d[14]), "+f"(d[15]), "+f"(d[16]), "+f"(d[17]), "+f"(d[18]), "+f"(d[19]), "+f"(d[20]), "+f"(d[21]), "+f"(d[22]), "+f"(d[23]), "+f"(d[24]), "+f"(d[25]), "+f"(d[26]), "+f"(d[27]), "+f"(d[28]), "+f"(d[29]), "+f"(d[30]), "+f"(d[31]), "+f"(d[32]), "+f"(d[33]), "+f"(d[34]), "+f"(d[35]), "+f"(d[36]), "+f"(d[37]), "+f"(d[38]), "+f"(d[39]), "+f"(d[40]), "+f"(d[41]), "+f"(d[42]), "+f"(d[43]), "+f"(d[44]), "+f"(d[45]), "+f"(d[46]), "+f"(d[47]), "+f"(d[48]), "+f"(d[49]), "+f"(d[50]), "+f"(d[51]), "+f"(d[52]), "+f"(d[53]), "+f"(d[54]), "+f"(d[55]), "+f"(d[56]), "+f"(d[57]), "+f"(d[58]), "+f"(d[59]), "+f"(d[60]), "+f"(d[61]), "+f"(d[62]), "+f"(d[63])
        : "l"(a), "l"(b), "r"(accumulate));
  }
};

template <> struct Wgmma<64, false, 1, 1> {
  static __device__ __forceinline__ void mma(float (&d)[32], uint64_t a, uint64_t b, uint32_t accumulate) {
    asm volatile(
        "{\n\t.reg .pred p;\n\tsetp.ne.b32 p, %34, 0;\n\t"
        "wgmma.mma_async.sync.aligned.m64n64k16.f32.bf16.bf16 {%0, %1, %2, %3, %4, %5, %6, %7, %8, %9, %10, %11, %12, %13, %14, %15, %16, %17, %18, %19, %20, %21, %22, %23, %24, %25, %26, %27, %28, %29, %30, %31}, %32, %33, p, 1, 1, 1, 1;\n\t}"
        : "+f"(d[0]), "+f"(d[1]), "+f"(d[2]), "+f"(d[3]), "+f"(d[4]), "+f"(d[5]), "+f"(d[6]), "+f"(d[7]), "+f"(d[8]), "+f"(d[9]), "+f"(d[10]), "+f"(d[11]), "+f"(d[12]), "+f"(d[13]), "+f"(d[14]), "+f"(d[15]), "+f"(d[16]), "+f"(d[17]), "+f"(d[18]), "+f"(d[19]), "+f"(d[20]), "+f"(d[21]), "+f"(d[22]), "+f"(d[23]), "+f"(d[24]), "+f"(d[25]), "+f"(d[26]), "+f"(d[27]), "+f"(d[28]), "+f"(d[29]), "+f"(d[30]), "+f"(d[31])
        : "l"(a), "l"(b), "r"(accumulate));
  }
};

template <> struct Wgmma<128, false, 1, 1> {
  static __device__ __forceinline__ void mma(float (&d)[64], uint64_t a, uint64_t b, uint32_t accumulate) {
    asm volatile(
        "{\n\t.reg .pred p;\n\tsetp.ne.b32 p, %66, 0;\n\t"
        "wgmma.mma_async.sync.aligned.m64n128k16.f32.bf16.bf16 {%0, %1, %2, %3, %4, %5, %6, %7, %8, %9, %10, %11, %12, %13, %14, %15, %16, %17, %18, %19, %20, %21, %22, %23, %24, %25, %26, %27, %28, %29, %30, %31, %32, %33, %34, %35, %36, %37, %38, %39, %40, %41, %42, %43, %44, %45, %46, %47, %48, %49, %50, %51, %52, %53, %54, %55, %56, %57, %58, %59, %60, %61, %62, %63}, %64, %65, p, 1, 1, 1, 1;\n\t}"
        : "+f"(d[0]), "+f"(d[1]), "+f"(d[2]), "+f"(d[3]), "+f"(d[4]), "+f"(d[5]), "+f"(d[6]), "+f"(d[7]), "+f"(d[8]), "+f"(d[9]), "+f"(d[10]), "+f"(d[11]), "+f"(d[12]), "+f"(d[13]), "+f"(d[14]), "+f"(d[15]), "+f"(d[16]), "+f"(d[17]), "+f"(d[18]), "+f"(d[19]), "+f"(d[20]), "+f"(d[21]), "+f"(d[22]), "+f"(d[23]), "+f"(d[24]), "+f"(d[25]), "+f"(d[26]), "+f"(d[27]), "+f"(d[28]), "+f"(d[29]), "+f"(d[30]), "+f"(d[31]), "+f"(d[32]), "+f"(d[33]), "+f"(d[34]), "+f"(d[35]), "+f"(d[36]), "+f"(d[37]), "+f"(d[38]), "+f"(d[39]), "+f"(d[40]), "+f"(d[41]), "+f"(d[42]), "+f"(d[43]), "+f"(d[44]), "+f"(d[45]), "+f"(d[46]), "+f"(d[47]), "+f"(d[48]), "+f"(d[49]), "+f"(d[50]), "+f"(d[51]), "+f"(d[52]), "+f"(d[53]), "+f"(d[54]), "+f"(d[55]), "+f"(d[56]), "+f"(d[57]), "+f"(d[58]), "+f"(d[59]), "+f"(d[60]), "+f"(d[61]), "+f"(d[62]), "+f"(d[63])
        : "l"(a), "l"(b), "r"(accumulate));
  }
};

template <> struct Wgmma<128, true, 0, 0> {
  static __device__ __forceinline__ void mma(float (&d)[64], uint64_t a, uint64_t b, uint32_t accumulate) {
    asm volatile(
        "{\n\t.reg .pred p;\n\tsetp.ne.b32 p, %66, 0;\n\t"
        "wgmma.mma_async.sync.aligned.m64n128k16.f32.f16.f16 {%0, %1, %2, %3, %4, %5, %6, %7, %8, %9, %10, %11, %12, %13, %14, %15, %16, %17, %18, %19, %20, %21, %22, %23, %24, %25, %26, %27, %28, %29, %30, %31, %32, %33, %34, %35, %36, %37, %38, %39, %40, %41, %42, %43, %44, %45, %46, %47, %48, %49, %50, %51, %52, %53, %54, %55, %56, %57, %58, %59, %60, %61, %62, %63}, %64, %65, p, 1, 1, 0, 0;\n\t}"
        : "+f"(d[0]), "+f"(d[1]), "+f"(d[2]), "+f"(d[3]), "+f"(d[4]), "+f"(d[5]), "+f"(d[6]), "+f"(d[7]), "+f"(d[8]), "+f"(d[9]), "+f"(d[10]), "+f"(d[11]), "+f"(d[12]), "+f"(d[13]), "+f"(d[14]), "+f"(d[15]), "+f"(d[16]), "+f"(d[17]), "+f"(d[18]), "+f"(d[19]), "+f"(d[20]), "+f"(d[21]), "+f"(d[22]), "+f"(d[23]), "+f"(d[24]), "+f"(d[25]), "+f"(d[26]), "+f"(d[27]), "+f"(d[28]), "+f"(d[29]), "+f"(d[30]), "+f"(d[31]), "+f"(d[32]), "+f"(d[33]), "+f"(d[34]), "+f"(d[35]), "+f"(d[36]), "+f"(d[37]), "+f"(d[38]), "+f"(d[39]), "+f"(d[40]), "+f"(d[41]), "+f"(d[42]), "+f"(d[43]), "+f"(d[44]), "+f"(d[45]), "+f"(d[46]), "+f"(d[47]), "+f"(d[48]), "+f"(d[49]), "+f"(d[50]), "+f"(d[51]), "+f"(d[52]), "+f"(d[53]), "+f"(d[54]), "+f"(d[55]), "+f"(d[56]), "+f"(d[57]), "+f"(d[58]), "+f"(d[59]), "+f"(d[60]), "+f"(d[61]), "+f"(d[62]), "+f"(d[63])
        : "l"(a), "l"(b), "r"(accumulate));
  }
};

}
}
```

### openibl_b200/engine.py

```python
from __future__ import annotations

import ctypes
import threading
from ctypes import byref, c_double, c_float, c_int, c_uint64, c_void_p
from typing import Optional, Sequence

import torch

from . import _cabi
from ._cabi import CONV_SIMT_FP32, CONV_TC_BF16X3, OUT_PCA, OUT_POOL, OUT_VLAD, check

_engines = {}
_engines_lock = threading.Lock()


def invalidate_caches() -> None:
    with _engines_lock:
        engines = list(_engines.values())
    for eng in engines:
        eng.invalidate()


def _require_cuda(t: torch.Tensor, name: str, dtype=torch.float32) -> torch.Tensor:
    if not isinstance(t, torch.Tensor):
# ... 326 lines not shown
        ptrs = (ctypes.c_char_p * n)(*[bytes(f) for f in files])
        lens = (ctypes.c_size_t * n)(*[len(f) for f in files])
        status = (c_int * n)()
        check(self.lib.ibl_jpeg_decode_u8(self.h, ptrs, lens, n, _ptr(out), offsets, status, _ptr(err),
                                          _stream(self.device)), "ibl_jpeg_decode_u8")
        for name, sub in (("ibl_jpeg_decode_progressive_u8", prog), ("ibl_png_decode_u8", png)):
            if not sub:
                continue
            idx = sorted(sub)
            m = len(idx)
            s_status = (c_int * m)()
            s_err = torch.empty(m, dtype=torch.int32, device=dev)
            check(getattr(self.lib, name)(
                self.h, (ctypes.c_char_p * m)(*[bytes(files[i]) for i in idx]),
                (ctypes.c_size_t * m)(*[len(files[i]) for i in idx]),
                m, _ptr(out), (c_uint64 * m)(*[offsets[i] for i in idx]), s_status, _ptr(s_err), _stream(self.device)),
                name)
            err[idx] = s_err
            for j, i in enumerate(idx):
                status[i] = s_status[j]
        imgs = []
        for i, inf in enumerate(infos):
            inf = device.get(i, inf)
            if i in host:
                im = out[offsets[i]: offsets[i] + host[i].size].view(host[i].shape)
                im.copy_(torch.from_numpy(host[i]))
                imgs.append(im)
            elif status[i] != _cabi.IBL_OK:
                imgs.append(None)
            else:
                h, w = inf["height"], inf["width"]
                imgs.append(out[offsets[i]: offsets[i] + h * w * 3].view(h, w, 3))
        return imgs, err

    def decode_jpeg(self, files: Sequence[bytes]):
        imgs, err = self.decode_jpeg_async(files)
        bad = torch.nonzero(err).flatten().tolist()
        if bad:
            png = [i for i in bad if bytes(files[i][:8]) == _cabi.PNG_SIGNATURE]
            jpeg = [i for i in bad if i not in png]
            what = ([f"corrupt JPEG entropy data in file(s) {jpeg}"] if jpeg else []) + \
                   ([f"corrupt PNG image data in file(s) {png}"] if png else [])
            raise RuntimeError(" and ".join(what) + " of the batch")
        return imgs

    def color_jitter_u8(self, images: Sequence[torch.Tensor], params: Sequence) -> None:
        n = len(images)
        if n != len(params):
            raise ValueError(f"{n} images but {len(params)} parameter sets")
        if n == 0:
            return
        ims = []
        for i, im in enumerate(images):
            _require_cuda(im, f"images[{i}]", dtype=torch.uint8)
            if im.dim() != 3 or im.shape[2] != 3 or not im.is_contiguous() or im.numel() == 0:
                raise ValueError(f"images[{i}] must be a non-empty contiguous uint8 [H,W,3] tensor, got {tuple(im.shape)}")
            ims.append(im)
        nan = float("nan")
        p = (_cabi.ColorJitterParams * n)()
        for i, (order, b, c, s, h) in enumerate(params):
            p[i].order[:] = [int(k) for k in order]
            p[i].brightness, p[i].contrast, p[i].saturation, p[i].hue = [nan if v is None else float(v)
                                                                          for v in (b, c, s, h)]
        if any(im.device.index != self.device for im in ims):
            raise ValueError(f"images must be on cuda:{self.device}, the engine's device")
        base = ims[0].untyped_storage().data_ptr()
        if any(im.untyped_storage().data_ptr() != base for im in ims):
            raise ValueError("images must be views into one device buffer (decode_jpeg_async(..., fallback=...))")
        sizes = [im.numel() for im in ims]
        offs = [im.data_ptr() - base for im in ims]
        spans = sorted(zip(offs, sizes))
        if any(o0 + s0 > o1 for (o0, s0), (o1, _) in zip(spans, spans[1:])):
            raise ValueError("images overlap in memory")
        buf = c_void_p(base)
        off_a = (c_uint64 * n)(*offs)
        h_a = (c_int * n)(*[im.shape[0] for im in ims])
        w_a = (c_int * n)(*[im.shape[1] for im in ims])
        check(self.lib.ibl_color_jitter_u8(self.h, buf, off_a, h_a, w_a, p, n, _stream(self.device)),
              "ibl_color_jitter_u8")

    def argsort_rows(self, dist: torch.Tensor) -> torch.Tensor:
        dist = _require_cuda(dist, "distance matrix")
        m, n = dist.shape
        out = torch.empty(m, n, dtype=torch.int64, device=dist.device)
        check(self.lib.ibl_argsort_rows(self.h, _ptr(dist), m, n, _ptr(out), _stream(self.device)), "ibl_argsort_rows")
        return out

    def extract_host_u8(self, x_u8_host: torch.Tensor, out_host: torch.Tensor, mean, std, pca=False,
                        pool_host: Optional[torch.Tensor] = None) -> torch.Tensor:
        assert not x_u8_host.is_cuda and not out_host.is_cuda and x_u8_host.is_contiguous() and out_host.is_contiguous()
        assert x_u8_host.dtype == torch.uint8 and out_host.dtype == torch.float32
        N, H, W, C = x_u8_host.shape
        assert C == 3
        flags = OUT_VLAD | (OUT_PCA if pca else 0) | (OUT_POOL if pool_host is not None else 0)
        m, s = self._norm_consts(mean, std)
        check(self.lib.ibl_extract_host_u8(self.h, _ptr(x_u8_host), N, H, W, m, s, flags, _ptr(out_host),
                                           _ptr(pool_host), _stream(self.device)), "ibl_extract_host_u8")
        return out_host

    def l2dist_dense(self, q: torch.Tensor, db: torch.Tensor) -> torch.Tensor:
        q = _require_cuda(q, "queries")
        db = _require_cuda(db, "database")
        m, d = q.shape
        n = db.shape[0]
        out = torch.empty(m, n, device=q.device)
        check(self.lib.ibl_l2dist_dense(self.h, _ptr(q), m, _ptr(db), n, d, _ptr(out), _stream(self.device)),
              "ibl_l2dist_dense")
        return out

    def l2dist_self(self, x: torch.Tensor) -> torch.Tensor:
        x = _require_cuda(x, "features")
        n, d = x.shape
        out = torch.empty(n, n, device=x.device)
        check(self.lib.ibl_l2dist_self(self.h, _ptr(x), n, d, _ptr(out), _stream(self.device)), "ibl_l2dist_self")
        return out

    def l2dist_topk(self, q: torch.Tensor, db: torch.Tensor, k: int, idx_base: int = 0,
                    n_valid: Optional[int] = None):
        q = _require_cuda(q, "queries")
        db = _require_cuda(db, "database")
        m, d = q.shape
        n = db.shape[0]
        if n_valid is None:
            n_valid = n
        od = torch.empty(m, k, device=q.device)
        oi = torch.empty(m, k, device=q.device, dtype=torch.int64)
        check(self.lib.ibl_l2dist_topk(self.h, _ptr(q), m, _ptr(db), n, int(n_valid), d, int(k), int(idx_base),
                                       _ptr(od), _ptr(oi), _stream(self.device)), "ibl_l2dist_topk")
        return od, oi

    def topk_rows(self, dist: torch.Tensor, k: int):
        dist = _require_cuda(dist, "distance matrix")
        m, n = dist.shape
        od = torch.empty(m, k, device=dist.device)
        oi = torch.empty(m, k, device=dist.device, dtype=torch.int64)
        check(self.lib.ibl_topk_rows(self.h, _ptr(dist), m, n, int(k), _ptr(od), _ptr(oi), _stream(self.device)),
              "ibl_topk_rows")
        return od, oi

    def topk_merge(self, cand_dist: torch.Tensor, cand_idx: torch.Tensor, k_out: int):
        cand_dist = _require_cuda(cand_dist, "candidate distances")
        cand_idx = _require_cuda(cand_idx, "candidate indices", torch.int64)
        parts, m, k_in = cand_dist.shape
        od = torch.empty(m, k_out, device=cand_dist.device)
        oi = torch.empty(m, k_out, device=cand_dist.device, dtype=torch.int64)
        check(self.lib.ibl_topk_merge(self.h, _ptr(cand_dist), _ptr(cand_idx), parts, m, k_in, int(k_out),
                                      _ptr(od), _ptr(oi), _stream(self.device)), "ibl_topk_merge")
        return od, oi

    def knn_rowmax(self, x: torch.Tensor, w: int, row0: int = 0, n_rows: Optional[int] = None):
        x = _require_cuda(x, "descriptors")
        N, d = x.shape
        if n_rows is None:
            n_rows = N - row0
        oi = torch.empty(n_rows, w, dtype=torch.int64, device=x.device)
        od = torch.empty(n_rows, w, device=x.device)
        om = torch.empty(n_rows, device=x.device)
        check(self.lib.ibl_knn_rowmax(self.h, _ptr(x), N, d, int(row0), int(n_rows), int(w), _ptr(oi), _ptr(od),
                                      _ptr(om), _stream(self.device)), "ibl_knn_rowmax")
        return oi, od, om

    def rerank_topk(self, x: torch.Tensor, m: int, nbr_idx: torch.Tensor, nbr_dist: torch.Tensor,
                    rowmax: torch.Tensor, k1: int, k2: int, lambda_value: float, k: int,
                    orig_idx: Optional[torch.Tensor] = None):
        x = _require_cuda(x, "descriptors")
        nbr_idx = _require_cuda(nbr_idx, "neighbour lists", torch.int64)
        nbr_dist = _require_cuda(nbr_dist, "neighbour distances")
        rowmax = _require_cuda(rowmax, "row maxima")
        N, d = x.shape
        w = nbr_idx.shape[1]
        k_orig = 0
        if orig_idx is not None:
            orig_idx = _require_cuda(orig_idx, "original ranking", torch.int64)
            k_orig = orig_idx.shape[1]
        od = torch.empty(m, k, device=x.device)
        oi = torch.empty(m, k, dtype=torch.int64, device=x.device)
        check(self.lib.ibl_rerank_topk(self.h, _ptr(x), N, int(m), d, _ptr(nbr_idx), _ptr(nbr_dist), int(w),
                                       _ptr(rowmax), int(k1), int(k2), c_float(lambda_value), _ptr(orig_idx),
                                       int(k_orig), int(k), _ptr(od), _ptr(oi), _stream(self.device)),
              "ibl_rerank_topk")
        return od, oi

    def rerank_dense(self, qg: torch.Tensor, qq: torch.Tensor, gg: torch.Tensor, k1: int = 20, k2: int = 6,
                     lambda_value: float = 0.3) -> torch.Tensor:
        qg = _require_cuda(qg, "query-gallery distances")
        qq = _require_cuda(qq, "query-query distances")
        gg = _require_cuda(gg, "gallery-gallery distances")
        m, n = qg.shape
        if tuple(qq.shape) != (m, m) or tuple(gg.shape) != (n, n):
            raise ValueError(f"re_ranking: shapes qg {tuple(qg.shape)}, qq {tuple(qq.shape)}, gg {tuple(gg.shape)} "
                             "do not fit together")
        if m + n < k1 + 1:
            raise ValueError("re_ranking needs at least k1 + 1 images")
        out = torch.empty(m, n, device=qg.device)
        check(self.lib.ibl_rerank_dense(self.h, _ptr(qg), _ptr(qq), _ptr(gg), m, n, int(k1), int(k2),
                                        c_double(lambda_value), _ptr(out), _stream(self.device)), "ibl_rerank_dense")
        return out

    def knn_flagged(self) -> int:
        c = c_int()
        check(self.lib.ibl_debug_knn_flagged(self.h, byref(c), _stream(self.device)), "ibl_debug_knn_flagged")
        return c.value

    def rerank_workspace_bytes(self) -> int:
        c = c_uint64()
        check(self.lib.ibl_debug_rerank_workspace_bytes(self.h, byref(c)), "ibl_debug_rerank_workspace_bytes")
        return c.value

    def l2dist_topk_host(self, q_host: torch.Tensor, db_host: torch.Tensor, k: int,
                         out_dist_host: torch.Tensor, out_idx_host: torch.Tensor):
        m, d = q_host.shape
        n = db_host.shape[0]
        check(self.lib.ibl_l2dist_topk_host(self.h, _ptr(q_host), m, _ptr(db_host), n, d, int(k),
                                            _ptr(out_dist_host), _ptr(out_idx_host), _stream(self.device)),
              "ibl_l2dist_topk_host")
        return out_dist_host, out_idx_host

    def dist_flagged(self) -> int:
        c = c_int()
        check(self.lib.ibl_debug_dist_flagged(self.h, byref(c), _stream(self.device)), "ibl_debug_dist_flagged")
        return c.value

    def dist_path(self) -> int:
        c = c_int()
        check(self.lib.ibl_debug_dist_path(self.h, byref(c)), "ibl_debug_dist_path")
        return c.value

    def gemm_nt(self, a: torch.Tensor, b: torch.Tensor, alpha: float = 1.0, mode: int = CONV_SIMT_FP32) -> torch.Tensor:
        a = _require_cuda(a, "A")
        b = _require_cuda(b, "B")
        m, k = a.shape
        n = b.shape[0]
        if b.shape[1] != k:
            raise ValueError("gemm_nt: inner dimensions differ")
        pad = (-k) % 64
        if pad:
            a = torch.nn.functional.pad(a, (0, pad))
            b = torch.nn.functional.pad(b, (0, pad))
        out = torch.empty(m, n, device=a.device)
        rows = max(1, min(m, (2 ** 31 - 1) // max(n, 1)))
        for r0 in range(0, m, rows):
            r1 = min(m, r0 + rows)
            check(self.lib.ibl_gemm_nt(self.h, _ptr(a[r0:r1]), r1 - r0, _ptr(b), n, k + pad, c_float(alpha), _ptr(out[r0:r1]),
                                       int(mode), _stream(self.device)), "ibl_gemm_nt")
        return out

    def vgg16_prefix_forward(self, x: torch.Tensor, n_layers: int) -> torch.Tensor:
        from .synth import VGG16_PLAN
        x = _require_cuda(x, "input images")
        N, _, H, W = x.shape
        h, w, c, seen = H, W, 3, 0
        for item in VGG16_PLAN:
            if item == "P":
                h, w = h // 2, w // 2
            else:
                if seen == n_layers:
                    break
                c = item[2]
                seen += 1
        out = torch.empty(N, h, w, c, device=x.device)
        check(self.lib.ibl_vgg16_prefix_forward(self.h, _ptr(x), N, H, W, int(n_layers), _ptr(out), _stream(self.device)),
              "ibl_vgg16_prefix_forward")
        return out

    def vgg16_layer_forward(self, layer: int, x: torch.Tensor, cout: int) -> torch.Tensor:
        x = _require_cuda(x, "layer input")
        if layer == 0:
            N, _, H, W = x.shape
        else:
            N, H, W, _ = x.shape
        y = torch.empty(N, H, W, cout, device=x.device)
        check(self.lib.ibl_vgg16_layer_forward(self.h, int(layer), _ptr(x), N, H, W, _ptr(y), _stream(self.device)),
              "ibl_vgg16_layer_forward")
        return y

    def vgg16_layer_backward(self, layer: int, x: torch.Tensor, y: Optional[torch.Tensor], gy: torch.Tensor,
                             w_shape, need_gx: bool):
        x = _require_cuda(x, "layer input")
        gy = _require_cuda(gy, "grad output")
        N, H, W, cout = gy.shape
        gx = torch.empty_like(x) if need_gx else None
        gw = torch.empty(w_shape, device=x.device)
        gb = torch.empty(cout, device=x.device)
        check(self.lib.ibl_vgg16_layer_backward(self.h, int(layer), _ptr(x), _ptr(y), _ptr(gy), N, H, W, _ptr(gx), _ptr(gw),
                                                _ptr(gb), _stream(self.device)), "ibl_vgg16_layer_backward")
        return gx, gw, gb

    def maxpool2x2(self, x: torch.Tensor) -> torch.Tensor:
        x = _require_cuda(x, "pool input")
        N, H, W, C = x.shape
        y = torch.empty(N, H // 2, W // 2, C, device=x.device)
        check(self.lib.ibl_maxpool2x2_forward(self.h, _ptr(x), N, H, W, C, _ptr(y), _stream(self.device)), "ibl_maxpool2x2_forward")
        return y

    def maxpool2x2_backward(self, x: torch.Tensor, gy: torch.Tensor) -> torch.Tensor:
        x = _require_cuda(x, "pool input")
        gy = _require_cuda(gy, "pool grad")
        N, H, W, C = x.shape
        gx = torch.empty_like(x)
        check(self.lib.ibl_maxpool2x2_backward(self.h, _ptr(x), _ptr(gy), N, H, W, C, _ptr(gx), _stream(self.device)),
              "ibl_maxpool2x2_backward")
        return gx

    def debug_conv3x3(self, x_nhwc, w_oihw, bias, relu=True, pool=False, mode=CONV_TC_BF16X3, bn=0):
        x = _require_cuda(x_nhwc, "x")
        w = _require_cuda(w_oihw, "w")
        b = _require_cuda(bias, "bias")
        N, H, W, cin = x.shape
        cout = w.shape[0]
        oh, ow = (H // 2, W // 2) if pool else (H, W)
        y = torch.empty(N, oh, ow, cout, device=x.device)
        check(self.lib.ibl_debug_conv3x3(self.h, _ptr(x), N, H, W, cin, _ptr(w), _ptr(b), cout, int(relu),
                                         int(pool), int(mode), int(bn), _ptr(y), _stream(self.device)),
              "ibl_debug_conv3x3")
        return y

    def debug_conv1_fused(self, x_nchw):
        x = _require_cuda(x_nchw, "x")
        N, C, H, W = x.shape
        if C != 3:
            raise ValueError(f"conv1 input must have 3 channels, got {C}")
        hi = torch.empty(N, H // 2, W // 2, 64, dtype=torch.bfloat16, device=x.device)
        lo = torch.empty_like(hi)
        check(self.lib.ibl_debug_conv1_fused(self.h, _ptr(x), N, H, W, _ptr(hi), _ptr(lo), _stream(self.device)),
              "ibl_debug_conv1_fused")
        return hi, lo
```

Baseline: 1192.

## Add wide 16x16-pixel conv3x3 tile variant using register-A wgmma over halo

Adds a conv3x3 kernel variant where weights are loaded into registers via ldmatrix and used as the wgmma A operand, while the activation halo tile (256 pixels, 16x16 patch) is the shared-memory B operand. The accumulator is held transposed and redistributed with shuffles in a new epilogue that handles bias, ReLU, pooling, the bf16 hi/lo split and the sum-of-squares output. The aim is more reuse per halo load and no staging buffer for accumulators, at the cost of a larger halo ring and heavier register pressure. The variant is picked by a launch heuristic or a debug override, and the ssq workspace is sized by cout/16.

Result: faster. 1244 (median of 6 runs) (+4.3%).

```diff
diff --git a/include/iblb200.h b/include/iblb200.h
--- a/include/iblb200.h
+++ b/include/iblb200.h
@@ -176,6 +176,9 @@
                            int base_mode, float* D, void* stream);
 int ibl_debug_umma_halo_view(ibl_engine* e, const void* A, int rows, const void* B, int s0, int group_rows,
                              int half_rows, float* D, void* stream);
+int ibl_debug_wgmma_rs_halo_view(ibl_engine* e, const void* W, const void* X, int pitch, int hrows, int n, int s0,
+                                 float* D, void* stream);
+int ibl_debug_set_conv3x3_variant(ibl_engine* e, int variant);
 int ibl_debug_conv1_fused(ibl_engine* e, const float* x, int N, int H, int W, void* y_hi, void* y_lo, void* stream);
 int ibl_debug_time_layer(ibl_engine* e, int layer, const float* x, int N, int H, int W, int bn_override,
                          int reps, float* ms_out);
diff --git a/openibl_b200/_cabi.py b/openibl_b200/_cabi.py
--- a/openibl_b200/_cabi.py
+++ b/openibl_b200/_cabi.py
@@ -97,6 +97,8 @@
     "ibl_debug_gemm_tn": (c_int, [_P, _P, _P, _P, _P]),
     "ibl_debug_umma_strided": (c_int, [_P, _P, c_int, _P, c_int, c_int, c_int, _P, _P]),
     "ibl_debug_umma_halo_view": (c_int, [_P, _P, c_int, _P, c_int, c_int, c_int, _P, _P]),
+    "ibl_debug_wgmma_rs_halo_view": (c_int, [_P, _P, _P, c_int, c_int, c_int, c_int, _P, _P]),
+    "ibl_debug_set_conv3x3_variant": (c_int, [_P, c_int]),
     "ibl_debug_conv1_fused": (c_int, [_P, _P, c_int, c_int, c_int, _P, _P, _P]),
     "ibl_debug_time_layer": (c_int, [_P, c_int, _P, c_int, c_int, c_int, c_int, c_int, POINTER(c_float)]),
     "ibl_debug_conv3x3": (c_int, [_P, _P, c_int, c_int, c_int, c_int, _P, _P, c_int, c_int, c_int, c_int,
diff --git a/openibl_b200/csrc/common.cuh b/openibl_b200/csrc/common.cuh
--- a/openibl_b200/csrc/common.cuh
+++ b/openibl_b200/csrc/common.cuh
@@ -150,6 +150,7 @@
                       __nv_bfloat16* y_hi, __nv_bfloat16* y_lo, cudaStream_t s);
 int debug_gmma_strided(const void* A, int rows, const void* B, int s0, int group_rows, int half_rows, int base_mode,
                        float* D, cudaStream_t s);
+int debug_wgmma_rs_halo(const void* W, const void* X, int pitch, int hrows, int n, int s0, float* D, cudaStream_t s);
 int debug_gemm_tn(const float* A, const float* B, float* C, cudaStream_t s);
 int netvlad_tc_units(int B, int S);
 int launch_netvlad_tc(const __nv_bfloat16* x_hi, const __nv_bfloat16* x_lo, int B, int S, int K,
diff --git a/openibl_b200/csrc/engine.cu b/openibl_b200/csrc/engine.cu
--- a/openibl_b200/csrc/engine.cu
+++ b/openibl_b200/csrc/engine.cu
@@ -11,6 +11,7 @@
 static thread_local std::string g_last_error;
 void set_last_error(const std::string& s) { g_last_error = s; }
 void tc_set_bn_override(int bn);
+void tc_set_variant_override(int v);
 
 static const ConvLayer kVgg16[13] = {
     {3, 64, true, false},    {64, 64, true, true},
@@ -176,7 +177,7 @@
     const int oh = L.pool ? h / 2 : h, ow = L.pool ? w / 2 : w;
     const size_t out_elems = (size_t)N * oh * ow * L.cout;
     if (last && planes_out) {
-      IBL_RET(e->ssq.ensure((size_t)8 * N * oh * ow * sizeof(float)));
+      IBL_RET(e->ssq.ensure((size_t)(L.cout / 16) * N * oh * ow * sizeof(float)));
       IBL_RET(launch_conv3x3_tc(hi_of(cur, in_elems), lo_of(cur, in_elems), e->conv[l], N, h, w, L.cin,
                                 L.cout, L.relu, L.pool, hi_of(cur ^ 1, out_elems), lo_of(cur ^ 1, out_elems),
                                 nullptr, s, e->ssq.as<float>(), &planes_out->ssq_parts));
@@ -1266,6 +1267,20 @@
   return debug_gmma_strided(A, rows, B, s0, group_rows, half_rows, 0, D, S(stream));
 }
 
+int ibl_debug_wgmma_rs_halo_view(ibl_engine* e, const void* W, const void* X, int pitch, int hrows, int n, int s0,
+                                 float* D, void* stream) {
+  IBL_REQUIRE(e && W && X && D, "null argument");
+  DeviceGuard g(e->device);
+  e->launches += 1;
+  return debug_wgmma_rs_halo(W, X, pitch, hrows, n, s0, D, S(stream));
+}
+
+int ibl_debug_set_conv3x3_variant(ibl_engine* e, int variant) {
+  IBL_REQUIRE(e && variant >= 0 && variant <= 2, "bad argument");
+  tc_set_variant_override(variant);
+  return IBL_OK;
+}
+
 int ibl_debug_conv1_fused(ibl_engine* e, const float* x, int N, int H, int W, void* y_hi, void* y_lo, void* stream) {
   IBL_REQUIRE(e && x && y_hi && y_lo && N >= 1 && H >= 2 && W >= 2, "bad argument");
   if (!e->vgg_ready) { set_last_error("ibl_engine_set_vgg16 was not called"); return IBL_ERR_NOT_READY; }
diff --git a/openibl_b200/csrc/tc_common.cuh b/openibl_b200/csrc/tc_common.cuh
--- a/openibl_b200/csrc/tc_common.cuh
+++ b/openibl_b200/csrc/tc_common.cuh
@@ -202,6 +202,15 @@
   return d;
 }
 
+__device__ __forceinline__ void ldsm_a_sw128(uint32_t (&r)[4], uint32_t tile, int row, int k16) {
+  const uint32_t chunk = (uint32_t)(2 * k16 + ((threadIdx.x >> 4) & 1)) ^ (uint32_t)(row & 7);
+  const uint32_t addr = tile + (uint32_t)row * 128u + (chunk << 4);
+  asm volatile("ldmatrix.sync.aligned.m8n8.x4.shared.b16 {%0, %1, %2, %3}, [%4];"
+               : "=r"(r[0]), "=r"(r[1]), "=r"(r[2]), "=r"(r[3])
+               : "r"(addr)
+               : "memory");
+}
+
 __device__ __forceinline__ void wgmma_fence() { asm volatile("wgmma.fence.sync.aligned;" ::: "memory"); }
 __device__ __forceinline__ void wgmma_commit() { asm volatile("wgmma.commit_group.sync.aligned;" ::: "memory"); }
 template <int N>
diff --git a/openibl_b200/csrc/tc_conv.cu b/openibl_b200/csrc/tc_conv.cu
--- a/openibl_b200/csrc/tc_conv.cu
+++ b/openibl_b200/csrc/tc_conv.cu
@@ -191,25 +191,148 @@
 constexpr int TC_HALO_PLANE = 23 * 1024;
 constexpr int TC_HALO_STAGE = 2 * TC_HALO_PLANE;
 
-template <int BN, int STAGES, bool HALO = false, int NA = 0>
+constexpr int TC_WIDE_PX = 256;
+constexpr int TC_WIDE_HALO_PLANE = 41 * 1024;
+
+template <int BN, int STAGES, bool HALO = false, int NA = 0, int WTW = 0>
 struct ConvTcSmem {
   static constexpr int THREADS = HALO ? 384 : 160;
   static constexpr int CONSUMERS = HALO ? 2 : 1;
   static constexpr int B_BYTES = BN * TC_BK * 2;
   static constexpr int STAGE_BYTES = HALO ? 2 * B_BYTES : 2 * TC_A_BYTES + 2 * B_BYTES;
-  static constexpr int A_RING = HALO ? NA * TC_HALO_STAGE : 0;
-  static constexpr int STG = CONSUMERS * ACC_STG_BYTES;
+  static constexpr int HALO_PLANE = WTW ? TC_WIDE_HALO_PLANE : TC_HALO_PLANE;
+  static constexpr int A_RING = HALO ? NA * 2 * HALO_PLANE : 0;
+  static constexpr int STG = WTW ? 0 : CONSUMERS * ACC_STG_BYTES;
   static constexpr int BYTES = A_RING + STAGES * STAGE_BYTES + STG + 1024  + 256 ;
 };
 
-template <int BN, int STAGES, bool HALO, int NA>
-__global__ void __launch_bounds__(ConvTcSmem<BN, STAGES, HALO, NA>::THREADS, 1)
+struct AccWide {
+  float d[2][64];
+};
+
+__device__ __forceinline__ float wide_pick(bool swap, float a, float b) { return swap ? b : a; }
+
+__device__ __forceinline__ void wide_transpose4(uint32_t (&x)[4][2], int j) {
+#pragma unroll
+  for (int bit = 0; bit < 2; ++bit) {
+    const bool mine = ((j >> bit) & 1) != 0;
+#pragma unroll
+    for (int p0 = 0; p0 < 4; ++p0) {
+      if (p0 & (1 << bit)) continue;
+      const int p1 = p0 | (1 << bit);
+#pragma unroll
+      for (int h = 0; h < 2; ++h) {
+        const uint32_t got = __shfl_xor_sync(0xffffffffu, mine ? x[p0][h] : x[p1][h], 4 << bit);
+        if (mine) x[p0][h] = got; else x[p1][h] = got;
+      }
+    }
+  }
+}
+
+__device__ __forceinline__ void conv_wide_epilogue(const ConvTcArgs& a, const AccWide& acc, int img, int h0, int w0,
+                                                   int nt) {
+  constexpr int NV = 2, TH = 16;
+  const int t = threadIdx.x & 127, w = t >> 5, lane = t & 31, g = lane >> 2, q = lane & 3, j = g & 3;
+  const bool sw = (g >> 2) != 0;
+  const int c = nt * 64 + 16 * w + 2 * g;
+  const int cst = nt * 64 + 16 * w + 8 * (g >> 2);
+  const float b0 = __ldg(a.bias + c), b1 = __ldg(a.bias + c + 1);
+  auto activate = [&](float& v0, float& v1) {
+    v0 += b0; v1 += b1;
+    if (a.relu) { v0 = fmaxf(v0, 0.f); v1 = fmaxf(v1, 0.f); }
+  };
+  auto pack = [&](float v0, float v1, uint32_t (&x)[2]) {
+    if (a.y_f32) {
+      x[0] = __float_as_uint(v0); x[1] = __float_as_uint(v1);
+    } else {
+      const __nv_bfloat16 h0b = __float2bfloat16_rn(v0), h1b = __float2bfloat16_rn(v1);
+      __nv_bfloat162 hh(h0b, h1b);
+      x[0] = *reinterpret_cast<uint32_t*>(&hh);
+      x[1] = pack_bf16x2(v0 - __bfloat162float(h0b), v1 - __bfloat162float(h1b));
+    }
+  };
+  auto store = [&](const uint32_t (&x)[4][2], bool valid, long long pix) {
+    if (!valid) return;
+    const long long off = pix * a.cout + cst;
+    if (a.y_f32) {
+      float4* o = reinterpret_cast<float4*>(a.y_f32 + off);
+      o[0] = make_float4(__uint_as_float(x[0][0]), __uint_as_float(x[0][1]), __uint_as_float(x[1][0]), __uint_as_float(x[1][1]));
+      o[1] = make_float4(__uint_as_float(x[2][0]), __uint_as_float(x[2][1]), __uint_as_float(x[3][0]), __uint_as_float(x[3][1]));
+    } else {
+      *reinterpret_cast<uint4*>(a.y_hi + off) = make_uint4(x[0][0], x[1][0], x[2][0], x[3][0]);
+      *reinterpret_cast<uint4*>(a.y_lo + off) = make_uint4(x[0][1], x[1][1], x[2][1], x[3][1]);
+    }
+  };
+  if (a.pool) {
+    const int OH = a.H >> 1, OW = a.W >> 1;
+    const int ow = (w0 >> 1) + q;
+#pragma unroll
+    for (int v = 0; v < NV; ++v)
+#pragma unroll
+      for (int m = 0; m < TH / 8; ++m) {
+        uint32_t x[4][2];
+#pragma unroll
+        for (int p = 0; p < 4; ++p) {
+          const float* r0 = &acc.d[v][4 * (2 * (4 * m + p))];
+          const float* r1 = r0 + 4;
+          const float e0 = fmaxf(fmaxf(r0[0], r0[1]), fmaxf(r1[0], r1[1]));
+          const float e1 = fmaxf(fmaxf(r0[2], r0[3]), fmaxf(r1[2], r1[3]));
+          float v0 = wide_pick(sw, e0, e1), v1 = wide_pick(sw, e1, e0);
+          activate(v0, v1);
+          pack(v0, v1, x[p]);
+        }
+        wide_transpose4(x, j);
+        const int oh = (h0 >> 1) + 4 * m + j, owv = ow + 4 * v;
+        store(x, oh < OH && owv < OW && img < a.N, ((long long)img * OH + oh) * OW + owv);
+      }
+    return;
+  }
+#pragma unroll
+  for (int v = 0; v < NV; ++v)
+#pragma unroll
+    for (int b = 0; b < TH / 2; ++b) {
+      uint32_t x[4][2];
+      float sq[4];
+#pragma unroll
+      for (int p = 0; p < 4; ++p) {
+        const float* r = &acc.d[v][4 * (2 * b + (p >> 1)) + (p & 1)];
+        const float e0 = r[0], e1 = r[2];
+        float v0 = wide_pick(sw, e0, e1), v1 = wide_pick(sw, e1, e0);
+        activate(v0, v1);
+        sq[p] = fmaf(v1, v1, v0 * v0);
+        pack(v0, v1, x[p]);
+      }
+      wide_transpose4(x, j);
+      const int h = h0 + 2 * b + (j >> 1), wc = w0 + 8 * v + 2 * q + (j & 1);
+      const bool valid = h < a.H && wc < a.W && img < a.N;
+      const long long pix = ((long long)img * a.H + h) * a.W + wc;
+      store(x, valid, pix);
+      if (a.ssq) {
+        float mine = 0.f;
+#pragma unroll
+        for (int p = 0; p < 4; ++p) {
+          float s2 = sq[p];
+          s2 += __shfl_xor_sync(0xffffffffu, s2, 4);
+          s2 += __shfl_xor_sync(0xffffffffu, s2, 8);
+          s2 += __shfl_xor_sync(0xffffffffu, s2, 16);
+          if (p == j) mine = s2;
+        }
+        if (valid && g < 4) a.ssq[(long long)(nt * 4 + w) * a.ssq_stride + pix] = mine;
+      }
+    }
+}
+
+template <int BN, int STAGES, bool HALO, int NA, int WTW = 0>
+__global__ void __launch_bounds__(ConvTcSmem<BN, STAGES, HALO, NA, WTW>::THREADS, 1)
 conv3x3_tc_kernel(const __grid_constant__ CUtensorMap tm_xhi, const __grid_constant__ CUtensorMap tm_xlo,
                   const __grid_constant__ CUtensorMap tm_whi, const __grid_constant__ CUtensorMap tm_wlo,
                   const ConvTcArgs a) {
   extern __shared__ __align__(1024) uint8_t smem_raw[];
   uint8_t* smem = reinterpret_cast<uint8_t*>((reinterpret_cast<uintptr_t>(smem_raw) + 1023) & ~uintptr_t(1023));
-  using L = ConvTcSmem<BN, STAGES, HALO, NA>;
+  using L = ConvTcSmem<BN, STAGES, HALO, NA, WTW>;
+  constexpr int HALO_PLANE = L::HALO_PLANE;
+  constexpr int HALO_STAGE = 2 * HALO_PLANE;
+  constexpr int PX = WTW ? TC_WIDE_PX : TC_BM;
   constexpr int B_BYTES = L::B_BYTES;
   constexpr int STAGE_BYTES = L::STAGE_BYTES;
   constexpr int A_RING = L::A_RING;
@@ -257,7 +380,7 @@
     const int pt = tile / a.n_tiles;
     img = pt / tiles_per_img;
     const int rem = pt - img * tiles_per_img;
-    h0 = (rem / a.tiles_w) * (TC_BM >> a.tw_log2);
+    h0 = (rem / a.tiles_w) * (PX >> a.tw_log2);
     w0 = (rem % a.tiles_w) * TW;
   };
 
@@ -301,12 +424,12 @@
           img = (int)warp_uniform((uint32_t)img); h0 = (int)warp_uniform((uint32_t)h0);
           w0 = (int)warp_uniform((uint32_t)w0);
           const int c0 = (int)warp_uniform((uint32_t)(kcA * TC_BK));
-          const uint32_t sa = smem_a + as_u * TC_HALO_STAGE;
-          constexpr uint32_t kHaloBytes = 2u * TC_HALO_ROWS * 128u;
+          const uint32_t sa = smem_a + as_u * HALO_STAGE;
+          constexpr uint32_t kHaloBytes = WTW ? 2u * (WTW + 2) * (TC_WIDE_PX / WTW + 2) * 128u : 2u * TC_HALO_ROWS * 128u;
           if (elect_one()) {
             mbar_arrive_expect_tx_a(afull_a + 8 * as_u, kHaloBytes);
             tma_load_4d_a(sa, &tm_xhi, afull_a + 8 * as_u, c0, w0 - 1, h0 - 1, img);
-            tma_load_4d_a(sa + TC_HALO_PLANE, &tm_xlo, afull_a + 8 * as_u, c0, w0 - 1, h0 - 1, img);
+            tma_load_4d_a(sa + HALO_PLANE, &tm_xlo, afull_a + 8 * as_u, c0, w0 - 1, h0 - 1, img);
           }
           __syncwarp();
           if (++astage == NA) { astage = 0; aphase ^= 1; }
@@ -361,7 +484,81 @@
     auto release_w = [&](int st) {
       if (lane == 0) mbar_arrive(&empty_bar[st]);
     };
-    if constexpr (HALO) {
+    if constexpr (WTW != 0) {
+    setmaxnreg_inc<232>();
+    static_assert(WTW == 16, "the wide tiles are 16x16 patches");
+    constexpr int NV = 2;
+    const int cw = warp / 4 - 1;
+    const int wq = (threadIdx.x >> 5) & 3, jl = lane & 7, hl = (lane >> 3) & 1;
+    const int wrow = 16 * wq + 2 * jl + (hl ^ (jl >> 2));
+    const uint32_t halo_w = (uint32_t)WTW + 2;
+    const uint64_t halo_desc = ((uint64_t)1 << 16) | ((uint64_t)((halo_w * 128) >> 4) << 32) | ((uint64_t)1 << 62);
+    for (int i = cw; worker + i * n_workers < a.total_tiles; i += 2) {
+      int img, h0, w0, nt;
+      coords(worker + i * n_workers, img, h0, w0, nt);
+      int astage = (i * kchunks) % NA, stage = (i * kiters) % STAGES;
+      uint32_t aphase = (uint32_t)((i * kchunks) / NA) & 1u, phase = (uint32_t)((i * kiters) / STAGES) & 1u;
+      if (i > 0) mbar_wait(&order_bar[cw], (uint32_t)((i - 1) >> 1) & 1u);
+      AccWide acc;
+      int prev = -1, prev_a = -1, kc = 0, tap = 0;
+      uint32_t f[2][2][4];
+      for (int kit = 0; kit < kiters; ++kit) {
+        if (tap == 0) mbar_wait(&afull_bar[astage], aphase);
+        mbar_wait(&full_bar[stage], phase);
+        const uint32_t sb = ring_a + stage * STAGE_BYTES;
+        ldsm_a_sw128(f[0][0], sb, wrow, 0);
+        ldsm_a_sw128(f[0][1], sb + B_BYTES, wrow, 0);
+        const uint32_t ha = smem_a + astage * HALO_STAGE;
+        const uint32_t toff = ((uint32_t)(tap / 3) * halo_w + (uint32_t)(tap % 3)) * 128u;
+        const uint64_t x_hi = halo_desc | (uint64_t)(((ha + toff) >> 4) & 0x3fffu);
+        const uint64_t x_lo = halo_desc | (uint64_t)(((ha + HALO_PLANE + toff) >> 4) & 0x3fffu);
+        const uint32_t acc0 = (kc > 0 || tap > 0) ? 1u : 0u;
+#pragma unroll
+        for (int k = 0; k < TC_BK / 16; ++k) {
+          const uint32_t(&fh)[4] = f[k & 1][0];
+          const uint32_t(&fl)[4] = f[k & 1][1];
+          const uint64_t ko = (uint64_t)(k * 2);
+          wgmma_fence();
+#pragma unroll
+          for (int v = 0; v < NV; ++v) WgmmaRS<256 / NV>::mma(acc.d[v], fh, x_lo + 64 * v + ko, (acc0 | k) ? 1u : 0u);
+#pragma unroll
+          for (int v = 0; v < NV; ++v) WgmmaRS<256 / NV>::mma(acc.d[v], fl, x_hi + 64 * v + ko, 1u);
+#pragma unroll
+          for (int v = 0; v < NV; ++v) WgmmaRS<256 / NV>::mma(acc.d[v], fh, x_hi + 64 * v + ko, 1u);
+          wgmma_commit();
+          if (k == 3 && kc == kchunks - 1 && tap == 8 && lane == 0) mbar_arrive(&order_bar[cw ^ 1]);
+          wgmma_wait<1>();
+          if (k == 0) {
+            if (prev >= 0) release_w(prev);
+            if (prev_a >= 0) {
+              if (lane == 0) mbar_arrive(&aempty_bar[prev_a]);
+              prev_a = -1;
+            }
+          }
+          if (k + 1 < TC_BK / 16) {
+            ldsm_a_sw128(f[(k + 1) & 1][0], sb, wrow, k + 1);
+            ldsm_a_sw128(f[(k + 1) & 1][1], sb + B_BYTES, wrow, k + 1);
+          }
+        }
+        prev = stage;
+        if (++stage == STAGES) { stage = 0; phase ^= 1; }
+        if (++tap == 9) {
+          tap = 0;
+          ++kc;
+          prev_a = astage;
+          if (++astage == NA) { astage = 0; aphase ^= 1; }
+        }
+      }
+      wgmma_wait<0>();
+#pragma unroll
+      for (int v = 0; v < NV; ++v)
+#pragma unroll
+        for (int e = 0; e < 128 / NV; ++e) asm volatile("" : "+f"(acc.d[v][e])::"memory");
+      release_w(prev);
+      if (lane == 0) mbar_arrive(&aempty_bar[prev_a]);
+      conv_wide_epilogue(a, acc, img, h0, w0, nt);
+    }
+    } else if constexpr (HALO) {
     setmaxnreg_inc<232>();
     const int cw = warp / 4 - 1;
     const int bar = 1 + cw;
@@ -382,7 +579,7 @@
       int prev = -1, prev_a = -1;
       for (int kc = 0; kc < kchunks; ++kc) {
         mbar_wait(&afull_bar[astage], aphase);
-        const uint32_t ha = smem_a + astage * TC_HALO_STAGE;
+        const uint32_t ha = smem_a + astage * HALO_STAGE;
         for (int tap = 0; tap < 9; ++tap) {
           mbar_wait(&full_bar[stage], phase);
           const uint32_t toff = ((uint32_t)(tap / 3) * halo_w + (uint32_t)(tap % 3)) * 128u;
@@ -459,25 +656,29 @@
   __syncthreads();
 }
 
-template <int BN, int STAGES, bool HALO = false, int NA = 0>
+template <int BN, int STAGES, bool HALO = false, int NA = 0, int WTW = 0>
 static int launch_tc_variant(const CUtensorMap& xhi, const CUtensorMap& xlo, const CUtensorMap& whi,
                              const CUtensorMap& wlo, const ConvTcArgs& a, cudaStream_t s) {
-  constexpr int smem = ConvTcSmem<BN, STAGES, HALO, NA>::BYTES;
+  constexpr int smem = ConvTcSmem<BN, STAGES, HALO, NA, WTW>::BYTES;
   static_assert(smem <= 232448, "shared-memory budget");
   static DeviceOnce attr_done;
   if (!attr_done.done()) {
-    IBL_CUDA_OK(cudaFuncSetAttribute(conv3x3_tc_kernel<BN, STAGES, HALO, NA>, cudaFuncAttributeMaxDynamicSharedMemorySize, smem));
+    IBL_CUDA_OK(cudaFuncSetAttribute(conv3x3_tc_kernel<BN, STAGES, HALO, NA, WTW>,
+                                     cudaFuncAttributeMaxDynamicSharedMemorySize, smem));
     attr_done.mark();
   }
   const int sms = device_sm_count();
   const int grid = a.total_tiles < sms ? a.total_tiles : sms;
-  conv3x3_tc_kernel<BN, STAGES, HALO, NA><<<grid, ConvTcSmem<BN, STAGES, HALO, NA>::THREADS, smem, s>>>(xhi, xlo, whi, wlo, a);
+  conv3x3_tc_kernel<BN, STAGES, HALO, NA, WTW>
+      <<<grid, ConvTcSmem<BN, STAGES, HALO, NA, WTW>::THREADS, smem, s>>>(xhi, xlo, whi, wlo, a);
   IBL_CUDA_OK(cudaGetLastError());
   return IBL_OK;
 }
 
 static int g_tc_bn_override = 0;
 void tc_set_bn_override(int bn) { g_tc_bn_override = bn; }
+static int g_tc_variant_override = 0;
+void tc_set_variant_override(int v) { g_tc_variant_override = v; }
 
 int launch_conv3x3_tc(const __nv_bfloat16* x_hi, const __nv_bfloat16* x_lo, const ConvParams& p,
                       int N, int H, int W, int cin, int cout, bool relu, bool pool,
@@ -488,25 +689,30 @@
   IBL_REQUIRE(H >= 1 && W >= 1 && N >= 1, "empty conv input");
   ConvTcArgs a{};
   a.N = N; a.H = H; a.W = W; a.cin = cin; a.cout = cout;
-  auto waste = [&](int tw) {
-    int th = 128 / tw;
+  auto waste = [&](int tw, int px) {
+    int th = px / tw;
     return (long long)cdiv(W, tw) * tw * cdiv(H, th) * th;
   };
-  a.tw_log2 = (waste(16) <= waste(8)) ? 4 : 3;
-  const int TW = 1 << a.tw_log2, TH = 128 / TW;
+  const int tw128 = (waste(16, 128) <= waste(8, 128)) ? 16 : 8;
+  constexpr int tw256 = 16;
+  bool wide = waste(tw256, 256) <= waste(tw128, 128);
+  if (g_tc_bn_override) wide = false;
+  if (g_tc_variant_override) wide = g_tc_variant_override == 2;
+  const int TW = wide ? tw256 : tw128, TH = (wide ? TC_WIDE_PX : TC_BM) / TW;
+  a.tw_log2 = TW == 16 ? 4 : 3;
   a.tiles_w = cdiv(W, TW);
   a.tiles_h = cdiv(H, TH);
-  int bn = cout % 128 == 0 ? 128 : 64;
-  if (g_tc_bn_override && cout % g_tc_bn_override == 0 && (g_tc_bn_override == 64 || g_tc_bn_override == 128))
+  int bn = wide ? 64 : cout % 128 == 0 ? 128 : 64;
+  if (!wide && g_tc_bn_override && cout % g_tc_bn_override == 0 && (g_tc_bn_override == 64 || g_tc_bn_override == 128))
     bn = g_tc_bn_override;
-  const bool halo = bn == 128;
+  const bool halo = wide || bn == 128;
   a.n_tiles = cout / bn;
   a.total_tiles = (int)((long long)N * a.tiles_h * a.tiles_w * a.n_tiles);
   a.relu = relu; a.pool = pool;
   a.bias = p.bias; a.y_hi = y_hi; a.y_lo = y_lo; a.y_f32 = y_f32;
   a.ssq = pool ? nullptr : ssq;
   a.ssq_stride = (long long)N * H * W;
-  if (ssq_parts) *ssq_parts = a.n_tiles;
+  if (ssq_parts) *ssq_parts = wide ? cout / 16 : a.n_tiles;
 
   CUtensorMap m_xhi, m_xlo, m_whi, m_wlo;
   {
@@ -523,6 +729,7 @@
     IBL_RET(make_tmap(&m_whi, CU_TENSOR_MAP_DATA_TYPE_BFLOAT16, 3, p.w_hi, dims, str, box));
     IBL_RET(make_tmap(&m_wlo, CU_TENSOR_MAP_DATA_TYPE_BFLOAT16, 3, p.w_lo, dims, str, box));
   }
+  if (wide) return launch_tc_variant<64, 3, true, 2, 16>(m_xhi, m_xlo, m_whi, m_wlo, a, s);
   if (halo) return launch_tc_variant<128, 3, true, 2>(m_xhi, m_xlo, m_whi, m_wlo, a, s);
   return launch_tc_variant<64, 4>(m_xhi, m_xlo, m_whi, m_wlo, a, s);
 }
diff --git a/openibl_b200/csrc/tc_probe.cu b/openibl_b200/csrc/tc_probe.cu
--- a/openibl_b200/csrc/tc_probe.cu
+++ b/openibl_b200/csrc/tc_probe.cu
@@ -88,4 +88,86 @@
   return IBL_OK;
 }
 
+template <int N>
+__global__ void __launch_bounds__(128, 1)
+wgmma_rs_halo_probe_kernel(const __grid_constant__ CUtensorMap tm_w, const __grid_constant__ CUtensorMap tm_x, int pitch,
+                           int s0, uint32_t x_bytes, float* __restrict__ D) {
+  extern __shared__ __align__(1024) uint8_t smem_raw[];
+  uint8_t* smem = reinterpret_cast<uint8_t*>((reinterpret_cast<uintptr_t>(smem_raw) + 1023) & ~uintptr_t(1023));
+  uint8_t* w_sm = smem;
+  uint8_t* x_sm = smem + 8192;
+  uint64_t* bars = reinterpret_cast<uint64_t*>(smem + 8192 + 45056);
+  if (threadIdx.x == 0) {
+    mbar_init(&bars[0], 1);
+    fence_barrier_init();
+    fence_proxy_async();
+  }
+  __syncthreads();
+  if (threadIdx.x == 0) {
+    mbar_arrive_expect_tx(&bars[0], 8192 + x_bytes);
+    tma_load_2d(w_sm, &tm_w, &bars[0], 0, 0);
+    tma_load_3d(x_sm, &tm_x, &bars[0], 0, 0, 0);
+  }
+  mbar_wait(&bars[0], 0);
+  const int t = threadIdx.x, lane = t & 31;
+  const int row = 16 * (t >> 5) + (lane & 7) + 8 * ((lane >> 3) & 1);
+  const uint64_t xd = ((uint64_t)1 << 16) | ((uint64_t)(((uint32_t)pitch * 128u) >> 4) << 32) | ((uint64_t)1 << 62) |
+                      (uint64_t)(((smem_u32(x_sm) + (uint32_t)s0 * 128u) >> 4) & 0x3fffu);
+  float d[N / 2];
+  uint32_t f[4][4];
+#pragma unroll
+  for (int k = 0; k < 4; ++k) ldsm_a_sw128(f[k], smem_u32(w_sm), row, k);
+  wgmma_fence();
+#pragma unroll
+  for (int k = 0; k < 4; ++k) WgmmaRS<N>::mma(d, f[k], xd + (uint64_t)(k * 2), k > 0 ? 1u : 0u);
+  wgmma_commit();
+  wgmma_wait<0>();
+#pragma unroll
+  for (int i = 0; i < N / 2; ++i) asm volatile("" : "+f"(d[i])::"memory");
+  const int r0 = 16 * (t >> 5) + (lane >> 2), c0 = 2 * (lane & 3);
+#pragma unroll
+  for (int i = 0; i < N / 8; ++i)
+#pragma unroll
+    for (int e = 0; e < 4; ++e) D[(size_t)(r0 + 8 * (e >> 1)) * N + 8 * i + c0 + (e & 1)] = d[4 * i + e];
 }
+
+int debug_wgmma_rs_halo(const void* W, const void* X, int pitch, int hrows, int n, int s0, float* D, cudaStream_t s) {
+  IBL_REQUIRE(n == 64 || n == 128, "probe view: n is 64 or 128");
+  IBL_REQUIRE(pitch >= 8 && pitch <= 256 && hrows >= 1 && hrows <= 256 && pitch * hrows <= 352 && s0 >= 0 &&
+                  s0 + (n / 8 - 1) * pitch + 8 <= pitch * hrows,
+              "probe view does not fit the halo tile");
+  CUtensorMap mw, mx;
+  {
+    uint64_t dims[2] = {64, 64};
+    uint64_t str[1] = {128};
+    uint32_t box[2] = {64, 64};
+    IBL_RET(make_tmap(&mw, CU_TENSOR_MAP_DATA_TYPE_BFLOAT16, 2, W, dims, str, box));
+  }
+  {
+    uint64_t dims[3] = {64, (uint64_t)pitch, (uint64_t)hrows};
+    uint64_t str[2] = {128, (uint64_t)pitch * 128};
+    uint32_t box[3] = {64, (uint32_t)pitch, (uint32_t)hrows};
+    IBL_RET(make_tmap(&mx, CU_TENSOR_MAP_DATA_TYPE_BFLOAT16, 3, X, dims, str, box));
+  }
+  const int smem = 8192 + 45056 + 1024 + 64;
+  const uint32_t x_bytes = (uint32_t)pitch * (uint32_t)hrows * 128u;
+  if (n == 64) {
+    static DeviceOnce attr_done;
+    if (!attr_done.done()) {
+      IBL_CUDA_OK(cudaFuncSetAttribute(wgmma_rs_halo_probe_kernel<64>, cudaFuncAttributeMaxDynamicSharedMemorySize, smem));
+      attr_done.mark();
+    }
+    wgmma_rs_halo_probe_kernel<64><<<1, 128, smem, s>>>(mw, mx, pitch, s0, x_bytes, D);
+  } else {
+    static DeviceOnce attr_done;
+    if (!attr_done.done()) {
+      IBL_CUDA_OK(cudaFuncSetAttribute(wgmma_rs_halo_probe_kernel<128>, cudaFuncAttributeMaxDynamicSharedMemorySize, smem));
+      attr_done.mark();
+    }
+    wgmma_rs_halo_probe_kernel<128><<<1, 128, smem, s>>>(mw, mx, pitch, s0, x_bytes, D);
+  }
+  IBL_CUDA_OK(cudaGetLastError());
+  return IBL_OK;
+}
+
+}
diff --git a/openibl_b200/csrc/wgmma.cuh b/openibl_b200/csrc/wgmma.cuh
--- a/openibl_b200/csrc/wgmma.cuh
+++ b/openibl_b200/csrc/wgmma.cuh
@@ -5,6 +5,7 @@
 namespace tc {
 
 template <int N, bool F16, int TA, int TB> struct Wgmma;
+template <int N> struct WgmmaRS;
 
 template <> struct Wgmma<32, false, 0, 0> {
   static __device__ __forceinline__ void mma(float (&d)[16], uint64_t a, uint64_t b, uint32_t accumulate) {
@@ -66,5 +67,25 @@
   }
 };
 
+template <> struct WgmmaRS<64> {
+  static __device__ __forceinline__ void mma(float (&d)[32], const uint32_t (&a)[4], uint64_t b, uint32_t accumulate) {
+    asm volatile(
+        "{\n\t.reg .pred p;\n\tsetp.ne.b32 p, %37, 0;\n\t"
+        "wgmma.mma_async.sync.aligned.m64n64k16.f32.bf16.bf16 {%0, %1, %2, %3, %4, %5, %6, %7, %8, %9, %10, %11, %12, %13, %14, %15, %16, %17, %18, %19, %20, %21, %22, %23, %24, %25, %26, %27, %28, %29, %30, %31}, {%32, %33, %34, %35}, %36, p, 1, 1, 0;\n\t}"
+        : "+f"(d[0]), "+f"(d[1]), "+f"(d[2]), "+f"(d[3]), "+f"(d[4]), "+f"(d[5]), "+f"(d[6]), "+f"(d[7]), "+f"(d[8]), "+f"(d[9]), "+f"(d[10]), "+f"(d[11]), "+f"(d[12]), "+f"(d[13]), "+f"(d[14]), "+f"(d[15]), "+f"(d[16]), "+f"(d[17]), "+f"(d[18]), "+f"(d[19]), "+f"(d[20]), "+f"(d[21]), "+f"(d[22]), "+f"(d[23]), "+f"(d[24]), "+f"(d[25]), "+f"(d[26]), "+f"(d[27]), "+f"(d[28]), "+f"(d[29]), "+f"(d[30]), "+f"(d[31])
+        : "r"(a[0]), "r"(a[1]), "r"(a[2]), "r"(a[3]), "l"(b), "r"(accumulate));
+  }
+};
+
+template <> struct WgmmaRS<128> {
+  static __device__ __forceinline__ void mma(float (&d)[64], const uint32_t (&a)[4], uint64_t b, uint32_t accumulate) {
+    asm volatile(
+        "{\n\t.reg .pred p;\n\tsetp.ne.b32 p, %69, 0;\n\t"
+        "wgmma.mma_async.sync.aligned.m64n128k16.f32.bf16.bf16 {%0, %1, %2, %3, %4, %5, %6, %7, %8, %9, %10, %11, %12, %13, %14, %15, %16, %17, %18, %19, %20, %21, %22, %23, %24, %25, %26, %27, %28, %29, %30, %31, %32, %33, %34, %35, %36, %37, %38, %39, %40, %41, %42, %43, %44, %45, %46, %47, %48, %49, %50, %51, %52, %53, %54, %55, %56, %57, %58, %59, %60, %61, %62, %63}, {%64, %65, %66, %67}, %68, p, 1, 1, 0;\n\t}"
+        : "+f"(d[0]), "+f"(d[1]), "+f"(d[2]), "+f"(d[3]), "+f"(d[4]), "+f"(d[5]), "+f"(d[6]), "+f"(d[7]), "+f"(d[8]), "+f"(d[9]), "+f"(d[10]), "+f"(d[11]), "+f"(d[12]), "+f"(d[13]), "+f"(d[14]), "+f"(d[15]), "+f"(d[16]), "+f"(d[17]), "+f"(d[18]), "+f"(d[19]), "+f"(d[20]), "+f"(d[21]), "+f"(d[22]), "+f"(d[23]), "+f"(d[24]), "+f"(d[25]), "+f"(d[26]), "+f"(d[27]), "+f"(d[28]), "+f"(d[29]), "+f"(d[30]), "+f"(d[31]), "+f"(d[32]), "+f"(d[33]), "+f"(d[34]), "+f"(d[35]), "+f"(d[36]), "+f"(d[37]), "+f"(d[38]), "+f"(d[39]), "+f"(d[40]), "+f"(d[41]), "+f"(d[42]), "+f"(d[43]), "+f"(d[44]), "+f"(d[45]), "+f"(d[46]), "+f"(d[47]), "+f"(d[48]), "+f"(d[49]), "+f"(d[50]), "+f"(d[51]), "+f"(d[52]), "+f"(d[53]), "+f"(d[54]), "+f"(d[55]), "+f"(d[56]), "+f"(d[57]), "+f"(d[58]), "+f"(d[59]), "+f"(d[60]), "+f"(d[61]), "+f"(d[62]), "+f"(d[63])
+        : "r"(a[0]), "r"(a[1]), "r"(a[2]), "r"(a[3]), "l"(b), "r"(accumulate));
+  }
+};
+
 }
 }
diff --git a/openibl_b200/engine.py b/openibl_b200/engine.py
--- a/openibl_b200/engine.py
+++ b/openibl_b200/engine.py
@@ -652,7 +652,7 @@
               "ibl_maxpool2x2_backward")
         return gx
 
-    def debug_conv3x3(self, x_nhwc, w_oihw, bias, relu=True, pool=False, mode=CONV_TC_BF16X3, bn=0):
+    def debug_conv3x3(self, x_nhwc, w_oihw, bias, relu=True, pool=False, mode=CONV_TC_BF16X3, bn=0, variant=0):
         x = _require_cuda(x_nhwc, "x")
         w = _require_cuda(w_oihw, "w")
         b = _require_cuda(bias, "bias")
@@ -660,9 +660,13 @@
         cout = w.shape[0]
         oh, ow = (H // 2, W // 2) if pool else (H, W)
         y = torch.empty(N, oh, ow, cout, device=x.device)
-        check(self.lib.ibl_debug_conv3x3(self.h, _ptr(x), N, H, W, cin, _ptr(w), _ptr(b), cout, int(relu),
-                                         int(pool), int(mode), int(bn), _ptr(y), _stream(self.device)),
-              "ibl_debug_conv3x3")
+        check(self.lib.ibl_debug_set_conv3x3_variant(self.h, int(variant)), "ibl_debug_set_conv3x3_variant")
+        try:
+            check(self.lib.ibl_debug_conv3x3(self.h, _ptr(x), N, H, W, cin, _ptr(w), _ptr(b), cout, int(relu),
+                                             int(pool), int(mode), int(bn), _ptr(y), _stream(self.device)),
+                  "ibl_debug_conv3x3")
+        finally:
+            self.lib.ibl_debug_set_conv3x3_variant(self.h, 0)
         return y
 
     def debug_conv1_fused(self, x_nchw):
```
